# Ruyi-Zha/endosurf

Measured on AMD Instinct MI355X. Metric: training rays/sec (1024 rays x 64 samples), higher is better.
Workload: dtype f32

## Files before the change

### endosurf_amd/_lib.py

```python
from __future__ import annotations

import ctypes as C
import os

HERE = os.path.dirname(os.path.abspath(__file__))
LIB_PATH = os.path.join(HERE, "lib", "libendosurf_hip.so")

_c_float_p = C.c_void_p


class es_points(C.Structure):
    _fields_ = [("x", C.c_void_p), ("t", C.c_void_p), ("dirs", C.c_void_p), ("rays", C.c_void_p), ("z", C.c_void_p),
                ("mode", C.c_int), ("t_scalar", C.c_int), ("n_per_ray", C.c_int), ("ldz", C.c_int), ("M", C.c_int), ("M_split", C.c_int)]


class es_composite_args(C.Structure):
    _fields_ = ([(n, C.c_void_p) for n in ("rays", "z")] + [("ldz", C.c_int)]
                + [(n, C.c_void_p) for n in ("sdf", "g_o", "rgb", "variance")]
                + [("N", C.c_int), ("S", C.c_int), ("sample_dist", C.c_float), ("cos_anneal", C.c_float)]
                + [(n, C.c_void_p) for n in ("color", "depth", "weights", "cdf", "weight_max", "eik_acc", "wmax_idx",
                                             "g_color", "g_depth", "g_weights", "g_cdf", "g_wmax", "g_gradients_o", "g_eik",
                                             "eik_den", "d_sdf", "d_go", "d_rgb", "d_invs_acc", "ray_part", "cos_anneal_dev",
                                             "go_copy", "g_aux_sdf", "g_aux_go")] + [("n_aux", C.c_int)])


class es_render_args(C.Structure):
    _fields_ = [("c", es_composite_args), ("ws", C.c_void_p), ("scratch", C.c_void_p), ("flags", C.c_int), ("wg_scratch", C.c_void_p), ("packed_x3", C.c_void_p)]


class es_loss_args(C.Structure):
    _fields_ = ([(n, C.c_void_p) for n in ("color_map", "depth_map", "eik", "aux_sdf", "aux_go", "rays", "eod_pts", "color_gt", "depth_gt",
                                            "mask", "cmask", "valid_sn")]
                + [("N", C.c_int)] + [(n, C.c_float) for n in ("w_color", "w_depth", "w_sdf", "w_angle", "w_eik", "w_sn")]
                + [(n, C.c_void_p) for n in ("terms", "g_color", "g_depth", "g_eik", "g_aux_sdf", "g_aux_go", "den_out", "den_global")]
                + [("world", C.c_float), ("total_out", C.c_void_p)])


_P = C.c_void_p
_I = C.c_int
_F = C.c_float

PROTOTYPES = {
    "es_abi_version": (C.c_int, []),
    "es_last_error": (C.c_char_p, []),
    "es_init": (C.c_int, []),
    "es_param_floats": (C.c_int64, []),
    "es_param_layout": (C.c_int, [C.c_int, C.c_int, C.POINTER(C.c_int64), C.POINTER(C.c_int64), C.POINTER(C.c_int64),
                                  C.POINTER(C.c_int), C.POINTER(C.c_int)]),
    "es_param_variance_off": (C.c_int64, []),
    "es_weff_floats": (C.c_int64, []),
    "es_weff_layout": (C.c_int, [C.c_int, C.c_int, C.POINTER(C.c_int64), C.POINTER(C.c_int64)]),
    "es_packed_floats": (C.c_int64, []),
    "es_weightnorm_pack": (C.c_int, [_c_float_p, _c_float_p, _c_float_p, C.c_int, C.c_void_p]),
    "es_weightnorm_backward": (C.c_int, [_c_float_p, _c_float_p, _c_float_p, C.c_int, C.c_void_p]),
    "es_query_sdf": (C.c_int, [C.POINTER(es_points), _c_float_p, _c_float_p, _c_float_p, C.c_int, C.c_void_p]),
    "es_query_sdf_tiles": (C.c_int, [C.POINTER(es_points), _c_float_p, _c_float_p, _c_float_p, C.c_int, C.c_int, C.c_void_p]),
    "es_deform_forward": (_I, [C.POINTER(es_points), _P, _P, _P, _P, _P]),
    "es_deform_inverse": (_I, [C.POINTER(es_points), _P, _P, _P, _I, _F, _P, _P, _P, _P]),
    "es_deform_jacobian": (_I, [C.POINTER(es_points), _P, _P, _P, _P, _P]),
    "es_strain_rows": (_I, [_P, _P, _P, _I, _P, _P, _P, _P, _P, _P, _P]),
    "es_trace_surface": (_I, [_P, _I, _F, _F, _F, _F, _I, _I, _P, _P, _I, _P, _P, _P, _P, _P, _P]),
    "es_packed_x3_bytes": (C.c_int64, []),
    "es_pack_x3": (_I, [_P, _P, _I, _P]),
    "es_query_sdf_x3": (_I, [C.POINTER(es_points), _P, _P, _P, _I, _P, _I, _P]),
    "es_ray_setup": (_I, [_P, _P, _I, _I, _F, _I, _P, _I, _P, _P, _P]),
    "es_upsample_step": (_I, [_P, _P, _I, _P, _I, _I, _I, _I, _F, _P, _P, _I, _P, _P]),
    "es_merge_sdf": (_I, [_P, _I, _P, _I, _P, _I, _I, _I, _P, _P]),
    "es_mid_z": (_I, [_P, _I, _I, _I, _F, _P, _P]),
    "es_composite_forward": (_I, [C.POINTER(es_composite_args), _P]),
    "es_composite_backward": (_I, [C.POINTER(es_composite_args), _P]),
    "es_march_find": (_I, [_P, _P, _I, _I, _F, _P, _P, _P, _P]),
    "es_secant_points": (_I, [_P, _P, _I, _P, _P, _P]),
    "es_secant_update": (_I, [_P, _I, _F, _P, _P, _P]),
    "es_march_finish": (_I, [_P, _P, _I, _P, _P]),
    "es_point_workspace_floats": (C.c_int64, [_I, _I]),
    "es_point_workspace_offset": (C.c_int64, [_I, _I, _I]),
    "es_point_forward": (_I, [C.POINTER(es_points), _P, _P, _P, _I, _I, _P]),
    "es_point_forward_rows": (_I, [C.POINTER(es_points), _P, _P, _P, _I, _I, _I, _I, _P]),
    "es_eod_points": (_I, [_P, _P, _P, _I, _P, _P, _P, _P]),
    "es_sn_points": (_I, [_P, _P, _P, _P, _F, _I, _P, _P, _P, _P]),
    "es_eod_loss": (_I, [_P, _P, _P, _P, _P, _I, _P, _P, _P]),
    "es_eod_loss_backward": (_I, [_P, _P, _P, _P, _P, _P, _P, _I, _P, _P, _P]),
    "es_sn_loss": (_I, [_P, _P, _I, _P, _P]),
    "es_sn_loss_backward": (_I, [_P, _P, _P, _P, _I, _P, _P]),
    "es_copy2": (_I, [_P, _P, C.c_longlong, _P, _P, C.c_longlong, _P]),
    "es_color_forward": (_I, [C.POINTER(es_points), _P, _P, _P, _P]),
    "es_point_vjp": (_I, [C.POINTER(es_points), _P, _P, _P, _I, _P]),
    "es_point_backward_stages": (_I, [C.POINTER(es_points), _P, _P, _P, _I, _I, _P, _P, _P, _P, _P, _I, _P]),
    "es_weightnorm_backward_layers": (_I, [_P, _P, _P, _I, _I, _P]),
    "es_point_forward_x3": (_I, [C.POINTER(es_points), _P, _P, _P, _P, _I, _I, _P]),
    "es_gemm_atb": (_I, [_P, _P, _I, _P, _I, _P, _P]),
    "es_point_backward_x3": (_I, [C.POINTER(es_points), _P, _P, _P, _P, _I, _I, _P, _P, _P, _P, _P, _P]),
    "es_point_backward": (_I, [C.POINTER(es_points), _P, _P, _P, _I, _I, _P, _P, _P, _P, _P]),
    "es_wgrad_scratch_floats": (C.c_int64, []),
    "es_point_backward_det": (_I, [C.POINTER(es_points), _P, _P, _P, _I, _I, _P, _P, _P, _P, _P, _P]),
    "es_train_loss": (_I, [C.POINTER(es_loss_args), _P]),
    "es_query_sdf_rays": (_I, [C.POINTER(es_points), _P, _P, _P, _I, _P, _I, _P]),
    "es_march_progress": (_I, [_P, _I, _I, _I, C.c_float, _P, _P]),
    "es_variance_terms": (_I, [_P, _P, _P, _P, _P]),
    "es_sample_scratch_floats": (C.c_int64, [_I, _I, _I, _I]),
    "es_sample_z": (_I, [_P, _P, _I, _I, _I, _I, _I, _P, _P, _I, _P, _P, _P]),
    "es_march_scratch_floats": (C.c_int64, [_I, _I]),
    "es_ray_marching": (_I, [_P, _I, _I, _I, C.c_float, _I, _P, _P, _I, _P, _P, _P]),
    "es_render_scratch_floats": (C.c_int64, [_I, _I]),
    "es_render_forward": (_I, [C.POINTER(es_render_args), _P, _P, _P]),
    "es_render_backward": (_I, [C.POINTER(es_render_args), _P, _P, _P, _P]),
    "es_train_aux_points": (_I, [_P, _P, _P, _P, _P, C.c_float, _I, _P, _P, _P, _P]),
    "es_adam_step": (_I, [_P, _P, _P, _P, C.c_longlong, C.c_float, C.c_float, C.c_float, C.c_float, C.c_float, C.c_float, _P, C.c_longlong, _P]),
    "es_train_schedule": (_I, [_P, C.c_double, C.c_double, C.c_double, C.c_double, C.c_double, C.c_double, C.c_float, C.c_double, _P, _P]),
    "es_adam_step_dev": (_I, [_P, _P, _P, _P, C.c_longlong, C.c_float, C.c_float, C.c_float, _P, _P, C.c_longlong, _P]),
    "es_zero": (_I, [_P, C.c_longlong, _P]),
    "es_uniform": (_I, [_P, C.c_longlong, C.c_ulonglong, C.c_ulonglong, _P, _P]),
    "es_scale": (_I, [_P, _P, C.c_longlong, _P, _P]),
    "es_render_finish": (_I, [_P, _P, _P, _I, _P, _P, _P, _P, _P]),
    "es_iso_scratch_bytes": (C.c_int64, [_I, _I, _I]),
    "es_iso_count": (_I, [_P, _I, _I, _I, C.c_double, _P, _P, _P]),
    "es_iso_emit": (_I, [_P, _I, _I, _I, C.c_double, _P, C.c_longlong, C.c_longlong, _P, _P, _P, _P]),
    "es_cubes_scratch_bytes": (C.c_int64, [_I, _I, _I]),
    "es_cubes_count": (_I, [_P, _I, _I, _I, C.c_double, _P, _P, _P]),
    "es_cubes_emit": (_I, [_P, _I, _I, _I, C.c_double, _P, C.c_longlong, C.c_longlong, _P, _P, _P, _P]),
    "es_band_scratch_bytes": (C.c_int64, [_I, _I, _I, _I]),
    "es_band_lattice_points": (_I, [_P, _P, _P, _I, _I, _I, _I, C.c_longlong, C.c_longlong, _P, _P]),
    "es_band_seed": (_I, [_P, _I, _I, _I, _I, C.c_double, C.c_double, _P, _P, _P]),
# ... 102 lines not shown
```

### endosurf_amd/csrc/api.hip

```cpp
#include "arch.h"
#include "chain_common.h"
#include "host.h"
#include "launch.h"
#include "workspace.h"

namespace es {
static inline PointSrc to_src(const es_points* p) { PointSrc s; static_cast<es_points&>(s) = *p; return s; }
static inline int check_src(const es_points* p) {
    ES_REQUIRE(p != nullptr, "es_points is null");
    ES_REQUIRE(p->M >= 0, "negative point count");
    if (p->M == 0) return ST_OK;
    if (p->mode == 0) {
        ES_REQUIRE(p->x && p->t, "mode 0 needs x and t");
    } else {
        ES_REQUIRE(p->mode == 1 || p->mode == 2, "unknown point-source mode");
        ES_REQUIRE(p->rays && p->z && p->n_per_ray > 0 && p->ldz >= p->n_per_ray, "modes 1/2 need rays, z, n_per_ray <= ldz");
        if (p->mode == 2) ES_REQUIRE(p->M_split >= 0 && p->M_split <= p->M && (p->M_split == p->M || (p->x && p->t)), "mode 2 needs M_split <= M and x, t");
    }
    return ST_OK;
}
static inline int check_points(const es_points* p, bool weights, bool rows) {
    if (int e = check_src(p)) return e;
    ES_REQUIRE(weights && (rows || p->M == 0), "null buffer");
    return ST_OK;
// ... 143 lines not shown
    constexpr float FMAX = 3.402823466e+38f;
    ES_REQUIRE(N >= 0, "es_trace_surface: N must not be negative");
    ES_REQUIRE(tau >= -FMAX && tau <= FMAX, "es_trace_surface: tau must be finite");
    ES_REQUIRE(eps >= 0.f && eps <= FMAX, "es_trace_surface: eps must be finite and not negative");
    ES_REQUIRE(relax > 0.f && relax <= 1.f, "es_trace_surface: relax must be in (0, 1]");
    ES_REQUIRE(min_step > 0.f && min_step <= FMAX, "es_trace_surface: min_step must be finite and positive");
    ES_REQUIRE(max_iters >= 1 && max_iters <= ES_TRACE_MAX_ITERS, "es_trace_surface: max_iters must be in [1, 1024]");
    ES_REQUIRE(tile_points == 0 || tile_points == 32 || tile_points == 64, "es_trace_surface: tile_points: 0 (the library's choice), 32 or 64");
    if (N == 0) return ST_OK;
    ES_REQUIRE(rays && packed && weff && depth_out && status_out, "es_trace_surface: null buffer (rays, packed, weff, depth_out, status_out)");
    return trace_surface(rays, N, tau, eps, relax, min_step, max_iters, tile_points, packed, weff, use_deform, depth_out, status_out, iters_out,
                         residual_out, points_out, (hipStream_t)stream);
}
int64_t es_packed_x3_bytes(void) { return (int64_t)packed_x3_bytes(); }
int es_pack_x3(const float* weff, void* packed_x3, int use_deform, void* stream) {
    ES_REQUIRE(weff && packed_x3, "null buffer");
    return pack_x3(weff, packed_x3, use_deform, (hipStream_t)stream);
}
int es_query_sdf_x3(const es_points* pts, const void* packed_x3, const float* weff, float* sdf_out, int ld_out, const int* ray_done,
                    int use_deform, void* stream) {
    if (int e = check_points(pts, packed_x3 && weff, sdf_out)) return e;
    ES_REQUIRE(ld_out == 0 || (pts->mode == 1 && ld_out >= pts->n_per_ray), "ld_out > 0 needs ray samples (mode 1), ld_out >= n_per_ray");
    ES_REQUIRE(ray_done == nullptr || pts->mode == 1, "ray_done needs ray samples (mode 1)");
    return query_sdf_x3(to_src(pts), packed_x3, weff, sdf_out, use_deform, (hipStream_t)stream, ld_out, ray_done);
}
int es_variance_terms(const float* variance, const float* d_invs_acc, float* s_val, float* d_var, void* stream) {
    ES_REQUIRE(variance && (s_val || d_var) && (!d_var || d_invs_acc), "es_variance_terms arguments");
    return variance_terms(variance, d_invs_acc, s_val, d_var, (hipStream_t)stream);
}
int es_march_progress(const float* sdf, int N, int n, int n_valid, float tau, int* done, void* stream) {
    if (N == 0) return ST_OK;
    ES_REQUIRE(sdf && done && n >= 2 && n_valid >= 1 && n_valid <= n, "es_march_progress arguments");
    return march_progress(sdf, N, n, n_valid, tau, done, (hipStream_t)stream);
}

int es_ray_setup(const float* rays, const float* u, int N, int n, float sample_dist, int lin_mode, float* z, int ldz,
                 float* near_out, float* far_out, void* stream) {
    if (N == 0) return ST_OK;
    ES_REQUIRE(rays && z && N >= 0 && n >= 1 && ldz >= n, "es_ray_setup arguments");
    return ray_setup(rays, u, N, n, sample_dist, lin_mode, z, ldz, near_out, far_out, (hipStream_t)stream);
}
int es_upsample_step(const float* rays, const float* z_in, int ld_in, const float* sdf_in, int ld_sdf, int N, int n, int n_imp,
                     float inv_s, float* z_new, float* z_out, int ld_out, int32_t* src_idx, void* stream) {
    if (N == 0) return ST_OK;
    ES_REQUIRE(rays && z_in && sdf_in && z_new && z_out && src_idx && ld_in >= n && ld_sdf >= n, "es_upsample_step arguments");
    return upsample_step(rays, z_in, ld_in, sdf_in, ld_sdf, N, n, n_imp, inv_s, z_new, z_out, ld_out, src_idx, (hipStream_t)stream);
}
int es_merge_sdf(const float* sdf_in, int ld_in, const float* sdf_new, int n_imp, const int32_t* src_idx, int ld_out, int N, int n,
                 float* sdf_out, void* stream) {
    if (N == 0) return ST_OK;
    ES_REQUIRE(sdf_in && sdf_new && src_idx && sdf_out && sdf_out != sdf_in, "es_merge_sdf arguments (out must not alias in)");
    return merge_sdf(sdf_in, ld_in, sdf_new, n_imp, src_idx, ld_out, N, n, sdf_out, (hipStream_t)stream);
}
int es_mid_z(const float* z, int ldz, int N, int S, float sample_dist, float* mid, void* stream) {
    if (N == 0) return ST_OK;
    ES_REQUIRE(z && mid && ldz >= S && S >= 1, "es_mid_z arguments");
    return mid_z(z, ldz, N, S, sample_dist, mid, (hipStream_t)stream);
}
int es_composite_forward(const es_composite_args* a, void* stream) {
    if (a && a->N == 0) return ST_OK;
    ES_REQUIRE(a && a->rays && a->z && a->sdf && a->g_o && a->rgb && a->variance, "es_composite_forward inputs");
    ES_REQUIRE(a->color && a->depth && a->weights && a->cdf && a->weight_max && a->eik_acc && a->wmax_idx, "es_composite_forward outputs");
    return composite(as_comp(a), 0, (hipStream_t)stream);
}
int es_composite_backward(const es_composite_args* a, void* stream) {
    if (a && a->N == 0) return ST_OK;
    ES_REQUIRE(a && a->rays && a->z && a->sdf && a->g_o && a->rgb && a->variance, "es_composite_backward inputs");
    ES_REQUIRE(a->n_aux >= 0, "es_composite_backward: negative n_aux");
    ES_REQUIRE(a->g_color && a->g_depth && a->g_eik && a->eik_den && a->d_sdf && a->d_go && a->d_rgb && a->d_invs_acc,
               "es_composite_backward adjoints");
    return composite(as_comp(a), 1, (hipStream_t)stream);
}
int es_march_find(const float* sdf, const float* dprop, int N, int n, float tau, float* state, int32_t* flags, float* d_pred, void* stream) {
    if (N == 0) return ST_OK;
    ES_REQUIRE(sdf && dprop && state && flags && d_pred && n >= 2, "es_march_find arguments");
    return march_find(sdf, dprop, N, n, tau, state, flags, d_pred, (hipStream_t)stream);
}
int es_secant_points(const float* rays, const float* d_pred, int N, float* x, float* t, void* stream) {
    if (N == 0) return ST_OK;
    ES_REQUIRE(rays && d_pred && x && t, "es_secant_points arguments");
    return secant_points(rays, d_pred, N, x, t, (hipStream_t)stream);
}
int es_secant_update(const float* sdf_mid, int N, float tau, float* state, float* d_pred, void* stream) {
    if (N == 0) return ST_OK;
    ES_REQUIRE(sdf_mid && state && d_pred, "es_secant_update arguments");
    return secant_update(sdf_mid, N, tau, state, d_pred, (hipStream_t)stream);
}
int es_march_finish(const float* d_pred, const int32_t* flags, int N, float* d_out, void* stream) {
    if (N == 0) return ST_OK;
    ES_REQUIRE(d_pred && flags && d_out, "es_march_finish arguments");
    return march_finish(d_pred, flags, N, d_out, (hipStream_t)stream);
}

int64_t es_point_workspace_floats(int M, int flags) { return M <= 0 ? 0 : (int64_t)ws_layout(M, flags).off[WS_COUNT]; }
int64_t es_point_workspace_offset(int M, int flags, int buffer_id) {
    if (M <= 0 || buffer_id < 0 || buffer_id >= WS_COUNT) return -1;
    return (int64_t)ws_layout(M, flags).off[buffer_id];
}
int es_point_forward(const es_points* pts, const float* packed, const float* weff, float* ws, int flags, int m_color, void* stream) {
    if (int e = check_point_call(pts, packed && weff, ws, flags, m_color, false)) return e;
    return point_forward(to_src(pts), packed, weff, ws, flags, m_color, (hipStream_t)stream);
}
int es_point_forward_rows(const es_points* pts, const float* packed, const float* weff, float* ws, int flags, int m_color, int row0, int nrows,
                          void* stream) {
    if (int e = check_points(pts, packed && weff, ws)) return e;
    ES_REQUIRE(!(flags & (ES_PF_X3 | ES_PF_X3_CHAIN)), "es_point_forward_rows: fp32 family only");
    ES_REQUIRE(!(flags & ES_PF_COLOR) || pts->mode != 0 || pts->dirs, "colour evaluation needs view directions");
    ES_REQUIRE(row0 >= 0 && nrows >= 0, "es_point_forward_rows: negative row range");
    if (int e = check_mcolor(pts, flags, m_color)) return e;
    return point_forward_rows(to_src(pts), packed, weff, ws, flags, m_color, row0, nrows, (hipStream_t)stream);
}
int es_eod_points(const float* rays, const float* depth_gt, const float* mask, int N, float* x, float* t, float* inside, void* stream) {
    ES_REQUIRE(N >= 0 && (N == 0 || (rays && depth_gt && x && t)), "es_eod_points buffers");
    ES_REQUIRE(inside == nullptr || mask != nullptr || N == 0, "es_eod_points: the inside mask needs the ray mask");
    return eod_points(rays, depth_gt, mask, N, x, t, inside, (hipStream_t)stream);
}
int es_sn_points(const float* rays, const float* mask, const float* d_i, const float* u, float rad, int N, float* x, float* t,
                 unsigned char* valid, void* stream) {
    ES_REQUIRE(N >= 0 && (N == 0 || (rays && mask && d_i && u && x && t && valid)), "es_sn_points buffers");
    return sn_points(rays, mask, d_i, u, rad, N, x, t, valid, (hipStream_t)stream);
}
int es_eod_loss(const float* rays, const float* pts, const float* mask, const float* sdf, const float* g_o, int N, float* out, float* inside,
                void* stream) {
    ES_REQUIRE(N >= 0 && out && (N == 0 || (rays && pts && mask && sdf && g_o && inside)), "es_eod_loss buffers");
// ... 120 lines not shown
```

### endosurf_amd/csrc/host.h

```cpp
#pragma once
#include <hip/hip_runtime.h>

#include <cstddef>
#include <type_traits>

#include "../../include/endosurf_hip.h"

namespace es {

struct PointSrc; struct WsLayout; struct FwdArgs; struct BwdArgs;

struct CompositeArgs : ::es_composite_args {};
struct LossArgs : ::es_loss_args {};
static_assert(sizeof(CompositeArgs) == sizeof(es_composite_args) && std::is_standard_layout<CompositeArgs>::value, "es::CompositeArgs is es_composite_args");
static_assert(sizeof(LossArgs) == sizeof(es_loss_args) && std::is_standard_layout<LossArgs>::value, "es::LossArgs is es_loss_args");
inline const CompositeArgs& as_comp(const es_composite_args* a) { return *reinterpret_cast<const CompositeArgs*>(a); }

int init_tables();
int weightnorm_pack(const float* params, float* weff, float* packed, int use_deform, hipStream_t st);
int weightnorm_backward(const float* params, const float* dweff, float* dparams, int use_deform, hipStream_t st);
int weightnorm_backward_layers(const float* params, const float* dweff, float* dparams, int first_layer, int n_layers, hipStream_t st);

int query_sdf(const PointSrc& src, const float* packed, const float* weff, float* sdf_out, int use_deform, hipStream_t st,
              int ld_out = 0, const int* ray_done = nullptr, int tile_points = 0);
int query_sdf16(const PointSrc& src, const float* packed, const float* weff, float* sdf_out, int use_deform, hipStream_t st);
size_t packed_x3_bytes();
int pack_x3(const float* weff, void* packed_x3, int use_deform, hipStream_t st);
int query_sdf_x3(const PointSrc& src, const void* packed_x3, const float* weff, float* sdf_out, int use_deform, hipStream_t st, int ld_out, const int* ray_done);

int deform_forward(const PointSrc& src, const float* packed, const float* weff, float* xc_out, float* d_out, hipStream_t st);
int deform_inverse(const PointSrc& src, const float* init, const float* packed, const float* weff, int max_iters, float tol, float* y_out,
                   float* step_out, int* iters_out, hipStream_t st);

int trace_surface(const float* rays, int N, float tau, float eps, float relax, float min_step, int max_iters, int tile_points,
                  const float* packed, const float* weff, int use_deform, float* depth_out, int* status_out, int* iters_out,
                  float* residual_out, float* points_out, hipStream_t st);

int deform_jacobian(const PointSrc& src, const float* packed, const float* weff, float* jac_out, float* xc_out, hipStream_t st);
int strain_rows(const float* jac_from, const float* jac_to, const float* normals, int M, float* F_out, float* det_out, float* stretch_out,
                float* area_out, float* surface_out, unsigned char* valid_out, hipStream_t st);

int point_forward(const PointSrc& src, const float* packed, const float* weff, float* ws, int flags, int m_color, hipStream_t st,
                  const void* packed_x3 = nullptr);
int point_forward_rows(const PointSrc& src, const float* packed, const float* weff, float* ws, int flags, int m_color, int row0, int nrows, hipStream_t st);
int point_vjp(const PointSrc& src, const float* packed, const float* weff, float* ws, int flags, hipStream_t st);
int color_forward(const PointSrc& src, const float* packed, const float* weff, float* ws, hipStream_t st);
int point_backward_chains(const PointSrc& src, const float* packed, const float* weff, float* ws, int flags, int m_color,
                          const float* d_sdf, const float* d_go, const float* d_rgb, hipStream_t st, const void* packed_x3 = nullptr);

int deform_jvp_x3r(const PointSrc& src, const void* packed_r, const float* weff, float* ws, const WsLayout& L, bool save, hipStream_t st);
int deform_vjp_x3r(const PointSrc& src, const void* packed_r, const float* weff, float* ws, const WsLayout& L, bool save, hipStream_t st, int m_rows = 0);
int deform_jvp_x3r_with_tail(const FwdArgs& fa, const void* packed_r, int m_main, hipStream_t st);
int sdf_fwd_x3r(const PointSrc& src, const void* packed_r, const float* weff, float* ws, const WsLayout& L, bool deform, bool color, hipStream_t st);
int color_fwd_x3r(const PointSrc& src, const void* packed_r, const float* weff, float* ws, const WsLayout& L, bool deform, int Mcp, bool save, hipStream_t st);

int deform_tan_x3r(const PointSrc& src, const void* packed_r, const float* weff, float* ws, const WsLayout& L, const float* d_go, hipStream_t st, int m_rows = 0);
int deform_bwd_x3r_with_tail(const BwdArgs& ba, const void* packed_r, int m_main, hipStream_t st);
int color_bwd_x3r(const PointSrc& src, const void* packed_r, const float* weff, float* ws, const WsLayout& L, bool deform, int m_color, const float* d_rgb, hipStream_t st);
int deform_bwd_x3r(const void* packed_r, const float* weff, float* ws, const WsLayout& L, int M, int m_color, hipStream_t st);

int point_wgrad(int M, float* ws, int flags, int m_color, const float* d_sdf, float* dweff, float* det, hipStream_t st, int net_mask = 7);
size_t wgrad_det_floats();
int gemm_atb(const float* X, const float* dA, int M, float* out, int x3, float* det, hipStream_t st);

int ray_setup(const float* rays, const float* u, int N, int n, float sample_dist, int lin_mode, float* z, int ldz, float* near_out, float* far_out, hipStream_t st);
int upsample_step(const float* rays, const float* z_in, int ld_in, const float* sdf_in, int ld_sdf, int N, int n, int n_imp,
                  float inv_s, float* z_new, float* z_out, int ld_out, int* src_idx, hipStream_t st);
int merge_sdf(const float* sdf_in, int ld_in, const float* sdf_new, int n_imp, const int* src_idx, int ld_out, int N, int n, float* sdf_out, hipStream_t st);
int mid_z(const float* z, int ldz, int N, int S, float sample_dist, float* mid, hipStream_t st);
int composite(const CompositeArgs& a, int backward, hipStream_t st);
int variance_terms(const float* variance, const float* d_invs_acc, float* s_val, float* d_var, hipStream_t st);
int march_progress(const float* sdf, int N, int n, int n_valid, float tau, int* done, hipStream_t st);
int march_find(const float* sdf, const float* dprop, int N, int n, float tau, float* state, int* flags, float* d_pred, hipStream_t st);
int secant_points(const float* rays, const float* d_pred, int N, float* x, float* t, hipStream_t st);
int secant_update(const float* sdf_mid, int N, float tau, float* state, float* d_pred, hipStream_t st);
int march_finish(const float* d_pred, const int* flags, int N, float* d_out, hipStream_t st);
int train_aux_points(const float* rays, const float* depth_gt, const float* mask, const float* d_i, const float* u, float rad, int N, float* x, float* t, unsigned char* valid, hipStream_t st);

int eod_points(const float* rays, const float* depth_gt, const float* mask, int N, float* x, float* t, float* inside, hipStream_t st);
int sn_points(const float* rays, const float* mask, const float* d_i, const float* u, float rad, int N, float* x, float* t, unsigned char* valid, hipStream_t st);
int eod_loss(const float* rays, const float* pts, const float* mask, const float* sdf, const float* go, int N, float* out, float* inside, hipStream_t st);
int eod_loss_bwd(const float* rays, const float* inside, const float* sdf, const float* go, const float* out, const float* g_sdf_err,
                 const float* g_ang_err, int N, float* d_sdf, float* d_go, hipStream_t st);
int sn_loss(const float* g, const unsigned char* valid, int N, float* out, hipStream_t st);
int sn_loss_bwd(const float* g, const unsigned char* valid, const float* out, const float* g_loss, int N, float* d_g, hipStream_t st);
int copy2(float* da, const float* sa, long long na, float* db, const float* sb, long long nb, hipStream_t st);

int train_loss(const LossArgs& a, hipStream_t st);
int train_schedule(double* state, double lr_init, double n_iter, double warm_up_end, double lr_alpha, double beta1, double beta2, float grad_scale, double anneal_end, float* scal, hipStream_t st);
int adam_step_dev(float* p, const float* g, float* m, float* v, long long n, float beta1, float beta2, float eps, const float* scal, const float* g_extra, long long extra_index, hipStream_t st);
int adam_step(float* p, const float* g, float* m, float* v, long long n, float beta1, float beta2, float eps, float step_size,
              float bc2_sqrt, float grad_scale, const float* g_extra, long long extra_index, hipStream_t st);
int uniform(float* out, long long n, unsigned long long seed, unsigned long long subseq, const double* subseq_dev, hipStream_t st);
int scale(float* out, const float* in, long long n, const float* s, hipStream_t st);
int zero(void* p, long long nbytes, hipStream_t st);
int render_finish(const float* eik_acc, const float* aux_sdf_ws, const float* aux_go_ws, int n_aux, float* eik, float* eik_den, float* aux_sdf, float* aux_go, hipStream_t st);

}
```

### endosurf_amd/csrc/pack.hip

```cpp
#include <hip/hip_runtime.h>

#include "arch.h"
#include "host.h"
#include "launch.h"

namespace es {

struct SegDev {
    int net, layer, dir, row0, col0, kreal, nreal, skip_scale, kg, nt;
    unsigned long long off4;
};
__constant__ SegDev c_segs[SEG_COUNT];
__constant__ int c_layer_k[NETS * LAYERS];
__constant__ int c_layer_n[NETS * LAYERS];
__constant__ int c_param_off[NETS * LAYERS];
__constant__ int c_weff_off[NETS * LAYERS];
__constant__ int c_p16_segs[P16_COUNT];
#define P16_SEGS_DEV(i) c_p16_segs[i]

static DeviceOnce g_tables_ready;

int init_tables() {
    if (!g_tables_ready.first()) return 0;
    SegDev h[SEG_COUNT];
    size_t off = 0;
    for (int i = 0; i < SEG_COUNT; ++i) {
        const SegDesc& s = SEGS[i];
        h[i] = {s.net, s.layer, s.dir, s.row0, s.col0, s.kreal, s.nreal, s.skip_scale, seg_kg(s), seg_nt(s), (unsigned long long)off};
        off += (size_t)seg_kg(s) * seg_nt(s) * 64;
    }
    int lk[NETS * LAYERS], ln[NETS * LAYERS], po[NETS * LAYERS], wo[NETS * LAYERS];
    int p = 0, w = 0;
    for (int n = 0; n < NETS; ++n)
        for (int l = 0; l < LAYERS; ++l) {
            lk[n * LAYERS + l] = LAYER_K[n][l];
            ln[n * LAYERS + l] = LAYER_N[n][l];
            po[n * LAYERS + l] = p;
            wo[n * LAYERS + l] = w;
            p += LAYER_N[n][l] * (2 + LAYER_K[n][l]);
            w += LAYER_N[n][l] * (1 + LAYER_K[n][l]);
        }
    ES_HIP(hipMemcpyToSymbol(HIP_SYMBOL(c_segs), h, sizeof(h)));
    ES_HIP(hipMemcpyToSymbol(HIP_SYMBOL(c_layer_k), lk, sizeof(lk)));
    ES_HIP(hipMemcpyToSymbol(HIP_SYMBOL(c_layer_n), ln, sizeof(ln)));
    ES_HIP(hipMemcpyToSymbol(HIP_SYMBOL(c_param_off), po, sizeof(po)));
    ES_HIP(hipMemcpyToSymbol(HIP_SYMBOL(c_weff_off), wo, sizeof(wo)));
    ES_HIP(hipMemcpyToSymbol(HIP_SYMBOL(c_p16_segs), P16_SEGS, sizeof(P16_SEGS)));
    g_tables_ready.done();
    return 0;
}

__device__ __forceinline__ float wave_sum(float v) {
#pragma unroll
    for (int o = 32; o > 0; o >>= 1) v += __shfl_xor(v, o, 64);
    return v;
}

__global__ __launch_bounds__(256) void k_weff(const float* __restrict__ params, float* __restrict__ weff, int first_layer) {
    const int li = first_layer + blockIdx.y;
    const int N = c_layer_n[li], K = c_layer_k[li];
    const int n = blockIdx.x * 4 + (threadIdx.x >> 6);
    const int lane = threadIdx.x & 63;
    if (n >= N) return;
    const float* pb = params + c_param_off[li];
    const float* pg = pb + N;
    const float* pv = pg + N + (size_t)n * K;
    float ss = 0.f;
    for (int k = lane; k < K; k += 64) { const float v = pv[k]; ss = fmaf(v, v, ss); }
    ss = wave_sum(ss);
    const float scale = pg[n] / sqrtf(ss);
    float* w = weff + c_weff_off[li];
    for (int k = lane; k < K; k += 64) w[(size_t)n * K + k] = scale * pv[k];
    if (lane == 0) w[(size_t)N * K + n] = pb[n];
}

__global__ __launch_bounds__(256) void k_pack(const float* __restrict__ weff, float4* __restrict__ packed, int first_net) {
    const unsigned long long idx = (unsigned long long)blockIdx.x * 256 + threadIdx.x;
    if (idx >= PACKED_FLOAT4) return;
    int s = 0;
#pragma unroll 1
    for (int i = 1; i < SEG_COUNT; ++i)
        if (idx >= c_segs[i].off4) s = i;
    const SegDev sd = c_segs[s];
    if (sd.net < first_net) return;
    const unsigned rel = (unsigned)(idx - sd.off4);
    const int lane = rel & 63;
    const int g = (rel >> 6) % sd.kg;
    const int nt = (rel >> 6) / sd.kg;
    const int li = sd.net * LAYERS + sd.layer;
    const int K = c_layer_k[li];
    const float* W = weff + c_weff_off[li];
    const float sc = sd.skip_scale ? INV_SQRT2 : 1.f;
    const int n = 32 * nt + (lane & 31);
    float o[4];
#pragma unroll
    for (int j = 0; j < 4; ++j) {
        const int k = 8 * g + 2 * j + (lane >> 5);
        float v = 0.f;
        if (k < sd.kreal && n < sd.nreal) {
            const int row = sd.dir == 0 ? sd.row0 + n : sd.row0 + k;
            const int col = sd.dir == 0 ? sd.col0 + k : sd.col0 + n;
            v = sc * W[(size_t)row * K + col];
        }
        o[j] = v;
    }
    packed[idx] = make_float4(o[0], o[1], o[2], o[3]);
}

__global__ __launch_bounds__(256) void k_weightnorm_bwd(const float* __restrict__ params, const float* __restrict__ dweff,
                                                        float* __restrict__ dparams, int first_layer) {
    const int li = first_layer + blockIdx.y;
    const int N = c_layer_n[li], K = c_layer_k[li];
    const int n = blockIdx.x * 4 + (threadIdx.x >> 6);
    const int lane = threadIdx.x & 63;
    if (n >= N) return;
    const float* pb = params + c_param_off[li];
    const float* pg = pb + N;
    const float* pv = pg + N + (size_t)n * K;
    const float* dw = dweff + c_weff_off[li] + (size_t)n * K;
    const float lscale = (li % LAYERS) == 4 ? INV_SQRT2 : 1.f;
    float ss = 0.f, dot = 0.f;
    for (int k = lane; k < K; k += 64) { const float v = pv[k]; ss = fmaf(v, v, ss); dot = fmaf(dw[k] * lscale, v, dot); }
    ss = wave_sum(ss); dot = wave_sum(dot);
    const float inv = 1.f / sqrtf(ss);
    const float dg = dot * inv;
    const float gs = pg[n] * inv;
    float* ob = dparams + c_param_off[li];
    float* og = ob + N;
    float* ov = og + N + (size_t)n * K;
    for (int k = lane; k < K; k += 64) ov[k] = gs * (dw[k] * lscale - dg * inv * pv[k]);
    if (lane == 0) { og[n] = dg; ob[n] = dweff[c_weff_off[li] + (size_t)N * K + n]; }
}

__global__ __launch_bounds__(256) void k_pack16(const float* __restrict__ weff, float4* __restrict__ packed, int first_net) {
    const unsigned long long idx = PACKED_FLOAT4 + (unsigned long long)blockIdx.x * 256 + threadIdx.x;
    if (idx >= PACKED_TOTAL_FLOAT4) return;
    int pi = 0;
    unsigned long long base = PACKED_FLOAT4, off = PACKED_FLOAT4;
#pragma unroll 1
    for (int i = 0; i < P16_COUNT; ++i) {
        const unsigned long long sz = (unsigned long long)((c_segs[P16_SEGS_DEV(i)].kreal + 15) / 16) * 16 * 64;
        if (idx >= off) { pi = i; base = off; }
        off += sz;
    }
    const SegDev sd = c_segs[P16_SEGS_DEV(pi)];
    if (sd.net < first_net) return;
    const int kg = (sd.kreal + 15) / 16;
    const unsigned rel = (unsigned)(idx - base);
    const int lane = rel & 63;
    const int g = (rel >> 6) % kg;
    const int nt = (rel >> 6) / kg;
    const int li = sd.net * LAYERS + sd.layer;
    const int K = c_layer_k[li];
    const float* W = weff + c_weff_off[li];
    const float sc = sd.skip_scale ? INV_SQRT2 : 1.f;
    const int n = 16 * nt + (lane & 15);
    float o[4];
#pragma unroll
    for (int j = 0; j < 4; ++j) {
        const int k = 16 * g + 4 * j + (lane >> 4);
        o[j] = (k < sd.kreal && n < sd.nreal) ? sc * W[(size_t)(sd.row0 + n) * K + sd.col0 + k] : 0.f;
    }
    packed[idx] = make_float4(o[0], o[1], o[2], o[3]);
}

int weightnorm_pack(const float* params, float* weff, float* packed, int use_deform, hipStream_t st) {
    if (int e = init_tables()) return e;
    const int first_layer = use_deform ? 0 : LAYERS;
    dim3 g1(65, NETS * LAYERS - first_layer);
    hipLaunchKernelGGL(k_weff, g1, dim3(256), 0, st, params, weff, first_layer);
    const unsigned nb = (unsigned)((PACKED_FLOAT4 + 255) / 256);
    hipLaunchKernelGGL(k_pack, dim3(nb), dim3(256), 0, st, (const float*)weff, reinterpret_cast<float4*>(packed), use_deform ? 0 : 1);
    const unsigned nb16 = (unsigned)((PACKED_TOTAL_FLOAT4 - PACKED_FLOAT4 + 255) / 256);
    hipLaunchKernelGGL(k_pack16, dim3(nb16), dim3(256), 0, st, (const float*)weff, reinterpret_cast<float4*>(packed), use_deform ? 0 : 1);
    return hip_last("weightnorm_pack");
}

int weightnorm_backward_layers(const float* params, const float* dweff, float* dparams, int first_layer, int n_layers, hipStream_t st) {
    if (int e = init_tables()) return e;
    if (n_layers <= 0) return ST_OK;
    dim3 g1(65, n_layers);
    hipLaunchKernelGGL(k_weightnorm_bwd, g1, dim3(256), 0, st, params, dweff, dparams, first_layer);
    return hip_last("weightnorm_backward_layers");
}

int weightnorm_backward(const float* params, const float* dweff, float* dparams, int use_deform, hipStream_t st) {
    if (int e = init_tables()) return e;
    const int first_layer = use_deform ? 0 : LAYERS;
    dim3 g1(65, NETS * LAYERS - first_layer);
    hipLaunchKernelGGL(k_weightnorm_bwd, g1, dim3(256), 0, st, params, dweff, dparams, first_layer);
    return hip_last("weightnorm_backward");
}

}
```

### endosurf_amd/csrc/rays.hip

```cpp
#include <hip/hip_runtime.h>

#include "host.h"
#include "launch.h"

namespace es {

constexpr int RAY_NMAX = 256;
constexpr int WAVES_PER_BLOCK = 4;

__device__ __forceinline__ float wsum(float v) {
#pragma unroll
    for (int o = 32; o > 0; o >>= 1) v += __shfl_xor(v, o, 64);
    return v;
}
__device__ __forceinline__ float wmax(float v) {
#pragma unroll
    for (int o = 32; o > 0; o >>= 1) v = fmaxf(v, __shfl_xor(v, o, 64));
    return v;
}
__device__ __forceinline__ float wscan_add(float v, int lane) {
#pragma unroll
    for (int o = 1; o < 64; o <<= 1) { const float t = __shfl_up(v, o, 64); if (lane >= o) v += t; }
    return v;
}
__device__ __forceinline__ float wscan_mul(float v, int lane) {
#pragma unroll
    for (int o = 1; o < 64; o <<= 1) { const float t = __shfl_up(v, o, 64); if (lane >= o) v *= t; }
    return v;
}
__device__ __forceinline__ float sigmoidf_acc(float x) { return 1.f / (1.f + expf(-x)); }

__device__ __forceinline__ float linspace_f32(float start, float end, int steps, int i) {
    if (steps == 1) return start;
    const float step = (end - start) / (float)(steps - 1);
    return i < steps / 2 ? start + step * (float)i : end - step * (float)(steps - 1 - i);
}

struct RayGeom { float o[3], d[3], dz[3], t; };
__device__ __forceinline__ RayGeom load_ray(const float* __restrict__ rays, int ray) {
    RayGeom g;
    const float* r = rays + 9 * (size_t)ray;
    g.o[0] = r[0]; g.o[1] = r[1]; g.o[2] = r[2];
    g.d[0] = r[3]; g.d[1] = r[4]; g.d[2] = r[5];
    const float inv = r[5] + 1e-6f;
    g.dz[0] = r[3] / inv; g.dz[1] = r[4] / inv; g.dz[2] = r[5] / inv;
    g.t = r[8];
    return g;
}
__device__ __forceinline__ void sphere_near_far(const RayGeom& g, float& near, float& far) {
    const float dd = g.d[0] * g.d[0] + g.d[1] * g.d[1] + g.d[2] * g.d[2];
    const float d1 = -(g.d[0] * g.o[0] + g.d[1] * g.o[1] + g.d[2] * g.o[2]) / dd;
    const float p0 = g.o[0] + d1 * g.d[0], p1 = g.o[1] + d1 * g.d[1], p2 = g.o[2] + d1 * g.d[2];
    const float tmp = 1.f - (p0 * p0 + p1 * p1 + p2 * p2);
    const float d2 = sqrtf(fmaxf(tmp, 0.f)) / sqrtf(dd);
    near = fmaxf(d1 - d2, 0.f);
    far = d1 + d2;
}
__device__ __forceinline__ float pt_norm(const RayGeom& g, float z) {
    const float x = g.o[0] + g.dz[0] * z, y = g.o[1] + g.dz[1] * z, w = g.o[2] + g.dz[2] * z;
    return sqrtf(x * x + y * y + w * w);
}

__global__ __launch_bounds__(256) void k_ray_setup(const float* __restrict__ rays, const float* __restrict__ u, int N, int n,
                                                   float sample_dist, int lin_mode, float* __restrict__ z, int ldz,
                                                   float* __restrict__ near_out, float* __restrict__ far_out) {
    const int ray = blockIdx.x * WAVES_PER_BLOCK + (threadIdx.x >> 6), lane = threadIdx.x & 63;
    if (ray >= N) return;
    const RayGeom g = load_ray(rays, ray);
    float near, far;
    sphere_near_far(g, near, far);
    const float shift = u ? (u[ray] - 0.5f) * sample_dist : 0.f;
    for (int s = lane; s < n; s += 64) {
        const float tv = linspace_f32(0.f, 1.f, n, s);
        float v = lin_mode == 0 ? near + (far - near) * tv : near * (1.f - tv) + far * tv;
        if (u) v = v + shift;
        z[(size_t)ray * ldz + s] = v;
    }
    if (lane == 0) { if (near_out) near_out[ray] = near; if (far_out) far_out[ray] = far; }
}

__global__ __launch_bounds__(256) void k_upsample_step(const float* __restrict__ rays, const float* __restrict__ z_in, int ld_in,
                                                       const float* __restrict__ sdf_in, int ld_sdf, int N, int n, int n_imp,
                                                       float inv_s, float* __restrict__ z_new, float* __restrict__ z_out,
                                                       int ld_out, int* __restrict__ src_idx) {
    __shared__ float s_z[WAVES_PER_BLOCK][RAY_NMAX], s_a[WAVES_PER_BLOCK][RAY_NMAX], s_c[WAVES_PER_BLOCK][RAY_NMAX + 1],
        s_new[WAVES_PER_BLOCK][64];
    const int wv = threadIdx.x >> 6, lane = threadIdx.x & 63;
    const int ray = blockIdx.x * WAVES_PER_BLOCK + wv;
    if (ray >= N) return;
    float* zs = s_z[wv]; float* av = s_a[wv]; float* cdf0 = s_c[wv]; float* nz = s_new[wv];
    const RayGeom g = load_ray(rays, ray);
    const int nsec = n - 1;

    for (int e = lane; e < n; e += 64) { zs[e] = z_in[(size_t)ray * ld_in + e]; av[e] = sdf_in[(size_t)ray * ld_sdf + e]; }
    __builtin_amdgcn_wave_barrier();
    for (int e = lane; e < nsec; e += 64) cdf0[e] = (av[e + 1] - av[e]) / (zs[e + 1] - zs[e] + 1e-6f);
    __builtin_amdgcn_wave_barrier();
    float carry = 1.f, wsum_acc = 0.f;
    const int nchunk = (nsec + 63) / 64;
    float wloc[RAY_NMAX / 64];
#pragma unroll
    for (int c = 0; c < RAY_NMAX / 64; ++c) {
        wloc[c] = 0.f;
        if (c < nchunk) {
            const int e = c * 64 + lane;
            float alpha = 0.f, om = 1.f;
            if (e < nsec) {
                const float cosv = cdf0[e], prev = e == 0 ? 0.f : cdf0[e - 1];
                const bool inside = pt_norm(g, zs[e]) < 1.f || pt_norm(g, zs[e + 1]) < 1.f;
                float cv = fminf(fmaxf(fminf(prev, cosv), -1e3f), 0.f);
                cv = inside ? cv : cv * 0.f;
                const float dist = zs[e + 1] - zs[e];
                const float mid = (av[e] + av[e + 1]) * 0.5f;
                const float pe = mid - cv * dist * 0.5f, ne = mid + cv * dist * 0.5f;
                const float pc = sigmoidf_acc(pe * inv_s), nc = sigmoidf_acc(ne * inv_s);
                alpha = (pc - nc + 1e-6f) / (pc + 1e-6f);
                om = 1.f - alpha + 1e-7f;
            }
            const float incl = wscan_mul(om, lane);
            float excl = __shfl_up(incl, 1, 64);
            if (lane == 0) excl = 1.f;
            const float T = carry * excl;
            carry = carry * __shfl(incl, 63, 64);
            const float w = e < nsec ? alpha * T + 1e-5f : 0.f;
            wloc[c] = w;
            wsum_acc += wsum(w);
        }
    }
    __builtin_amdgcn_wave_barrier();
    float run = 0.f;
#pragma unroll
    for (int c = 0; c < RAY_NMAX / 64; ++c) {
        if (c < nchunk) {
            const int e = c * 64 + lane;
            const float pdf = wloc[c] / wsum_acc;
            const float incl = wscan_add(pdf, lane) + run;
            run = __shfl(incl, 63, 64);
            if (e < nsec) cdf0[e + 1] = incl;
        }
    }
    if (lane == 0) cdf0[0] = 0.f;
    __builtin_amdgcn_wave_barrier();
    if (lane < n_imp) {
        const float uu = linspace_f32(0.5f / (float)n_imp, 1.f - 0.5f / (float)n_imp, n_imp, lane);
        int lo = 0, hi = n;
        while (lo < hi) { const int m = (lo + hi) >> 1; if (cdf0[m] <= uu) lo = m + 1; else hi = m; }
        const int below = max(lo - 1, 0), above = min(lo, n - 1);
        float denom = cdf0[above] - cdf0[below];
        if (denom < 1e-5f) denom = 1.f;
        const float tt = (uu - cdf0[below]) / denom;
        const float v = zs[below] + tt * (zs[above] - zs[below]);
        nz[lane] = v;
        z_new[(size_t)ray * n_imp + lane] = v;
    }
    __builtin_amdgcn_wave_barrier();
    for (int e = lane; e < n; e += 64) {
        const float v = zs[e];
        int cnt = 0;
        for (int j = 0; j < n_imp; ++j) cnt += nz[j] < v ? 1 : 0;
        const int r = e + cnt;
        z_out[(size_t)ray * ld_out + r] = v;
        src_idx[(size_t)ray * ld_out + r] = e;
    }
    if (lane < n_imp) {
        const float v = nz[lane];
        int lo = 0, hi = n;
        while (lo < hi) { const int m = (lo + hi) >> 1; if (zs[m] <= v) lo = m + 1; else hi = m; }
        int before = 0;
        for (int j = 0; j < n_imp; ++j) before += (nz[j] < v || (nz[j] == v && j < lane)) ? 1 : 0;
        const int r = lo + before;
        z_out[(size_t)ray * ld_out + r] = v;
        src_idx[(size_t)ray * ld_out + r] = n + lane;
    }
}

__global__ __launch_bounds__(256) void k_merge_sdf(const float* __restrict__ sdf_in, int ld_in, const float* __restrict__ sdf_new,
                                                   int n_imp, const int* __restrict__ src_idx, int ld_out, int N, int n,
                                                   float* __restrict__ sdf_out) {
    const int i = blockIdx.x * 256 + threadIdx.x;
    const int tot = n + n_imp;
    if (i >= N * tot) return;
    const int ray = i / tot, r = i - ray * tot;
    const int s = src_idx[(size_t)ray * ld_out + r];
    float v = __builtin_nanf("");
    if (s >= 0 && s < n) v = sdf_in[(size_t)ray * ld_in + s];
    else if (s >= n && s < tot) v = sdf_new[(size_t)ray * n_imp + (s - n)];
    sdf_out[(size_t)ray * ld_out + r] = v;
}

__global__ __launch_bounds__(256) void k_mid_z(const float* __restrict__ z, int ldz, int N, int S, float sample_dist,
                                               float* __restrict__ mid) {
    const int i = blockIdx.x * 256 + threadIdx.x;
    if (i >= N * S) return;
    const int ray = i / S, s = i - ray * S;
    const float z0 = z[(size_t)ray * ldz + s];
    const float dist = s + 1 < S ? z[(size_t)ray * ldz + s + 1] - z0 : sample_dist;
    mid[(size_t)ray * S + s] = z0 + dist * 0.5f;
}


__device__ __forceinline__ float inv_s_from_variance(float var) { return fminf(fmaxf(expf(var * 10.f), 1e-6f), 1e6f); }

template <bool BWD>
__global__ __launch_bounds__(256) void k_composite(CompositeArgs a) {
    if (BWD && a.n_aux > 0) {
        const size_t P = (size_t)a.N * a.S;
        for (int i = blockIdx.x * 256 + threadIdx.x; i < a.n_aux; i += gridDim.x * 256) {
            a.d_sdf[P + i] = a.g_aux_sdf ? a.g_aux_sdf[i] : 0.f;
#pragma unroll
            for (int k = 0; k < 3; ++k) a.d_go[3 * (P + i) + k] = a.g_aux_go ? a.g_aux_go[3 * (size_t)i + k] : 0.f;
        }
    }
    const int ray = blockIdx.x * WAVES_PER_BLOCK + (threadIdx.x >> 6), lane = threadIdx.x & 63;
    if (ray >= a.N) return;
    const RayGeom g = load_ray(a.rays, ray);
    const float inv_s = inv_s_from_variance(a.variance[0]);
    const float r = a.cos_anneal_dev != nullptr ? a.cos_anneal_dev[0] : a.cos_anneal;
    const int S = a.S;
    const int nchunk = (S + 63) / 64;
    constexpr int CH = RAY_NMAX / 64;
    float alpha[CH], Texc[CH], w[CH], mid[CH], dist[CH], pcv[CH], ncv[CH], sdfv[CH], tc[CH], gnorm[CH], relax[CH], ratio[CH];
    float go[CH][3], rgb[CH][3];
    float carry = 1.f;
    float csum[3] = {0.f, 0.f, 0.f}, dsum = 0.f, wmx = -1.f, e_num = 0.f, e_den = 0.f;
    int wmx_i = 0;
#pragma unroll
    for (int c = 0; c < CH; ++c) {
        if (c < nchunk) {
            const int s = c * 64 + lane;
            const bool ok = s < S;
            const size_t p = (size_t)ray * S + (ok ? s : 0);
            const float z0 = a.z[(size_t)ray * a.ldz + (ok ? s : 0)];
            dist[c] = (ok && s + 1 < S) ? a.z[(size_t)ray * a.ldz + s + 1] - z0 : a.sample_dist;
            mid[c] = z0 + dist[c] * 0.5f;
            sdfv[c] = a.sdf[p];
#pragma unroll
            for (int k = 0; k < 3; ++k) { go[c][k] = a.g_o[3 * p + k]; rgb[c][k] = a.rgb[3 * p + k]; }
            tc[c] = g.d[0] * go[c][0] + g.d[1] * go[c][1] + g.d[2] * go[c][2];
            const float ic = -(fmaxf(-tc[c] * 0.5f + 0.5f, 0.f) * (1.f - r) + fmaxf(-tc[c], 0.f) * r);
            const float nx = sdfv[c] + ic * dist[c] * 0.5f, pv = sdfv[c] - ic * dist[c] * 0.5f;
            pcv[c] = sigmoidf_acc(pv * inv_s);
            ncv[c] = sigmoidf_acc(nx * inv_s);
            ratio[c] = (pcv[c] - ncv[c] + 1e-6f) / (pcv[c] + 1e-6f);
            alpha[c] = ok ? fminf(fmaxf(ratio[c], 0.f), 1.f) : 0.f;
            const float om = ok ? 1.f - alpha[c] + 1e-7f : 1.f;
            const float incl = wscan_mul(om, lane);
            float excl = __shfl_up(incl, 1, 64);
            if (lane == 0) excl = 1.f;
            Texc[c] = carry * excl;
            carry = carry * __shfl(incl, 63, 64);
            w[c] = alpha[c] * Texc[c];
            gnorm[c] = sqrtf(go[c][0] * go[c][0] + go[c][1] * go[c][1] + go[c][2] * go[c][2]);
            relax[c] = (ok && pt_norm(g, mid[c]) < 1.2f) ? 1.f : 0.f;
            if (ok) {
                csum[0] += w[c] * rgb[c][0]; csum[1] += w[c] * rgb[c][1]; csum[2] += w[c] * rgb[c][2];
                dsum += w[c] * mid[c];
                e_num += relax[c] * (gnorm[c] - 1.f) * (gnorm[c] - 1.f);
                e_den += relax[c];
                if (w[c] > wmx) { wmx = w[c]; wmx_i = s; }
            }
        }
    }
    {
        float m = wmx; int mi = wmx_i;
#pragma unroll
        for (int o = 32; o > 0; o >>= 1) {
            const float om = __shfl_xor(m, o, 64); const int oi = __shfl_xor(mi, o, 64);
            if (om > m || (om == m && oi < mi)) { m = om; mi = oi; }
        }
        wmx = m; wmx_i = mi;
    }
    if (!BWD) {
#pragma unroll
        for (int k = 0; k < 3; ++k) csum[k] = wsum(csum[k]);
        dsum = wsum(dsum); e_num = wsum(e_num); e_den = wsum(e_den);
#pragma unroll
        for (int c = 0; c < CH; ++c)
            if (c < nchunk) {
                const int s = c * 64 + lane;
                if (s < S) {
                    a.weights[(size_t)ray * S + s] = w[c]; a.cdf[(size_t)ray * S + s] = pcv[c];
                    if (a.go_copy != nullptr) {
                        const size_t p = (size_t)ray * S + s;
                        a.go_copy[3 * p] = go[c][0]; a.go_copy[3 * p + 1] = go[c][1]; a.go_copy[3 * p + 2] = go[c][2];
                    }
                }
            }
        if (lane == 0) {
            a.color[3 * (size_t)ray + 0] = csum[0]; a.color[3 * (size_t)ray + 1] = csum[1]; a.color[3 * (size_t)ray + 2] = csum[2];
            a.depth[ray] = dsum; a.weight_max[ray] = wmx; a.wmax_idx[ray] = wmx_i;
            if (a.ray_part) { a.ray_part[2 * (size_t)ray] = e_num; a.ray_part[2 * (size_t)ray + 1] = e_den; }
            else { atomicAdd(a.eik_acc + 0, e_num); atomicAdd(a.eik_acc + 1, e_den); }
        }
        return;
    }
    const float gc0 = a.g_color[3 * (size_t)ray], gc1 = a.g_color[3 * (size_t)ray + 1], gc2 = a.g_color[3 * (size_t)ray + 2];
    const float gd = a.g_depth[ray];
    const float gwm = a.g_wmax ? a.g_wmax[ray] : 0.f;
    const float geik = a.g_eik[0] / a.eik_den[0];
    float suffix_carry = 0.f, dinvs = 0.f;
#pragma unroll
    for (int c = CH - 1; c >= 0; --c) {
        if (c < nchunk) {
            const int s = c * 64 + lane;
            const bool ok = s < S;
            const size_t p = (size_t)ray * S + (ok ? s : 0);
            float wbar = 0.f;
            if (ok) {
                wbar = (a.g_weights ? a.g_weights[p] : 0.f) + gc0 * rgb[c][0] + gc1 * rgb[c][1] + gc2 * rgb[c][2] + gd * mid[c];
                if (s == wmx_i) wbar += gwm;
            }
            const float ww = ok ? wbar * w[c] : 0.f;
            float incl = ww;
#pragma unroll
            for (int o = 1; o < 64; o <<= 1) { const float t = __shfl_down(incl, o, 64); if (lane + o < 64) incl += t; }
            const float later = incl - ww + suffix_carry;
            suffix_carry += __shfl(incl, 0, 64);
            if (ok) {
                float abar = wbar * Texc[c] - later / (1.f - alpha[c] + 1e-7f);
                if (ratio[c] < 0.f || ratio[c] > 1.f) abar = 0.f;
                const float cden = pcv[c] + 1e-6f;
                const float pbar = abar / cden;
                const float cbar = -abar * (pcv[c] - ncv[c] + 1e-6f) / (cden * cden) + (a.g_cdf ? a.g_cdf[p] : 0.f);
                const float pcbar = pbar + cbar, ncbar = -pbar;
                const float dpv = pcbar * pcv[c] * (1.f - pcv[c]);
                const float dnx = ncbar * ncv[c] * (1.f - ncv[c]);
                const float ic = -(fmaxf(-tc[c] * 0.5f + 0.5f, 0.f) * (1.f - r) + fmaxf(-tc[c], 0.f) * r);
                const float nx = sdfv[c] + ic * dist[c] * 0.5f, pv = sdfv[c] - ic * dist[c] * 0.5f;
                dinvs += dpv * pv + dnx * nx;
                const float prevbar = dpv * inv_s, nextbar = dnx * inv_s;
                a.d_sdf[p] = prevbar + nextbar;
                const float icbar = (nextbar - prevbar) * dist[c] * 0.5f;
                const float tcbar = icbar * ((-tc[c] * 0.5f + 0.5f > 0.f ? 0.5f * (1.f - r) : 0.f) + (-tc[c] > 0.f ? r : 0.f));
                const float en = relax[c] * geik * 2.f * (gnorm[c] - 1.f);
                const float invn = gnorm[c] > 0.f ? 1.f / gnorm[c] : 0.f;
#pragma unroll
                for (int k = 0; k < 3; ++k) {
                    float v = tcbar * g.d[k] + en * go[c][k] * invn;
                    if (a.g_gradients_o) v += a.g_gradients_o[3 * p + k];
                    a.d_go[3 * p + k] = v;
                    a.d_rgb[3 * p + k] = w[c] * (k == 0 ? gc0 : (k == 1 ? gc1 : gc2));
                }
            }
        }
    }
    dinvs = wsum(dinvs);
    if (lane == 0) {
        if (a.ray_part) a.ray_part[2 * (size_t)ray] = dinvs;
        else atomicAdd(a.d_invs_acc, dinvs);
    }
}
__global__ __launch_bounds__(1024) void k_ray_part_reduce(const float* __restrict__ part, int N, int ncol, float* __restrict__ acc) {
    __shared__ float sh[1024];
    for (int j = 0; j < ncol; ++j) {
        float s = 0.f;
        for (int i = threadIdx.x; i < N; i += 1024) s += part[2 * (size_t)i + j];
        sh[threadIdx.x] = s;
        __syncthreads();
        for (int o = 512; o > 0; o >>= 1) {
            if ((int)threadIdx.x < o) sh[threadIdx.x] += sh[threadIdx.x + o];
            __syncthreads();
        }
        if (threadIdx.x == 0) acc[j] += sh[0];
        __syncthreads();
    }
}

__global__ __launch_bounds__(256) void k_march_find(const float* __restrict__ sdf, const float* __restrict__ dprop, int N, int n,
                                                    float tau, float* __restrict__ state, int* __restrict__ flags,
                                                    float* __restrict__ d_pred) {
    const int ray = blockIdx.x * WAVES_PER_BLOCK + (threadIdx.x >> 6), lane = threadIdx.x & 63;
    if (ray >= N) return;
    const float* v = sdf + (size_t)ray * n;
    int first = 0x7fffffff;
    for (int s = lane; s + 1 < n; s += 64) {
        const float a0 = -(v[s] - tau), a1 = -(v[s + 1] - tau);
        if (a0 * a1 < 0.f) first = min(first, s);
    }
#pragma unroll
    for (int o = 32; o > 0; o >>= 1) first = min(first, __shfl_xor(first, o, 64));
    if (lane == 0) {
        const float v0 = -(v[0] - tau);
        const bool m0 = v0 < 0.f;
        bool mask = false;
        float dl = 0.f, fl = -1.f, dh = 1.f, fh = 1.f;
        if (first != 0x7fffffff) {
            const int i2 = min(first + 1, n - 1);
            fl = -(v[first] - tau); fh = -(v[i2] - tau);
            dl = dprop[(size_t)ray * n + first]; dh = dprop[(size_t)ray * n + i2];
            mask = (fl < 0.f) && m0;
        }
        state[4 * (size_t)ray + 0] = dl; state[4 * (size_t)ray + 1] = fl; state[4 * (size_t)ray + 2] = dh; state[4 * (size_t)ray + 3] = fh;
        flags[ray] = (mask ? 1 : 0) | (m0 ? 2 : 0);
        d_pred[ray] = -fl * (dh - dl) / (fh - fl) + dl;
    }
}
__global__ __launch_bounds__(256) void k_march_progress(const float* __restrict__ sdf, int N, int n, int n_valid, float tau,
                                                        int* __restrict__ done) {
    const int ray = blockIdx.x * WAVES_PER_BLOCK + (threadIdx.x >> 6), lane = threadIdx.x & 63;
    if (ray >= N) return;
    const float* v = sdf + (size_t)ray * n;
    int found = 0;
    for (int s = lane; s + 1 < n_valid; s += 64) {
        const float a0 = -(v[s] - tau), a1 = -(v[s + 1] - tau);
        if (a0 * a1 < 0.f) found = 1;
    }
    if (lane == 0 && !(-(v[0] - tau) < 0.f)) found = 1;
#pragma unroll
    for (int o = 32; o > 0; o >>= 1) found |= __shfl_xor(found, o, 64);
    if (lane == 0) done[ray] = found;
}
__global__ __launch_bounds__(256) void k_secant_points(const float* __restrict__ rays, const float* __restrict__ d_pred, int N,
                                                       float* __restrict__ x, float* __restrict__ t) {
    const int i = blockIdx.x * 256 + threadIdx.x;
    if (i >= N) return;
    const float* r = rays + 9 * (size_t)i;
    const float dp = d_pred[i];
    x[3 * (size_t)i + 0] = r[0] + dp * (r[3] / r[5]);
// ... 10 lines not shown
    if (fm < 0.f) { dl = dp; fl = fm; } else { dh = dp; fh = fm; }
    state[4 * (size_t)i] = dl; state[4 * (size_t)i + 1] = fl; state[4 * (size_t)i + 2] = dh; state[4 * (size_t)i + 3] = fh;
    d_pred[i] = -fl * (dh - dl) / (fh - fl) + dl;
}
__global__ __launch_bounds__(256) void k_march_finish(const float* __restrict__ d_pred, const int* __restrict__ flags, int N,
                                                      float* __restrict__ d_out) {
    const int i = blockIdx.x * 256 + threadIdx.x;
    if (i >= N) return;
    const int f = flags[i];
    float v = (f & 1) ? d_pred[i] : __builtin_inff();
    if (!(f & 2)) v = 0.f;
    d_out[i] = v;
}

__global__ __launch_bounds__(256) void k_train_aux_points(const float* __restrict__ rays, const float* __restrict__ depth_gt,
                                                          const float* __restrict__ mask, const float* __restrict__ d_i,
                                                          const float* __restrict__ u, float rad, int N, float* __restrict__ x,
                                                          float* __restrict__ t, unsigned char* __restrict__ valid) {
    const int i = blockIdx.x * 256 + threadIdx.x;
    if (i >= N) return;
    const float* r = rays + 9 * (size_t)i;
    const float inv = r[5] + 1e-6f;
    const float dz[3] = {r[3] / inv, r[4] / inv, r[5] / inv};
    const float di = d_i[i];
    const bool ok = !__builtin_isinf(di) && !__builtin_isnan(di) && di != 0.f && mask[i] == 1.f;
    const float ds = ok ? di : 0.f, dg = depth_gt[i];
#pragma unroll
    for (int c = 0; c < 3; ++c) {
        const float ps = r[c] + ds * dz[c];
        x[3 * (size_t)i + c] = r[c] + dz[c] * dg;
        x[3 * (size_t)(N + i) + c] = ps;
        x[3 * (size_t)(2 * N + i) + c] = ps + (u[3 * (size_t)i + c] - 0.5f) * rad;
    }
    t[i] = r[8]; t[N + i] = r[8]; t[2 * N + i] = r[8];
    valid[i] = ok ? 1 : 0;
}

static inline dim3 ray_grid(int N) { return dim3((N + WAVES_PER_BLOCK - 1) / WAVES_PER_BLOCK); }

int ray_setup(const float* rays, const float* u, int N, int n, float sample_dist, int lin_mode, float* z, int ldz, float* near_out,
              float* far_out, hipStream_t st) {
    if (N <= 0) return ST_OK;
    hipLaunchKernelGGL(k_ray_setup, ray_grid(N), dim3(256), 0, st, rays, u, N, n, sample_dist, lin_mode, z, ldz, near_out, far_out);
    return hip_last("ray_setup");
}
int upsample_step(const float* rays, const float* z_in, int ld_in, const float* sdf_in, int ld_sdf, int N, int n, int n_imp,
                  float inv_s, float* z_new, float* z_out, int ld_out, int* src_idx, hipStream_t st) {
    ES_REQUIRE(n >= 2 && n <= RAY_NMAX && n_imp >= 1 && n_imp <= 64 && n + n_imp <= ld_out, "upsample_step sizes");
    if (N <= 0) return ST_OK;
    hipLaunchKernelGGL(k_upsample_step, ray_grid(N), dim3(256), 0, st, rays, z_in, ld_in, sdf_in, ld_sdf, N, n, n_imp, inv_s, z_new,
                       z_out, ld_out, src_idx);
    return hip_last("upsample_step");
}
int merge_sdf(const float* sdf_in, int ld_in, const float* sdf_new, int n_imp, const int* src_idx, int ld_out, int N, int n,
              float* sdf_out, hipStream_t st) {
    if (N <= 0) return ST_OK;
    const int tot = N * (n + n_imp);
    hipLaunchKernelGGL(k_merge_sdf, dim3((tot + 255) / 256), dim3(256), 0, st, sdf_in, ld_in, sdf_new, n_imp, src_idx, ld_out, N, n, sdf_out);
    return hip_last("merge_sdf");
}
int mid_z(const float* z, int ldz, int N, int S, float sample_dist, float* mid, hipStream_t st) {
    if (N <= 0) return ST_OK;
    hipLaunchKernelGGL(k_mid_z, dim3((N * S + 255) / 256), dim3(256), 0, st, z, ldz, N, S, sample_dist, mid);
    return hip_last("mid_z");
}
int composite(const CompositeArgs& a, int backward, hipStream_t st) {
    ES_REQUIRE(a.S >= 1 && a.S <= RAY_NMAX, "composite: samples per ray out of range");
    if (a.N <= 0) return ST_OK;
    if (backward) hipLaunchKernelGGL(k_composite<true>, ray_grid(a.N), dim3(256), 0, st, a);
    else hipLaunchKernelGGL(k_composite<false>, ray_grid(a.N), dim3(256), 0, st, a);
    if (a.ray_part)
        hipLaunchKernelGGL(k_ray_part_reduce, dim3(1), dim3(1024), 0, st, a.ray_part, a.N, backward ? 1 : 2, backward ? a.d_invs_acc : a.eik_acc);
    return hip_last("composite");
}
int march_find(const float* sdf, const float* dprop, int N, int n, float tau, float* state, int* flags, float* d_pred, hipStream_t st) {
    if (N <= 0) return ST_OK;
    hipLaunchKernelGGL(k_march_find, ray_grid(N), dim3(256), 0, st, sdf, dprop, N, n, tau, state, flags, d_pred);
    return hip_last("march_find");
}
__global__ void k_variance_terms(const float* __restrict__ variance, const float* __restrict__ d_invs_acc, float* __restrict__ s_val,
                                 float* __restrict__ d_var) {
    if (threadIdx.x != 0 || blockIdx.x != 0) return;
    const float e = expf(variance[0] * 10.f);
    if (s_val) s_val[0] = 1.f / fminf(fmaxf(e, 1e-6f), 1e6f);
    if (d_var) d_var[0] = (e >= 1e-6f && e <= 1e6f) ? d_invs_acc[0] * 10.f * e : 0.f;
}
int variance_terms(const float* variance, const float* d_invs_acc, float* s_val, float* d_var, hipStream_t st) {
    hipLaunchKernelGGL(k_variance_terms, dim3(1), dim3(64), 0, st, variance, d_invs_acc, s_val, d_var);
    return hip_last("variance_terms");
}

int march_progress(const float* sdf, int N, int n, int n_valid, float tau, int* done, hipStream_t st) {
    if (N <= 0) return ST_OK;
    hipLaunchKernelGGL(k_march_progress, ray_grid(N), dim3(256), 0, st, sdf, N, n, n_valid, tau, done);
    return hip_last("march_progress");
}
int secant_points(const float* rays, const float* d_pred, int N, float* x, float* t, hipStream_t st) {
    if (N <= 0) return ST_OK;
    hipLaunchKernelGGL(k_secant_points, dim3((N + 255) / 256), dim3(256), 0, st, rays, d_pred, N, x, t);
    return hip_last("secant_points");
}
int secant_update(const float* sdf_mid, int N, float tau, float* state, float* d_pred, hipStream_t st) {
    if (N <= 0) return ST_OK;
    hipLaunchKernelGGL(k_secant_update, dim3((N + 255) / 256), dim3(256), 0, st, sdf_mid, N, tau, state, d_pred);
    return hip_last("secant_update");
}
int train_aux_points(const float* rays, const float* depth_gt, const float* mask, const float* d_i, const float* u, float rad, int N,
                     float* x, float* t, unsigned char* valid, hipStream_t st) {
    if (N <= 0) return ST_OK;
    hipLaunchKernelGGL(k_train_aux_points, dim3((N + 255) / 256), dim3(256), 0, st, rays, depth_gt, mask, d_i, u, rad, N, x, t, valid);
    return hip_last("train_aux_points");
}
int march_finish(const float* d_pred, const int* flags, int N, float* d_out, hipStream_t st) {
    if (N <= 0) return ST_OK;
    hipLaunchKernelGGL(k_march_finish, dim3((N + 255) / 256), dim3(256), 0, st, d_pred, flags, N, d_out);
    return hip_last("march_finish");
}

}
```

### endosurf_amd/csrc/stages.hip

```cpp
#include "chain_common.h"
#include "host.h"
#include "launch.h"
#include "workspace.h"

using namespace es;

static inline long long up64(size_t n) { return (long long)((n + 63) / 64 * 64); }

struct SampleScratch { float *z, *sdf_a, *sdf_b; int* src; float *sdf_c0, *z_new, *sdf_new; long long floats; };
static SampleScratch sample_scratch(float* scratch, int N, int n_samples, int S, int n_imp) {
    Carver c(scratch);
    const long long NS = up64((size_t)N * S), NI = up64((size_t)N * n_imp);
    SampleScratch s{c.take<float>(NS), c.take<float>(NS), c.take<float>(NS), c.take<int>(NS), c.take<float>(up64((size_t)N * n_samples)),
                    c.take<float>(NI), c.take<float>(NI), 0};
    s.floats = c.off / (long long)sizeof(float);
    return s;
}
int64_t es_sample_scratch_floats(int N, int n_samples, int n_importance, int up_sample_steps) {
    if (N <= 0 || n_samples <= 0) return 0;
    const int n_imp_all = n_importance > 0 ? n_importance : 0;
    return sample_scratch(nullptr, N, n_samples, n_samples + n_imp_all, up_sample_steps > 0 ? n_imp_all / up_sample_steps : 0).floats;
}
int es_sample_z(const float* rays, const float* u_perturb, int N, int n_samples, int n_importance, int up_sample_steps, int upsample,
                const float* packed, const float* weff, int use_deform, float* z_out, float* scratch, void* stream) {
    if (N == 0) return ST_OK;
    ES_REQUIRE(rays && z_out && packed && weff && N >= 0 && n_samples >= 2, "es_sample_z arguments");
    hipStream_t st = (hipStream_t)stream;
    const bool do_up = upsample && n_importance > 0 && up_sample_steps > 0;
    const int S = n_samples + (do_up ? n_importance : 0);
    const float sample_dist = 2.0f / (float)n_samples;
    if (!do_up) return ray_setup(rays, u_perturb, N, n_samples, sample_dist, 0, z_out, S, nullptr, nullptr, st);
    ES_REQUIRE(scratch != nullptr && n_importance % up_sample_steps == 0, "es_sample_z needs scratch and n_importance divisible by up_sample_steps");
    const int n_imp = n_importance / up_sample_steps;
    const SampleScratch sc = sample_scratch(scratch, N, n_samples, S, n_imp);
    float* zbuf[2] = {z_out, sc.z};
    int cur = up_sample_steps % 2;
    if (int e = ray_setup(rays, u_perturb, N, n_samples, sample_dist, 0, zbuf[cur], S, nullptr, nullptr, st)) return e;
    PointSrc ps{};
    ps.rays = rays; ps.mode = 1; ps.t_scalar = 0;
    ps.z = zbuf[cur]; ps.n_per_ray = n_samples; ps.ldz = S; ps.M = N * n_samples;
    if (int e = query_sdf(ps, packed, weff, sc.sdf_c0, use_deform, st)) return e;
    const float* sdf_c = sc.sdf_c0;
    int ld_sdf = n_samples, n = n_samples;
    for (int i = 0; i < up_sample_steps; ++i) {
        if (int e = upsample_step(rays, zbuf[cur], S, sdf_c, ld_sdf, N, n, n_imp, 64.f * (float)(1 << i), sc.z_new, zbuf[cur ^ 1], S, sc.src, st)) return e;
        if (i + 1 != up_sample_steps) {
            ps.z = sc.z_new; ps.n_per_ray = n_imp; ps.ldz = n_imp; ps.M = N * n_imp;
            if (int e = query_sdf(ps, packed, weff, sc.sdf_new, use_deform, st)) return e;
            float* dst = sdf_c != sc.sdf_a ? sc.sdf_a : sc.sdf_b;
            if (int e = merge_sdf(sdf_c, ld_sdf, sc.sdf_new, n_imp, sc.src, S, N, n, dst, st)) return e;
            sdf_c = dst; ld_sdf = S;
        }
        cur ^= 1;
        n += n_imp;
    }
    return ST_OK;
}

struct RenderScratch { float *mid, *d_sdf, *d_go, *d_rgb; long long floats; };
static RenderScratch render_scratch(float* scratch, int N, int S) {
    Carver c(scratch);
    const long long P = up64((size_t)N * S), P3 = up64(3 * (size_t)N * S);
    RenderScratch r{c.take<float>(P), c.take<float>(P), c.take<float>(P3), c.take<float>(P3), 0};
    r.floats = c.off / (long long)sizeof(float);
    return r;
}
int64_t es_render_scratch_floats(int N, int S) {
    if (N <= 0 || S <= 0) return 0;
    return render_scratch(nullptr, N, S).floats;
}
static int render_points(const es_render_args* a, PointSrc& ps, int& flags) {
    ES_REQUIRE(a && a->c.rays && a->c.z && a->c.variance && a->ws && a->scratch && a->c.N >= 0 && a->c.S >= 1 && a->c.ldz >= a->c.S,
               "es_render arguments");
    ps = PointSrc{};
    ps.rays = a->c.rays; ps.z = render_scratch(a->scratch, a->c.N, a->c.S).mid; ps.mode = 1; ps.n_per_ray = a->c.S; ps.ldz = a->c.S; ps.M = a->c.N * a->c.S;
    flags = (a->flags & (ES_PF_DEFORM | ES_PF_SAVE | ES_PF_X3)) | ES_PF_COLOR;
    return ST_OK;
}
static CompositeArgs render_composite_args(const es_render_args* a, int flags) {
    CompositeArgs c = as_comp(&a->c);
    const WsLayout L = ws_layout(a->c.N * a->c.S, flags);
    c.sdf = a->ws + L.off[WS_SDF]; c.g_o = a->ws + L.off[WS_GO]; c.rgb = a->ws + L.off[WS_RGB];
    const RenderScratch r = render_scratch(a->scratch, a->c.N, a->c.S);
    c.d_sdf = r.d_sdf; c.d_go = r.d_go; c.d_rgb = r.d_rgb;
    c.n_aux = 0; c.g_aux_sdf = nullptr; c.g_aux_go = nullptr;
    return c;
}
int es_render_forward(const es_render_args* a, const float* packed, const float* weff, void* stream) {
    if (a && a->c.N == 0) return ST_OK;
    PointSrc ps; int flags;
    if (int e = render_points(a, ps, flags)) return e;
    ES_REQUIRE(packed && weff, "null weights");
    ES_REQUIRE(a->c.color && a->c.depth && a->c.weights && a->c.cdf && a->c.weight_max && a->c.eik_acc && a->c.wmax_idx, "es_render_forward outputs");
    hipStream_t st = (hipStream_t)stream;
    if (int e = mid_z(a->c.z, a->c.ldz, a->c.N, a->c.S, a->c.sample_dist, render_scratch(a->scratch, a->c.N, a->c.S).mid, st)) return e;
    if ((flags & ES_PF_X3) && (flags & ES_PF_SAVE) && a->packed_x3) flags = (flags & ~ES_PF_X3) | ES_PF_X3_CHAIN;
    if (int e = point_forward(ps, packed, weff, a->ws, flags, 0, st, a->packed_x3)) return e;
    return composite(render_composite_args(a, flags), 0, st);
}
int es_render_backward(const es_render_args* a, const float* packed, const float* weff, float* dweff, void* stream) {
    if (a && a->c.N == 0) return ST_OK;
    PointSrc ps; int flags;
    if (int e = render_points(a, ps, flags)) return e;
    ES_REQUIRE(packed && weff && dweff, "null weights / gradient buffer");
// ... 56 lines not shown
```

### endosurf_amd/csrc/step.hip

```cpp
#include <hip/hip_runtime.h>

#include <cstdint>

#include "host.h"
#include "launch.h"

namespace es {

__device__ __forceinline__ void philox_round(uint32_t (&c)[4], uint32_t k0, uint32_t k1) {
    const uint64_t p0 = (uint64_t)0xD2511F53u * c[0], p1 = (uint64_t)0xCD9E8D57u * c[2];
    const uint32_t n0 = (uint32_t)(p1 >> 32) ^ c[1] ^ k0, n2 = (uint32_t)(p0 >> 32) ^ c[3] ^ k1;
    c[1] = (uint32_t)p1; c[3] = (uint32_t)p0; c[0] = n0; c[2] = n2;
}
__global__ __launch_bounds__(256) void k_uniform(float* __restrict__ out, long long n, unsigned long long seed, unsigned long long subseq,
                                                 const double* __restrict__ subseq_dev) {
    const long long q = (long long)blockIdx.x * 256 + threadIdx.x;
    if (4 * q >= n) return;
    if (subseq_dev != nullptr) subseq += (unsigned long long)subseq_dev[0];
    uint32_t c[4] = {(uint32_t)q, (uint32_t)((unsigned long long)q >> 32), (uint32_t)subseq, (uint32_t)(subseq >> 32)};
    uint32_t k0 = (uint32_t)seed, k1 = (uint32_t)(seed >> 32);
#pragma unroll
    for (int r = 0; r < 10; ++r) {
        philox_round(c, k0, k1);
        k0 += 0x9E3779B9u; k1 += 0xBB67AE85u;
    }
#pragma unroll
    for (int j = 0; j < 4; ++j)
        if (4 * q + j < n) out[4 * q + j] = (float)(c[j] >> 8) * (1.f / 16777216.f);
}
int uniform(float* out, long long n, unsigned long long seed, unsigned long long subseq, const double* subseq_dev, hipStream_t st) {
    if (n <= 0) return ST_OK;
    const long long quads = (n + 3) / 4;
    hipLaunchKernelGGL(k_uniform, dim3((unsigned)((quads + 255) / 256)), dim3(256), 0, st, out, n, seed, subseq, subseq_dev);
    return hip_last("uniform");
}

__global__ __launch_bounds__(256) void k_scale(float* __restrict__ out, const float* __restrict__ in, long long n, const float* __restrict__ s) {
    const long long i = (long long)blockIdx.x * 256 + threadIdx.x;
    if (i < n) out[i] = in[i] * s[0];
}
int scale(float* out, const float* in, long long n, const float* s, hipStream_t st) {
    if (n <= 0) return ST_OK;
    hipLaunchKernelGGL(k_scale, dim3((unsigned)((n + 255) / 256)), dim3(256), 0, st, out, in, n, s);
    return hip_last("scale");
}

int zero(void* p, long long nbytes, hipStream_t st) {
    if (nbytes <= 0) return ST_OK;
    if (hipMemsetAsync(p, 0, (size_t)nbytes, st) != hipSuccess) return hip_last("zero");
    return ST_OK;
}

__global__ __launch_bounds__(256) void k_render_finish(const float* __restrict__ eik_acc, const float* __restrict__ aux_sdf_ws,
                                                       const float* __restrict__ aux_go_ws, int n_aux, float* __restrict__ eik,
                                                       float* __restrict__ eik_den, float* __restrict__ aux_sdf, float* __restrict__ aux_go) {
    const int i = blockIdx.x * 256 + threadIdx.x;
    if (i == 0) {
        const float den = eik_acc[1] + 1e-6f;
        eik_den[0] = den;
        eik_den[1] = den;
        eik[0] = eik_acc[0] / den;
    }
    if (i < n_aux) aux_sdf[i] = aux_sdf_ws[i];
    if (i < 3 * n_aux) aux_go[i] = aux_go_ws[i];
}
int render_finish(const float* eik_acc, const float* aux_sdf_ws, const float* aux_go_ws, int n_aux, float* eik, float* eik_den, float* aux_sdf,
                  float* aux_go, hipStream_t st) {
    const int n = 3 * n_aux > 1 ? 3 * n_aux : 1;
    hipLaunchKernelGGL(k_render_finish, dim3((n + 255) / 256), dim3(256), 0, st, eik_acc, aux_sdf_ws, aux_go_ws, n_aux, eik, eik_den, aux_sdf, aux_go);
    return hip_last("render_finish");
}

}
```

### endosurf_amd/engine.py

```python
from __future__ import annotations

import ctypes as C
import os
from typing import Optional

import torch

from . import _lib
from ._device import f32, mixed_in, u8
from ._lib import check, es_composite_args, es_points, ptr, stream_ptr
from .engine_eval import EvalMixin
from .engine_mesh import MeshMixin
from .engine_trace import TraceMixin
from .engine_track import TrackMixin


class PointCtx:
    _OUT = {"xc": (_lib.WS_XC, 3), "v": (_lib.WS_V, 3), "sdf": (_lib.WS_SDF, 1), "feat": (_lib.WS_FEAT, 256),
            "gc": (_lib.WS_GC, 3), "go": (_lib.WS_GO, 3), "rgb": (_lib.WS_RGB, 3), "curv": (_lib.WS_CURV, 3), "xcbar": (_lib.WS_XCBAR, 3),
            "tbar": (_lib.WS_TBAR, 1), "vbar": (_lib.WS_VBAR, 3)}

    def __init__(self, eng: "Engine", pts, flags: int, m_color: int = 0):
        self.eng, self.pts, self.flags, self.M, self.m_color = eng, pts, flags, pts.M, int(m_color)
        self.x3_chain, self.px3 = False, None
# ... 42 lines not shown
        self._timing_on, self._ssim_window = False, None

    def st(self):
        if torch.cuda.current_device() != self.device.index:
            raise _lib.EndoSurfHipError(
                f"engine for {self.device} used while the current device is cuda:{torch.cuda.current_device()}; "
                f"wrap the call in torch.cuda.device({self.device.index})")
        return stream_ptr(self.device)

    def wg_scratch(self):
        if not self.deterministic:
            return None
        if self._wg_scratch is None:
            self._wg_scratch = self.empty(int(self.lib.es_wgrad_scratch_floats()))
        return self._wg_scratch

    def empty(self, *shape, dtype=torch.float32):
        return torch.empty(*shape, device=self.device, dtype=dtype)

    def zeros(self, *shape, dtype=torch.float32):
        if self._arena_on and dtype == torch.float32:
            shp = tuple(shape[0]) if len(shape) == 1 and isinstance(shape[0], (tuple, list, torch.Size)) else tuple(shape)
            n = 1
            for s in shp:
                n *= int(s)
            off = self._arena_off
            if 0 < n and off + n <= self._arena.numel():
                self._arena_off = off + (n + 63) // 64 * 64
                return self._arena[off:off + n].view(shp)
        return torch.zeros(*shape, device=self.device, dtype=dtype)

    def arena_begin(self, extra_floats: int = 0):
        need = self.n_weff + self.n_param + 4096 + int(extra_floats) + 64 * 32
        need = (need + 4095) // 4096 * 4096
        if self._arena is None or self._arena.numel() < need:
            if torch.cuda.is_current_stream_capturing():
                raise _lib.EndoSurfHipError("the step arena must exist before a step is captured (run one eager step first)")
            self._arena = self.empty(need)
        self.zero(self._arena)
        self._arena_off, self._arena_on = 0, True
        self._rng_step_calls = 0

    def arena_end(self):
        self._arena_on = False

    @property
    def ones1(self) -> torch.Tensor:
        if self._ones1 is None:
            self._ones1 = torch.ones(1, device=self.device)
        return self._ones1

    def uniform(self, n: int, step_dev: Optional[torch.Tensor] = None) -> torch.Tensor:
        out = self.empty(int(n))
        seed = int(torch.initial_seed()) & 0xFFFFFFFFFFFFFFFF
        if step_dev is not None:
            sub = (1 << 63) + (self._rng_step_calls << 40)
            self._rng_step_calls += 1
        else:
            sub = self._rng_calls
            self._rng_calls += 1
        check(self.lib.es_uniform(ptr(out), int(n), seed, sub, ptr(step_dev) if step_dev is not None else None, self.st()), "es_uniform")
        return out

    def weightnorm_pack(self, flat_params: torch.Tensor, use_deform: bool):
        weff = self.empty(self.n_weff)
        packed = self.empty(self.n_packed)
        if not use_deform:
            self.zero(weff)
        check(self.lib.es_weightnorm_pack(ptr(flat_params), ptr(weff), ptr(packed), int(use_deform), self.st()), "es_weightnorm_pack")
        return weff, packed

    def weightnorm_backward_layers(self, flat_params, dweff, dparams, first_layer: int, n_layers: int):
        check(self.lib.es_weightnorm_backward_layers(ptr(flat_params), ptr(dweff), ptr(dparams), int(first_layer), int(n_layers), self.st()),
              "es_weightnorm_backward_layers")

    def weightnorm_backward(self, flat_params, dweff, use_deform: bool):
        dparams = self.zeros(self.n_param)
        check(self.lib.es_weightnorm_backward(ptr(flat_params), ptr(dweff), ptr(dparams), int(use_deform), self.st()),
              "es_weightnorm_backward")
        return dparams

    @staticmethod
    def points(x=None, t=None, dirs=None, rays=None, z=None, n_per_ray=1, ldz=None, M=None) -> es_points:
        for name, v in (("x", x), ("t", t), ("dirs", dirs), ("rays", rays), ("z", z)):
            if torch.is_tensor(v) and not v.is_cuda:
                raise ValueError(f"Engine.points: {name} is on {v.device}; a point source takes device tensors only "
                                 f"(move it with .to(device) first)")
        p = es_points()
        if rays is not None:
            p.rays, p.z = ptr(rays), ptr(z)
            p.n_per_ray = int(n_per_ray)
            p.ldz = int(ldz if ldz is not None else z.shape[-1])
            n_ray_pts = rays.shape[0] * n_per_ray
            if x is not None:
                p.mode, p.M_split = 2, n_ray_pts
                p.x, p.t = ptr(x), ptr(t)
                p.t_scalar = 0
                p.M = n_ray_pts + x.shape[0]
            else:
                p.mode = 1
                p.M = int(M if M is not None else n_ray_pts)
            p._keep = (rays, z, x, t)
        else:
            p.mode = 0
            p.x, p.t = ptr(x), ptr(t)
            p.dirs = ptr(dirs) if dirs is not None else None
            p.t_scalar = 1 if t.numel() == 1 and x.shape[0] != 1 else 0
            p.n_per_ray, p.ldz = 1, 1
            p.M = int(M if M is not None else x.shape[0])
            p._keep = (x, t, dirs)
        return p

    def packed_x3(self, weff, use_deform: bool):
        if self._x3 is None or self._x3["ptr"] != weff.data_ptr():
            self._x3 = {"ptr": weff.data_ptr(), "src": weff.detach(), "packs": {}}
        packs = self._x3["packs"]
        cur = torch.cuda.current_stream(self.device)
        e = packs.get(bool(use_deform))
        if e is None:
            buf = torch.empty(int(self.lib.es_packed_x3_bytes()), device=self.device, dtype=torch.uint8)
            check(self.lib.es_pack_x3(ptr(weff), ptr(buf), int(use_deform), self.st()), "es_pack_x3")
            ev = torch.cuda.Event()
            ev.record(cur)
            e = packs[bool(use_deform)] = (buf, ev, cur)
        elif e[2] != cur:
            cur.wait_event(e[1])
            if not torch.cuda.is_current_stream_capturing():
                e[0].record_stream(cur)
        return e[0]

    def x3_buffers(self):
        return [] if self._x3 is None else [self._x3["src"]] + [e[0] for e in self._x3["packs"].values()]

    def _use_x3(self, M: int) -> bool:
        return self.split_precision and M >= self.x3_query_min

    def query_sdf(self, pts: es_points, weff, packed, use_deform: bool, tile_points: int = 0) -> torch.Tensor:
        out = self.empty(pts.M)
        if self._use_x3(pts.M):
            check(self.lib.es_query_sdf_x3(C.byref(pts), ptr(self.packed_x3(weff, use_deform)), ptr(weff), ptr(out), 0, None, int(use_deform),
                                           self.st()), "es_query_sdf_x3")
            return out
        if tile_points:
            check(self.lib.es_query_sdf_tiles(C.byref(pts), ptr(packed), ptr(weff), ptr(out), int(use_deform), int(tile_points), self.st()),
                  "es_query_sdf_tiles")
            return out
        check(self.lib.es_query_sdf(C.byref(pts), ptr(packed), ptr(weff), ptr(out), int(use_deform), self.st()), "es_query_sdf")
        return out

    def ray_setup(self, rays, u, n, sample_dist, lin_mode, z, want_bounds=False):
        N = rays.shape[0]
        near = self.empty(N) if want_bounds else None
        far = self.empty(N) if want_bounds else None
        check(self.lib.es_ray_setup(ptr(rays), ptr(u) if u is not None else None, N, n, float(sample_dist), lin_mode, ptr(z),
                                    z.shape[1], ptr(near), ptr(far), self.st()), "es_ray_setup")
        return near, far

    def sample_z(self, rays, u_perturb, weff, packed, use_deform, n_samples, n_importance, up_sample_steps, upsample: bool,
                 trace: Optional[list] = None, racing: bool = False):
        N = rays.shape[0]
        n = n_samples
        sample_dist = 2.0 / n_samples
        do_up = upsample and n_importance > 0 and up_sample_steps > 0
        n_imp = n_importance // up_sample_steps if do_up else 0
        if do_up and n_imp == 0:
            raise ValueError(f"n_importance = {n_importance} gives no new sample in any of the {up_sample_steps} up-sampling steps")
        S = n + up_sample_steps * n_imp
        if do_up and not racing and trace is None and N > 0 and n_importance % up_sample_steps == 0 and not self._use_x3(N * n):
            z_out = self.empty(N, S)
            scratch = self.empty(int(self.lib.es_sample_scratch_floats(N, n_samples, n_importance, up_sample_steps)))
            check(self.lib.es_sample_z(ptr(rays), ptr(u_perturb) if u_perturb is not None else None, N, n_samples, n_importance, up_sample_steps, 1,
                                       ptr(packed), ptr(weff), int(use_deform), ptr(z_out), ptr(scratch), self.st()), "es_sample_z")
            return z_out
        zc = self.empty(N, S)
        self.ray_setup(rays, u_perturb, n, sample_dist, 0, zc)
        if trace is not None:
            trace.append(zc[:, :n].clone())
        if not do_up:
            return zc
        zn = self.empty(N, S)
        sdf_c = self.query_sdf(self.points(rays=rays, z=zc, n_per_ray=n, ldz=S), weff, packed, use_deform,
                               tile_points=_lib.QUERY_TILE_RACING if racing and N * n > 16384 else 0).view(N, n)
        ld_sdf = n
        sdf_a, sdf_b = self.empty(N, S), self.empty(N, S)
        src = self.empty(N, S, dtype=torch.int32)
        z_new = self.empty(N, n_imp)
        for i in range(up_sample_steps):
            self.upsample_step(rays, zc, S, sdf_c, ld_sdf, N, n, n_imp, 64 * 2 ** i, z_new, zn, S, src)
            if i + 1 != up_sample_steps:
                sdf_new = self.query_sdf(self.points(rays=rays, z=z_new, n_per_ray=n_imp, ldz=n_imp), weff, packed, use_deform)
                dst = sdf_a if sdf_c.data_ptr() != sdf_a.data_ptr() else sdf_b
                self.merge_sdf(sdf_c, ld_sdf, sdf_new, n_imp, src, S, N, n, dst)
                sdf_c, ld_sdf = dst, S
            zc, zn = zn, zc
            n += n_imp
            if trace is not None:
                trace.append(zc[:, :n].clone())
        return zc

    def mid_z(self, z, sample_dist):
        N, S = z.shape
        mid = self.empty(N, S)
        check(self.lib.es_mid_z(ptr(z), S, N, S, float(sample_dist), ptr(mid), self.st()), "es_mid_z")
        return mid

    def composite_args(self, rays, z, sdf, g_o, rgb, variance, sample_dist, cos_anneal) -> es_composite_args:
        a = es_composite_args()
        N, S = z.shape
        a.rays, a.z, a.ldz = ptr(rays), ptr(z), S
        a.sdf, a.g_o, a.rgb, a.variance = ptr(sdf), ptr(g_o), ptr(rgb), ptr(variance)
        a.N, a.S, a.sample_dist = N, S, float(sample_dist)
        if torch.is_tensor(cos_anneal):
            a.cos_anneal, a.cos_anneal_dev = 0.0, ptr(cos_anneal)
        else:
            a.cos_anneal, a.cos_anneal_dev = float(cos_anneal), None
        a._keep = [rays, z, sdf, g_o, rgb, variance, cos_anneal]
        if self.deterministic:
            part = self.empty(N, 2)
            a.ray_part = ptr(part)
            a._keep.append(part)
        return a

    def composite_forward(self, a: es_composite_args, eik_acc=None, go_copy: bool = False):
        N, S = a.N, a.S
        out = dict(color=self.empty(N, 3), depth=self.empty(N, 1), weights=self.empty(N, S), cdf=self.empty(N, S),
                   weight_max=self.empty(N, 1), eik_acc=eik_acc if eik_acc is not None else self.zeros(2),
                   wmax_idx=self.empty(N, dtype=torch.int32))
        for k, v in out.items():
            setattr(a, k, ptr(v))
        if go_copy:
            out["go"] = self.empty(N, S, 3)
            a.go_copy = ptr(out["go"])
        a._keep.append(out)
        check(self.lib.es_composite_forward(C.byref(a), self.st()), "es_composite_forward")
        return out

    def composite_backward(self, a: es_composite_args, g_color, g_depth, g_eik, eik_den, g_weights=None, g_cdf=None, g_wmax=None,
                           g_gradients_o=None, d_invs_acc=None, n_aux: int = 0, g_aux_sdf=None, g_aux_go=None):
        N, S = a.N, a.S
        out = dict(d_sdf=self.empty(N * S + n_aux), d_go=self.empty(N * S + n_aux, 3), d_rgb=self.empty(N * S, 3),
                   d_invs_acc=d_invs_acc if d_invs_acc is not None else self.zeros(1))
        keep = [g_color, g_depth, g_eik, eik_den, g_weights, g_cdf, g_wmax, g_gradients_o, g_aux_sdf, g_aux_go]
        a.n_aux = int(n_aux)
        a.g_aux_sdf = ptr(g_aux_sdf) if (n_aux and g_aux_sdf is not None) else None
        a.g_aux_go = ptr(g_aux_go) if (n_aux and g_aux_go is not None) else None
        a.g_color, a.g_depth, a.g_eik, a.eik_den = ptr(g_color), ptr(g_depth), ptr(g_eik), ptr(eik_den)
        a.g_weights = ptr(g_weights) if g_weights is not None else None
        a.g_cdf = ptr(g_cdf) if g_cdf is not None else None
        a.g_wmax = ptr(g_wmax) if g_wmax is not None else None
        a.g_gradients_o = ptr(g_gradients_o) if g_gradients_o is not None else None
        for k, v in out.items():
            setattr(a, k, ptr(v))
        a._keep += keep + [out]
        check(self.lib.es_composite_backward(C.byref(a), self.st()), "es_composite_backward")
        return out

    def variance_terms(self, variance, d_invs_acc=None):
        out = self.empty(1)
        v = f32(variance).reshape(1)
        if d_invs_acc is None:
            check(self.lib.es_variance_terms(ptr(v), None, ptr(out), None, self.st()), "es_variance_terms")
        else:
            check(self.lib.es_variance_terms(ptr(v), ptr(d_invs_acc), None, ptr(out), self.st()), "es_variance_terms")
        return out

    def march_begin(self, rays, weff, packed, use_deform, n_steps=128, tau=0.0):
        N = rays.shape[0]
        dprop = self.empty(N, n_steps)
        self.ray_setup(rays, None, n_steps, 0.0, 1, dprop)
        B = self.march_block
        if B and n_steps % B == 0 and n_steps > B and N * B >= 16384:
            sdf = self.zeros(N, n_steps)
            done = self.empty(N, dtype=torch.int32)
            for b in range(n_steps // B):
                p = self.points(rays=rays, z=dprop, n_per_ray=B, ldz=n_steps)
                p.z = C.c_void_p(dprop.data_ptr() + 4 * b * B)
                if self._use_x3(p.M):
                    check(self.lib.es_query_sdf_x3(C.byref(p), ptr(self.packed_x3(weff, use_deform)), ptr(weff),
                                                   C.c_void_p(sdf.data_ptr() + 4 * b * B), n_steps, ptr(done) if b else None, int(use_deform),
                                                   self.st()), "es_query_sdf_x3")
                else:
                    check(self.lib.es_query_sdf_rays(C.byref(p), ptr(packed), ptr(weff), C.c_void_p(sdf.data_ptr() + 4 * b * B), n_steps,
                                                     ptr(done) if b else None, int(use_deform), self.st()), "es_query_sdf_rays")
                if b + 1 < n_steps // B:
                    check(self.lib.es_march_progress(ptr(sdf), N, n_steps, (b + 1) * B, float(tau), ptr(done), self.st()), "es_march_progress")
        else:
            sdf = self.query_sdf(self.points(rays=rays, z=dprop, n_per_ray=n_steps, ldz=n_steps), weff, packed, use_deform)
        state = self.empty(N, 4)
        flags = self.empty(N, dtype=torch.int32)
        d_pred = self.empty(N)
        check(self.lib.es_march_find(ptr(sdf), ptr(dprop), N, n_steps, float(tau), ptr(state), ptr(flags), ptr(d_pred), self.st()),
              "es_march_find")
        return dict(rays=rays, weff=weff, packed=packed, use_deform=use_deform, tau=float(tau), state=state, flags=flags, d_pred=d_pred,
                    keep=(dprop, sdf))

    def march_refine(self, ms, n_secant_steps=8):
        rays, N = ms["rays"], ms["rays"].shape[0]
        x = self.empty(N, 3)
        t = self.empty(N)
        for _ in range(n_secant_steps):
            self.secant_points(rays, ms["d_pred"], N, x, t)
            f_mid = self.query_sdf(self.points(x=x, t=t), ms["weff"], ms["packed"], ms["use_deform"])
            self.secant_update(f_mid, N, ms["tau"], ms["state"], ms["d_pred"])
        d_out = self.empty(N, 1)
        check(self.lib.es_march_finish(ptr(ms["d_pred"]), ptr(ms["flags"]), N, ptr(d_out), self.st()), "es_march_finish")
        return d_out

    def ray_marching(self, rays, weff, packed, use_deform, n_steps=128, n_secant_steps=8, tau=0.0):
        N = rays.shape[0]
        B = self.march_block
        blocks = bool(B and n_steps % B == 0 and n_steps > B and N * B >= 16384)
        if N > 0 and not self._use_x3(N * (B if blocks else n_steps)):
            d_out = self.empty(N, 1)
            scratch = self.empty(int(self.lib.es_march_scratch_floats(N, n_steps)))
            check(self.lib.es_ray_marching(ptr(rays), N, int(n_steps), int(n_secant_steps), float(tau), int(B) if blocks else 0, ptr(packed), ptr(weff),
                                           int(use_deform), ptr(d_out), ptr(scratch), self.st()), "es_ray_marching")
            return d_out
        return self.march_refine(self.march_begin(rays, weff, packed, use_deform, n_steps, tau), n_secant_steps)

    def point_forward(self, pts, weff, packed, flags: int, m_color: int = 0, fp32_only: bool = False) -> PointCtx:
        ctx = PointCtx(self, pts, flags, m_color)
        save = bool(flags & _lib.PF_SAVE)
# ... 134 lines not shown
```

### endosurf_amd/functions.py

```python
from __future__ import annotations

import torch

from . import _lib
from .engine import Engine, PointCtx, f32, u8

class _PackFn(torch.autograd.Function):

    @staticmethod
    def forward(ctx, model_ref, eng: Engine, *plist):
        model = model_ref()
        weff, packed = eng.weightnorm_pack(model._flat, model.use_deform)
        ctx.model_ref, ctx.eng, ctx.flat, ctx.use_deform = model_ref, eng, model._flat, model.use_deform
        ctx.slots = [(model._layout[key][0], p.numel(), tuple(p.shape)) for key, p in model.ordered_params()]
        ctx.mark_non_differentiable(packed)
        ctx.set_materialize_grads(False)
        return weff, packed

    @staticmethod
    def backward(ctx, dweff, _dpacked):
        model = ctx.model_ref()
        if model is not None:
            model._pack_cache = None
        if dweff is None:
            return (None, None, *[None for _ in ctx.slots])
        pipe = getattr(ctx.eng, "_grad_pipeline", None)
        if pipe is not None and pipe.get("dflat") is not None and pipe.get("dweff_ptr") == dweff.data_ptr() and pipe.get("buffers") == 1:
            pipe["adopted"] = True
            dflat = pipe["dflat"]
            for first, n in pipe["remaining"]:
                ctx.eng.weightnorm_backward_layers(ctx.flat, dweff, dflat, first, n)
        else:
            dflat = ctx.eng.weightnorm_backward(ctx.flat, dweff.contiguous(), ctx.use_deform)
        if model is not None:
            model._flat_grad = dflat
        return (None, None, *[dflat[off:off + n].view(shape) for off, n, shape in ctx.slots])


class _SValFn(torch.autograd.Function):

    @staticmethod
    def forward(ctx, variance, eng: Engine):
        s = eng.variance_terms(variance.detach())
        ctx.save_for_backward(s)
        ctx.shape = variance.shape
        return s.reshape(variance.shape)

    @staticmethod
    def backward(ctx, g):
        s, = ctx.saved_tensors
        inside = ((s > 1e-6) & (s < 1e6)).to(s.dtype)
        return (g.reshape(1) * -10.0 * s * inside).reshape(ctx.shape), None


class _PointEvalFn(torch.autograd.Function):

    @staticmethod
    def forward(ctx, weff, packed, eng: Engine, pts, flags: int, x_in=None):
        pctx = eng.point_forward(pts, weff, packed, flags, fp32_only=x_in is not None)
        ctx.pctx, ctx.eng, ctx.weff, ctx.packed = pctx, eng, weff, packed
        ctx.pts, ctx.flags = pts, flags
        ctx.set_materialize_grads(False)
        ctx.wrt_x = x_in is not None
        ctx.x_shape = tuple(x_in.shape) if x_in is not None else None
        ctx.x_dtype = x_in.dtype if x_in is not None else None
        outs = [pctx.view("sdf").clone(), pctx.view("go").clone()]
        if flags & _lib.PF_COLOR:
            outs.append(pctx.view("rgb").clone())
        return tuple(outs)

    @staticmethod
    def backward(ctx, d_sdf, d_go, d_rgb=None):
        eng, pctx = ctx.eng, ctx.pctx
        if not (ctx.flags & _lib.PF_SAVE):
            raise RuntimeError("point evaluation was run without PF_SAVE; cannot backpropagate")
        if ctx.wrt_x and d_go is None and d_rgb is None and not ctx.needs_input_grad[0]:
            return None, None, None, None, None, torch.zeros(ctx.x_shape, device=eng.device, dtype=ctx.x_dtype)
        if pctx is None:
            with torch.no_grad():
                pctx = eng.point_forward(ctx.pts, ctx.weff.detach(), ctx.packed, ctx.flags, fp32_only=ctx.wrt_x)
        dweff = eng.point_backward(pctx, ctx.weff, ctx.packed, d_sdf, d_go, d_rgb)
        xbar = None
        if ctx.wrt_x and ctx.needs_input_grad[5]:
            if d_go is None:
                xbar = torch.zeros(ctx.x_shape, device=eng.device, dtype=ctx.x_dtype)
            else:
                xbar = eng.point_input_adjoint(pctx, ctx.weff, ctx.packed, d_sdf, d_go).reshape(ctx.x_shape).to(ctx.x_dtype)
        ctx.pctx = None
        return dweff, None, None, None, None, xbar


class _NetForwardFn(torch.autograd.Function):

    @staticmethod
    def forward(ctx, weff, packed, eng: Engine, inputs, flags: int):
        inp = inputs.detach().to(torch.float32).reshape(-1, 7)
        x, d, t = inp[:, :3].contiguous(), inp[:, 3:6].contiguous(), inp[:, 6].contiguous()
        pts = eng.points(x=x, t=t, dirs=d)
        pctx = eng.point_forward(pts, weff, packed, flags, fp32_only=True)
        ctx.pctx, ctx.eng, ctx.weff, ctx.packed, ctx.pts, ctx.flags, ctx.d = pctx, eng, weff, packed, pts, flags, d
        ctx.in_shape, ctx.in_dtype = tuple(inputs.shape), inputs.dtype
        ctx.set_materialize_grads(False)
        return pctx.view("sdf").clone(), pctx.view("rgb").clone()

    @staticmethod
# ... 67 lines not shown
            raise ValueError("surface_neighbour_error expects the gradients of N surface points followed by their N neighbours")
        v8 = u8(valid)
        out = eng.empty(2)
        eng.sn_loss(g_, v8, N, out)
        ctx.eng, ctx.saved, ctx.n, ctx.shape = eng, (g_, v8, out), N, tuple(g.shape)
        ctx.set_materialize_grads(False)
        return out[0]

    @staticmethod
    def backward(ctx, g_loss):
        if g_loss is None:
            return None, None, None
        eng, N = ctx.eng, ctx.n
        g_, v8, out = ctx.saved
        gl = g_loss.detach().to(torch.float32).reshape(1)
        d_g = eng.empty(2 * N, 3)
        eng.sn_loss_backward(g_, v8, out, gl, N, d_g)
        return d_g.view(ctx.shape), None, None


class _RenderFn(torch.autograd.Function):

    @staticmethod
    def forward(ctx, weff, packed, variance, eng: Engine, rays, z, sample_dist: float, cos_anneal: float, flags: int, aux_x, aux_t,
                chunk_rays: int, tail=None):
        N, S = z.shape
        P_ = N * S
        ctx.tail = None
        ctx.set_materialize_grads(False)
        var1 = variance.detach().reshape(1)
        ctx.eng, ctx.weff, ctx.packed, ctx.variance = eng, weff, packed, variance
        ctx.geom = (rays, z, float(sample_dist), cos_anneal if torch.is_tensor(cos_anneal) else float(cos_anneal))
        ctx.flags = flags
        if (flags & _lib.PF_SAVE) and 0 < chunk_rays < N:
            ctx.chunk_rays, ctx.pctx, ctx.n_aux = int(chunk_rays), None, 0
            outs = {k: [] for k in ("color", "depth", "weights", "weight_max", "cdf", "wmax_idx", "go")}
            eik_acc = eng.zeros(2)
            for i in range(0, N, chunk_rays):
                r_, z_ = rays[i:i + chunk_rays], z[i:i + chunk_rays]
                n_ = r_.shape[0]
                mid = eng.mid_z(z_, sample_dist)
                pctx = eng.point_forward(eng.points(rays=r_, z=mid, n_per_ray=S, ldz=S), weff, packed, flags | _lib.PF_COLOR)
                a = eng.composite_args(r_, z_, pctx.view("sdf").view(-1), pctx.view("go"), pctx.view("rgb"), var1, sample_dist, cos_anneal)
                out = eng.composite_forward(a, eik_acc=eik_acc)
                for k in ("color", "depth", "weights", "weight_max", "cdf", "wmax_idx"):
                    outs[k].append(out[k])
                outs["go"].append(pctx.view("go")[:n_ * S].view(n_, S, 3).clone())
            cat = {k: torch.cat(v, 0) for k, v in outs.items()}
            ctx.eik_den = (eik_acc[1] + 1e-6).reshape(1)
            eik = eik_acc[0] / ctx.eik_den[0]
            den_out = ctx.eik_den.clone()
            ctx.mark_non_differentiable(cat["wmax_idx"], den_out)
            return (cat["color"], cat["depth"], cat["go"], eik, cat["weights"], cat["weight_max"], cat["cdf"], cat["wmax_idx"],
                    eng.zeros(0, 1), eng.zeros(0, 3), den_out, eng.empty(1))
        ctx.chunk_rays = 0
        mid = eng.mid_z(z, sample_dist)
        fused = aux_x is not None and aux_x.shape[0] > 0 and P_ % 64 == 0
        if tail is not None and not fused and (flags & _lib.PF_SAVE) and P_ % 64 == 0 and P_ > 0:
            pts = eng.points(rays=rays, z=mid, n_per_ray=S, ldz=S, x=tail.aux_x, t=tail.aux_t)
            pctx = PointCtx(eng, pts, flags | _lib.PF_COLOR, m_color=P_)
            eng.point_forward_rows(pctx, weff, packed, 0, P_)
            tail.open(pctx, weff, flags)
            ctx.tail = tail
        else:
            pts = eng.points(rays=rays, z=mid, n_per_ray=S, ldz=S, x=aux_x if fused else None, t=aux_t if fused else None)
            pctx = eng.point_forward(pts, weff, packed, flags | _lib.PF_COLOR, m_color=P_ if fused else 0)
        sdf_all, go_all = pctx.view("sdf"), pctx.view("go")
        a = eng.composite_args(rays, z, sdf_all.view(-1), go_all, pctx.view("rgb"), var1, sample_dist, cos_anneal)
        out = eng.composite_forward(a, go_copy=True)
        n_aux = aux_x.shape[0] if fused else 0
        eik, den2 = eng.empty(1), eng.empty(2)
        aux_sdf, aux_go = eng.empty(n_aux, 1), eng.empty(n_aux, 3)
        eng.render_finish(out["eik_acc"], sdf_all[P_:] if n_aux else None, go_all[P_:] if n_aux else None, n_aux, eik, den2,
                          aux_sdf if n_aux else None, aux_go if n_aux else None)
        eik_den, den_out = den2[0:1], den2[1:2]
        ctx.pctx, ctx.eik_den = pctx, eik_den
        ctx.n_aux = n_aux
        ctx.mark_non_differentiable(out["wmax_idx"], den_out)
        return (out["color"], out["depth"], out["go"], eik.reshape(()), out["weights"], out["weight_max"], out["cdf"], out["wmax_idx"], aux_sdf,
                aux_go, den_out, eng.empty(1))

    @staticmethod
    def backward(ctx, g_color, g_depth, g_go, g_eik, g_weights, g_wmax, g_cdf, _, g_aux_sdf, g_aux_go, _g_den=None, _g_token=None):
        eng = ctx.eng
        tail = ctx.tail
        if tail is not None:
            tail.finish(eng, ctx.weff, ctx.packed)
            ctx.n_aux, g_aux_sdf, g_aux_go = tail.cap, tail.g_sdf, tail.g_go
            if ctx.pctx is None:
                rays_, zs_, sd_, _ = ctx.geom
                mid = eng.mid_z(zs_, sd_)
                pts = eng.points(rays=rays_, z=mid, n_per_ray=zs_.shape[1], ldz=zs_.shape[1], x=tail.aux_x, t=tail.aux_t)
                ctx.pctx = eng.point_forward(pts, ctx.weff, ctx.packed, ctx.flags | _lib.PF_COLOR, m_color=zs_.numel(), fp32_only=True)
        if not (ctx.flags & _lib.PF_SAVE):
            raise RuntimeError("render was run without saved activations; cannot backpropagate")
        rays, zs, sample_dist, cos_anneal = ctx.geom
        N, S = zs.shape
        var = ctx.variance.detach()
        var1 = var.reshape(1)
        z = lambda g, *shape: (g.contiguous() if g is not None else eng.zeros(*shape))
        opt = lambda g: g.contiguous() if g is not None else None
        g_color, g_depth, g_eik = z(g_color, N, 3), z(g_depth, N, 1).view(-1), z(g_eik, 1).reshape(1)
        g_weights, g_cdf, g_go = opt(g_weights), opt(g_cdf), opt(g_go)
        g_wmax = g_wmax.contiguous().view(-1) if g_wmax is not None else None
        sl = lambda g, i, j: g[i:j] if g is not None else None
        d_invs_acc = eng.zeros(1)
        dweff = eng.zeros(eng.n_weff) if N == 0 else None
        C = max(1, ctx.chunk_rays if ctx.chunk_rays else N)
        for i in range(0, N, C):
            j = min(i + C, N)
            if ctx.chunk_rays:
                r_, z_ = rays[i:j], zs[i:j]
                mid = eng.mid_z(z_, sample_dist)
                pctx = eng.point_forward(eng.points(rays=r_, z=mid, n_per_ray=S, ldz=S), ctx.weff, ctx.packed, ctx.flags | _lib.PF_COLOR)
            else:
                r_, z_, pctx = rays, zs, ctx.pctx
            a = eng.composite_args(r_, z_, pctx.view("sdf").view(-1), pctx.view("go"), pctx.view("rgb"), var1, sample_dist, cos_anneal)
            bw = eng.composite_backward(a, g_color[i:j], g_depth[i:j], g_eik, ctx.eik_den, g_weights=sl(g_weights, i, j), g_cdf=sl(g_cdf, i, j),
                                        g_wmax=sl(g_wmax, i, j), g_gradients_o=sl(g_go, i, j), d_invs_acc=d_invs_acc, n_aux=ctx.n_aux,
                                        g_aux_sdf=opt(g_aux_sdf), g_aux_go=opt(g_aux_go))
            d_sdf, d_go = bw["d_sdf"].view(-1, 1), bw["d_go"]
            dweff = eng.point_backward(pctx, ctx.weff, ctx.packed, d_sdf, d_go, bw["d_rgb"], dweff=dweff, staged=not ctx.chunk_rays)
            del pctx
        dvar = eng.variance_terms(var, d_invs_acc=d_invs_acc).reshape(ctx.variance.shape)
        ctx.pctx = None
        if tail is not None:
            tail.close(eng)
        return dweff, None, dvar, None, None, None, None, None, None, None, None, None, None
```

### endosurf_amd/renderer.py

```python
from __future__ import annotations

import os
import weakref

import numpy as np
import torch
import torch.nn as nn

from . import _lib
from ._device import _on_device, mixed_in
from .engine import Engine, f32
from .functions import _EodLossFn, _PackFn, _PointEvalFn, _RenderFn, _SnLossFn, _SValFn
from .model import EndoSurfNet, WNLinear, _check_arch, _reference_style_init
from .renderer_mesh import RendererMeshMixin
from .renderer_trace import RendererTraceMixin
from .renderer_track import RendererTrackMixin
from .tail import _Lazy, _LazyEodFn, _PendingEod, _Tail, _TailEvalFn


@mixed_in(RendererTraceMixin)
@mixed_in(RendererTrackMixin)
class EndoSurfRenderer(RendererMeshMixin, nn.Module):

    def __init__(self, render_cfg, net_cfg, device="cuda"):
# ... 127 lines not shown
        if g is None or g["key"] != key:
            slots[skey] = dict(key=key, graph=None)
            while len(slots) > 3:
                slots.pop(next(iter(slots)))
            return None
        slots[skey] = g
        cos = self.get_cos_anneal_ratio(iter_step)
        if g["graph"] is False:
            return None
        if g["graph"] is None:
            static_in = eng.empty(*rays.shape)
            static_in.copy_(self._rays32(rays))
            cos_dev = torch.full((1,), float(cos), device=self.device)
            kw = dict(kwargs, perturb_overwrite=perturb)
            graph = torch.cuda.CUDAGraph()
            self._cos_anneal_dev = cos_dev
            try:
                with torch.cuda.graph(graph):
                    ret = self.render_rays(static_in, **kw)
                    names = sorted(ret)
                    flat = torch.cat([ret[k].reshape(-1) for k in names])
            except Exception as e:
                g["graph"] = False
                import warnings
                warnings.warn(f"endosurf_amd: capturing the no-grad forward failed ({type(e).__name__}: {e}); it stays eager for this shape",
                              RuntimeWarning, stacklevel=3)
                return None
            finally:
                self._cos_anneal_dev = None
            g.update(graph=graph, static_in=static_in, cos_dev=cos_dev, cos=float(cos), flat=flat,
                     layout=[(k, tuple(ret[k].shape), ret[k].numel()) for k in names],
                     keep=(self._weights(), eng.x3_buffers()))
        g["static_in"].copy_(rays if rays.dtype == torch.float32 else rays.to(torch.float32))
        if float(cos) != g["cos"]:
            g["cos_dev"].fill_(float(cos))
            g["cos"] = float(cos)
        g["graph"].replay()
        flat = g["flat"].clone()
        out, off = {}, 0
        for k, shape, n in g["layout"]:
            out[k] = flat[off:off + n].view(shape)
            off += n
        return out

    @property
    def _fwd_graph(self):
        slots = self.__dict__.get("_fwd_graphs")
        return slots[next(reversed(slots))] if slots else None

    def release_forward_graphs(self):
        self.__dict__.pop("_fwd_graphs", None)

    @_on_device
    def sample_z(self, rays, iter_step=0, perturb_overwrite=None, u_perturb=None, racing=False):
        rays = self._rays32(rays)
        weff, packed = self._weights()
        perturb = self.perturb if perturb_overwrite is None else perturb_overwrite
        u = None
        if perturb:
            u = u_perturb if u_perturb is not None else torch.rand([rays.shape[0], 1], device=self.device)
            u = f32(u).reshape(-1)
        upsample = iter_step >= self.important_begin_iter and self.n_importance > 0
        with torch.no_grad():
            return self.engine.sample_z(rays, u, weff.detach(), packed, self.use_deform, self.n_samples, self.n_importance,
                                        self.up_sample_steps, upsample, racing=racing)

    def _rays_from(self, rays_o, rays_d, time=None):
        n = rays_o.shape[0]
        t = time.reshape(n, 1) if time is not None else torch.zeros(n, 1, device=self.device)
        return f32(torch.cat([rays_o, rays_d, torch.zeros(n, 2, device=self.device), t], -1))

    @_on_device
    def up_sample(self, rays_o, rays_d, z_vals, sdf, n_importance, inv_s):
        N, n = z_vals.shape
        eng = self.engine
        rays = self._rays_from(rays_o, rays_d)
        z = f32(z_vals)
        sd = f32(sdf).reshape(N, n)
        S = n + int(n_importance)
        z_new, z_out, src = eng.empty(N, int(n_importance)), eng.empty(N, S), eng.empty(N, S, dtype=torch.int32)
        eng.upsample_step(rays, z, n, sd, n, N, n, int(n_importance), inv_s, z_new, z_out, S, src)
        return z_new

    @_on_device
    def cat_z_vals(self, rays_o, rays_d, time, z_vals, new_z_vals, sdf, last=False):
        N, n = z_vals.shape
        m = new_z_vals.shape[1]
        eng = self.engine
        z_new = f32(new_z_vals)
        z_cat = torch.cat([z_vals.detach().to(torch.float32), z_new], dim=-1)
        z_sorted, index = torch.sort(z_cat, dim=-1, stable=True)
        if last:
            return z_sorted, sdf
        rays = self._rays_from(rays_o, rays_d, time)
        weff, packed = self._weights()
        with torch.no_grad():
            sdf_new = eng.query_sdf(eng.points(rays=rays, z=z_new, n_per_ray=m, ldz=m), weff.detach(), packed, self.use_deform)
        sd = f32(sdf).reshape(N, n)
        src = index.to(torch.int32).contiguous()
        out = eng.empty(N, n + m)
        eng.merge_sdf(sd, n, sdf_new, m, src, n + m, N, n, out)
        return z_sorted, out

    @_on_device
    def secant(self, f_low, f_high, d_low, d_high, n_secant_steps, rays, tau, max_points=64000):
        M = rays.shape[0]
        eng = self.engine
        if M == 0:
            return torch.zeros(0, device=self.device)
        rays32 = self._rays32(rays)
        weff, packed = self._weights()
        f = lambda a: a.detach().to(torch.float32).reshape(M)
        state = torch.stack([f(d_low), f(f_low), f(d_high), f(f_high)], -1).contiguous()
        d_pred = (-state[:, 1] * (state[:, 2] - state[:, 0]) / (state[:, 3] - state[:, 1]) + state[:, 0]).contiguous()
        x, t = eng.empty(M, 3), eng.empty(M)
        with torch.no_grad():
            for _ in range(int(n_secant_steps)):
                eng.secant_points(rays32, d_pred, M, x, t)
                f_mid = eng.query_sdf(eng.points(x=x, t=t), weff.detach(), packed, self.use_deform)
                eng.secant_update(f_mid, M, tau, state, d_pred)
            for k, dst in enumerate((d_low, f_low, d_high, f_high)):
                dst.copy_(state[:, k].reshape(dst.shape).to(dst.dtype))
        return d_pred

    @_on_device
    def render_rays(self, rays, iter_step=0, perturb_overwrite=None, eval=False, u_perturb=None, aux_points=None, z_vals=None, **kwargs):
        rays = self._rays32(rays)
        n_rays = rays.shape[0]
        weff, packed = self._weights()
        z = z_vals if z_vals is not None else self.sample_z(rays, iter_step, perturb_overwrite, u_perturb)
        sample_dist = 2.0 / self.n_samples
        ret = self.render_core(rays[:, :3], rays[:, 3:6], rays[:, 8], z, sample_dist,
                               cos_anneal_ratio=self._cos_anneal(iter_step), eval=eval, _rays=rays, _aux=aux_points)
        n_samples = z.shape[1]
        extra = {"aux_sdf": ret["aux_sdf"], "aux_gradients_o": ret["aux_gradients_o"], "eik_den": ret["eik_den"]} if aux_points is not None else {}
        return {
            **extra,
            "color_map": ret["color_map"],
            "depth_map": ret["depth_map"],
            "gradients_o": ret["gradients_o"],
            "gradient_o_error": ret["gradient_o_error"],
            "weights": ret["weights"],
            "weight_max": ret["weight_max"],
            "cdf": ret["cdf"],
            "s_val": ret["s_val"].reshape(1, 1).expand(n_rays, 1),
        }

    @_on_device
    def render_core(self, rays_o, rays_d, time, z_vals, sample_dist, cos_anneal_ratio=0.0, eval=False, _rays=None, _aux=None):
        if _rays is None:
            n = rays_o.shape[0]
            _rays = torch.cat([rays_o, rays_d, torch.zeros(n, 2, device=self.device), time.reshape(n, 1)], -1).to(torch.float32).contiguous()
        weff, packed = self._weights()
        var = self.model.deviation_network.variance
        z = f32(z_vals)
        aux_x = aux_t = None
        if _aux is not None:
            aux_x = f32(_aux[0])
            aux_t = f32(_aux[1]).reshape(-1)
        flags = self._flags(weff)
        chunk = self._chunk_rays(z.shape[0], z.shape[1], flags)
        tail = self._new_tail(z.numel(), flags, chunk, z.shape[0]) if _aux is None else None
        color, depth, g_o, eik, weights, wmax, cdf, _, aux_sdf, aux_go, eik_den, token = _RenderFn.apply(
            weff, packed, var, self.engine, _rays, z, float(sample_dist), cos_anneal_ratio if torch.is_tensor(cos_anneal_ratio) else float(cos_anneal_ratio), flags, aux_x, aux_t,
            chunk, tail)
        self._live_tail = (tail, token) if (tail is not None and tail.pctx is not None) else None
        if _aux is not None and aux_sdf.shape[0] != aux_x.shape[0]:
            aux_sdf, aux_go = self._point_eval(aux_x, aux_t)
        s_val = _SValFn.apply(var, self.engine)
        return {"color_map": color, "depth_map": depth, "gradients_o": g_o, "gradient_o_error": eik, "cdf": cdf,
                "weights": weights, "weight_max": wmax, "s_val": s_val, "aux_sdf": aux_sdf, "aux_gradients_o": aux_go, "eik_den": eik_den}

    def _point_eval(self, x, t, dirs=None, canonical=False, x_in=None):
        weff, packed = self._weights()
        flags = self._flags(weff)
        if (flags & _lib.PF_SAVE) and not canonical and x_in is None and dirs is None:
            xx, tt = x.detach().to(torch.float32).reshape(-1, 3), t.detach().to(torch.float32).reshape(-1)
            m = xx.shape[0]
            self._aux_demand = (self._aux_demand or 0) + _Tail.rows64(m)
            slot = self._tail_peek(m, weff, flags)
            if slot is not None and tt.numel() == m:
                eng = self.engine
                tail, token = self._live_tail
                if xx.data_ptr() != slot.x.data_ptr():
                    eng.copy2(slot.x, xx.contiguous(), 3 * m, slot.t, tt.contiguous(), m)
                off = tail.claim(m)
                tail.evaluate(eng, off, m, weff, packed)
                return _TailEvalFn.apply(token, tail, eng, off, m)
        pts = self.engine.points(x=f32(x), t=f32(t).reshape(-1), dirs=dirs)
        if canonical:
            flags &= ~_lib.PF_DEFORM
        if x_in is not None:
            sdf, g_o = _PointEvalFn.apply(weff, packed, self.engine, pts, flags | _lib.PF_SAVE, x_in)
        else:
            sdf, g_o = _PointEvalFn.apply(weff, packed, self.engine, pts, flags)
        return sdf, g_o

    def _new_tail(self, P_: int, flags: int, chunk: int, n_rays: int = 0):
        if not (flags & _lib.PF_SAVE):
            return None
        if self.__dict__.get("_fwd_graphs"):
            self.release_forward_graphs()
        demand = self._aux_demand if self._aux_demand is not None else _Tail.rows64(n_rays) + _Tail.rows64(2 * n_rays)
        self._aux_demand = 0
        eng = self.engine
        if demand <= 0 or chunk or P_ <= 0 or P_ % 64 or eng.split_precision or torch.cuda.is_current_stream_capturing():
            return None
        demand = min(demand, max(P_ // 4, 4096) // 64 * 64)
        if demand <= 0:
            return None
        cap = demand + (-(P_ + demand)) % 128
        self.tails_made = getattr(self, "tails_made", 0) + 1
        return _Tail(eng, P_, cap)

    def _tail_peek(self, m: int, weff, flags: int):
        live = self._live_tail
        if live is None or m == 0 or not torch.is_grad_enabled():
            return None
        return live[0].peek(m, weff, flags)

    def _aux_buffers(self, m: int):
        weff, _ = self._weights()
# ... 8 lines not shown
        rays = self._rays32(rays)
        N = rays.shape[0]
        weff, packed = self._weights()
        flags = self._flags(weff)
        slot = None
        if (bool(self.render_cfg.get("defer_errorondepth", True)) and (flags & _lib.PF_SAVE) and N > 0 and torch.is_grad_enabled()
                and not torch.cuda.is_current_stream_capturing()):
            slot = self._tail_peek(N, weff, flags)
        if slot is None:
            pts, time, inside = self._eod_points(rays, d_gt, mask)
            sdf, gradient_o = self._point_eval(pts, time)
            return self._eod_loss(rays, pts, mask, sdf, gradient_o)
        tail, token = self._live_tail
        self._aux_demand = (self._aux_demand or 0) + _Tail.rows64(N)
        tail.force_pending()
        inside = self._eod_points(rays, d_gt, mask, into=(slot.x, slot.t))[2]
        pend = _PendingEod(self.engine, tail, tail.claim(N), N, rays, f32(mask).reshape(-1), weff, packed)
        tail.defer(pend)
        a, b = _LazyEodFn.apply(token, pend)
        return _Lazy.wrap(a, pend), _Lazy.wrap(b, pend), inside

    def _eod_points(self, rays, d_gt, mask=None, into=None):
        N = rays.shape[0]
        x, t = into if into is not None else self._aux_buffers(N)
        d = f32(d_gt).reshape(-1)
        if d.numel() != N:
            raise ValueError("errorondepth expects one ground-truth depth per ray")
        inside = m = None
        if mask is not None:
            m = f32(mask).reshape(-1)
            if m.numel() != N:
                raise ValueError("errorondepth expects one mask value per ray")
            inside = self.engine.empty(N, 1)
        self.engine.eod_points(rays, d, m, N, x, t, inside)
        return (x, t, inside) if mask is not None else (x, t)

    def _eod_loss(self, rays, pts, mask, sdf, gradient_o):
        return _EodLossFn.apply(sdf, gradient_o, self.engine, rays, pts, mask)

    @_on_device
    def ray_marching(self, rays, tau=0.0, n_steps=(128, 129), n_secant_steps=8, max_points=64000):
        rays = self._rays32(rays)
        weff, packed = self._weights()
        with torch.no_grad():
            return self.engine.ray_marching(rays, weff.detach(), packed, self.use_deform, int(n_steps[0]), n_secant_steps, tau)

    @_on_device
    def surface_neighbour_error(self, rays, mask, iter_step=0, neighbour_rad=0.05, u_neigh=None):
        rays = self._rays32(rays)
        pp, tt, valid = self._sn_points(rays, mask, neighbour_rad, u_neigh)
        _, g = self._point_eval(pp, tt)
        return self._sn_loss(g, valid)

    def _march_begin(self, rays):
        weff, packed = self._weights()
        with torch.no_grad():
            return self.engine.march_begin(self._rays32(rays), weff.detach(), packed, self.use_deform)

    def _march_refine(self, ms):
        with torch.no_grad():
            return self.engine.march_refine(ms)

    def _sn_points(self, rays, mask, neighbour_rad, u_neigh=None, d_i=None):
        N = rays.shape[0]
        eng = self.engine
        x, t = self._aux_buffers(2 * N)
        with torch.no_grad():
            if d_i is None:
                d_i = self.ray_marching(rays)
            if u_neigh is not None:
                u = f32(u_neigh)
            elif torch.cuda.is_current_stream_capturing():
                u = torch.rand(N, 3, device=self.device)
            else:
                u = eng.uniform(3 * N).view(N, 3)
            m = f32(mask).reshape(-1)
            if m.numel() != N:
                raise ValueError("surface_neighbour_error expects one mask value per ray")
            valid = eng.empty(N, dtype=torch.bool)
            eng.sn_points(rays, m, f32(d_i).reshape(-1), u, neighbour_rad, N, x, t, valid)
            return x, t, valid

    def _train_aux_points(self, rays, depth_gt, mask, d_i, neighbour_rad, u_neigh=None):
        N = rays.shape[0]
        u = f32(u_neigh) if u_neigh is not None else torch.rand(N, 3, device=self.device)
        x, t = self.engine.empty(3 * N, 3), self.engine.empty(3 * N)
        valid = self.engine.empty(N, dtype=torch.bool)
        self.engine.train_aux_points(rays, f32(depth_gt), f32(mask), f32(d_i), u, neighbour_rad, N, x, t, valid)
        return x, t, valid

    def _sn_loss(self, g, valid):
        return _SnLossFn.apply(g, self.engine, valid)

    @_on_device
    def render_frames(self, rays, iter_step=0, ray_chunk=2048, perturb_overwrite=None, use_graph=True):
        flat = self._rays32(rays.reshape(-1, rays.shape[-1]))
        n = flat.shape[0]
        C = int(ray_chunk)
        out = {"color": self.engine.empty(n, 3), "depth": self.engine.empty(n, 1), "normal": self.engine.empty(n, 3)}
        if n == 0:
            return out

        def chunk_forward(r):
            ret = self.render_rays(r, iter_step=iter_step, perturb_overwrite=perturb_overwrite)
            normal = (ret["gradients_o"] * ret["weights"][:, :, None]).sum(dim=1)
            return ret["color_map"], ret["depth_map"], normal

        with torch.no_grad():
            weff, _ = self._weights()
            if not use_graph:
# ... 113 lines not shown
```

### endosurf_amd/trainer.py

```python
from __future__ import annotations

import math
from typing import Dict, Optional

import numpy as np
import torch

from . import _lib
from .engine import f32, u8

LOSS_WEIGHTS = dict(color=1.0, depth=1.0, sdf=1.0, angle=0.1, eikonal=0.1, surf_neig=0.1)


def compute_loss(renderer, batch: Dict[str, torch.Tensor], iter_step: int, weights=LOSS_WEIGHTS, surf_neig_rad: float = 0.1,
                 u_perturb=None, u_neigh=None):
    rays, color_gt, depth_gt = batch["rays"], batch["color"], batch["depth"]
    mask_gt, cmask = batch["mask"], batch["color_mask"]
    ret = renderer(rays, iter_step=iter_step, u_perturb=u_perturb)
    color_error = (ret["color_map"] - color_gt) * cmask
    color_loss = color_error.abs().sum() / (cmask.sum() + 1e-10)
    sdf_loss, angle_loss, valid = renderer.errorondepth(rays, d_gt=depth_gt, mask=mask_gt, iter_step=iter_step)
    depth_error = (ret["depth_map"] - depth_gt) * valid * mask_gt
    depth_loss = depth_error.abs().sum() / ((valid * mask_gt).sum() + 1e-10)
    eik = ret["gradient_o_error"]
    sn = renderer.surface_neighbour_error(rays=rays, mask=mask_gt, iter_step=iter_step, neighbour_rad=surf_neig_rad, u_neigh=u_neigh)
    total = (color_loss * weights["color"] + depth_loss * weights["depth"] + sdf_loss * weights["sdf"]
             + angle_loss * weights["angle"] + eik * weights["eikonal"] + weights["surf_neig"] * sn)
    terms = dict(color=color_loss, depth=depth_loss, sdf=sdf_loss, angle=angle_loss, eikonal=eik, surf_neig=sn)
    return total, terms, ret


def compute_loss_fused(renderer, batch: Dict[str, torch.Tensor], iter_step: int, weights=LOSS_WEIGHTS, surf_neig_rad: float = 0.1,
                       u_perturb=None, u_neigh=None, loss_kernel: bool = True, exact: bool = False, group=None):
    rays = renderer._rays32(batch["rays"])
    color_gt, depth_gt, mask_gt, cmask = batch["color"], batch["depth"], batch["mask"], batch["color_mask"]
    N = rays.shape[0]
    eng = renderer.engine
    need_p, need_n = renderer.perturb and u_perturb is None, u_neigh is None
    if need_p or need_n:
        u4 = eng.uniform(4 * N, renderer._rng_step_dev)
        if need_p:
            u_perturb = u4[:N]
        if need_n:
            u_neigh = u4[N:].view(N, 3)
    renderer._weights()
    main = torch.cuda.current_stream(rays.device)
    side = renderer._side_stream
    if side is None:
        side = renderer._side_stream = torch.cuda.Stream(device=rays.device)
    ms = renderer._march_begin(rays)
    side.wait_stream(main)
    with torch.cuda.stream(side):
        z = renderer.sample_z(rays, iter_step, u_perturb=u_perturb, racing=True)
    d_i = renderer._march_refine(ms)
    aux_x, aux_t, valid_sn = renderer._train_aux_points(rays, depth_gt, mask_gt, d_i, surf_neig_rad, u_neigh)
    eod_pts = aux_x[:N]
    main.wait_stream(side)
    if not torch.cuda.is_current_stream_capturing():
        z.record_stream(main)
    ret = renderer(rays, iter_step=iter_step, aux_points=(aux_x, aux_t), z_vals=z)
    a_sdf, a_go = ret["aux_sdf"], ret["aux_gradients_o"]
    if loss_kernel:
        eik = ret["gradient_o_error"]
        exact_args = None
        if exact:
            import torch.distributed as dist
            world = dist.get_world_size(group) if dist.is_initialized() else 1
            den = renderer.engine.empty(5)
            _LossFn.sums(renderer.engine, rays, eod_pts, mask_gt, cmask, valid_sn, den)
            den_local_eik = ret["eik_den"]
            den[4:5].copy_(den_local_eik - 1e-6)
            if world > 1:
                dist.all_reduce(den, group=group)
            eik = eik * (float(world) * den_local_eik[0] / (den[4] + 1e-6))
            exact_args = (den, float(world))
        total, t = _LossFn.apply(ret["color_map"], ret["depth_map"], eik, a_sdf, a_go, renderer.engine, rays, eod_pts,
                                 color_gt, depth_gt, mask_gt, cmask, valid_sn, weights, exact_args)
        return total, dict(color=t[0], depth=t[1], sdf=t[2], angle=t[3], eikonal=t[4], surf_neig=t[5]), ret
    color_loss = ((ret["color_map"] - color_gt) * cmask).abs().sum() / (cmask.sum() + 1e-10)
    sdf_loss, angle_loss, valid = renderer._eod_loss(rays, eod_pts, mask_gt, a_sdf[:N], a_go[:N])
    depth_loss = ((ret["depth_map"] - depth_gt) * valid * mask_gt).abs().sum() / ((valid * mask_gt).sum() + 1e-10)
    eik = ret["gradient_o_error"]
    sn = renderer._sn_loss(a_go[N:], valid_sn)
    total = (color_loss * weights["color"] + depth_loss * weights["depth"] + sdf_loss * weights["sdf"]
             + angle_loss * weights["angle"] + eik * weights["eikonal"] + weights["surf_neig"] * sn)
    terms = dict(color=color_loss, depth=depth_loss, sdf=sdf_loss, angle=angle_loss, eikonal=eik, surf_neig=sn)
    return total, terms, ret


class _LossFn(torch.autograd.Function):

    @staticmethod
    def sums(eng, rays, eod_pts, mask, cmask, valid_sn, out):
        N = rays.shape[0]
        keep = [f32(rays), f32(eod_pts), f32(mask), f32(cmask), u8(valid_sn)]
        z3, z1 = eng.zeros(3 * N, 3), eng.zeros(3 * N, 1)
        a = _lib.es_loss_args()
        for name, t in zip(("rays", "eod_pts", "mask", "cmask", "valid_sn"), keep):
            setattr(a, name, _lib.ptr(t))
        for name, t in (("color_map", z3), ("color_gt", z3), ("depth_map", z1), ("depth_gt", z1), ("aux_sdf", z1), ("aux_go", z3), ("eik", z1)):
            setattr(a, name, _lib.ptr(t))
        a.N = N
        a.den_out = _lib.ptr(out)
        eng.train_loss(a)

    @staticmethod
# ... 461 lines not shown
```

### include/endosurf_hip.h

```cpp
#ifndef ENDOSURF_HIP_H
#define ENDOSURF_HIP_H

#include <stddef.h>
#include <stdint.h>

#ifdef __cplusplus
extern "C" {
#endif

#define ES_ABI_VERSION 14

int es_abi_version(void);
const char* es_last_error(void);
int es_init(void);

int64_t es_param_floats(void);
int es_param_layout(int net, int layer, int64_t* bias_off, int64_t* g_off, int64_t* v_off, int* out_dim, int* in_dim);
int64_t es_param_variance_off(void);
int64_t es_weff_floats(void);
int es_weff_layout(int net, int layer, int64_t* w_off, int64_t* b_off);
int64_t es_packed_floats(void);

int es_weightnorm_pack(const float* params, float* weff, float* packed, int use_deform, void* stream);
int es_weightnorm_backward(const float* params, const float* dweff, float* dparams, int use_deform, void* stream);
int es_weightnorm_backward_layers(const float* params, const float* dweff, float* dparams, int first_layer, int n_layers, void* stream);

typedef struct es_points {
    const float* x;
    const float* t;
    const float* dirs;
    const float* rays;
    const float* z;
    int mode, t_scalar, n_per_ray, ldz;
    int M;
    int M_split;
} es_points;

int es_query_sdf(const es_points* pts, const float* packed, const float* weff, float* sdf_out, int use_deform, void* stream);
#define ES_QUERY_TILE_RACING 32
int es_query_sdf_tiles(const es_points* pts, const float* packed, const float* weff, float* sdf_out, int use_deform, int tile_points,
                       void* stream);
int es_query_sdf_rays(const es_points* pts, const float* packed, const float* weff, float* sdf_out, int ld_out, const int* ray_done,
                      int use_deform, void* stream);
int es_march_progress(const float* sdf, int N, int n, int n_valid, float tau, int* done, void* stream);

int es_deform_forward(const es_points* pts, const float* packed, const float* weff, float* xc_out, float* d_out, void* stream);
int es_deform_inverse(const es_points* pts, const float* init, const float* packed, const float* weff, int max_iters, float tol, float* y_out,
                      float* step_out, int* iters_out, void* stream);

int es_deform_jacobian(const es_points* pts, const float* packed, const float* weff, float* jac_out, float* xc_out, void* stream);
int es_strain_rows(const float* jac_from, const float* jac_to, const float* normals, int M, float* F_out, float* det_out, float* stretch_out,
                   float* area_out, float* surface_out, unsigned char* valid_out, void* stream);

#define ES_TRACE_HIT 1
#define ES_TRACE_MISS 2
#define ES_TRACE_OCCUPIED 3
#define ES_TRACE_NOT_CONVERGED 4
#define ES_TRACE_MAX_ITERS 1024
int es_trace_surface(const float* rays, int N, float tau, float eps, float relax, float min_step, int max_iters, int tile_points,
                     const float* packed, const float* weff, int use_deform, float* depth_out, int* status_out, int* iters_out,
                     float* residual_out, float* points_out, void* stream);

int64_t es_packed_x3_bytes(void);
int es_pack_x3(const float* weff, void* packed_x3, int use_deform, void* stream);
int es_query_sdf_x3(const es_points* pts, const void* packed_x3, const float* weff, float* sdf_out, int ld_out, const int* ray_done,
                    int use_deform, void* stream);

int es_ray_setup(const float* rays, const float* u, int N, int n, float sample_dist, int lin_mode, float* z, int ldz,
                 float* near_out, float* far_out, void* stream);
int es_upsample_step(const float* rays, const float* z_in, int ld_in, const float* sdf_in, int ld_sdf, int N, int n, int n_imp,
                     float inv_s, float* z_new, float* z_out, int ld_out, int32_t* src_idx, void* stream);
int es_merge_sdf(const float* sdf_in, int ld_in, const float* sdf_new, int n_imp, const int32_t* src_idx, int ld_out, int N, int n,
                 float* sdf_out, void* stream);
int es_mid_z(const float* z, int ldz, int N, int S, float sample_dist, float* mid, void* stream);

typedef struct es_composite_args {
    const float* rays; const float* z; int ldz; const float* sdf; const float* g_o; const float* rgb;
    const float* variance;
    int N, S; float sample_dist, cos_anneal;
    float* color; float* depth; float* weights; float* cdf; float* weight_max; float* eik_acc; int32_t* wmax_idx;
    const float* g_color; const float* g_depth; const float* g_weights ; const float* g_cdf ; const float* g_wmax ;
    const float* g_gradients_o ; const float* g_eik ; const float* eik_den ;
    float* d_sdf; float* d_go; float* d_rgb; float* d_invs_acc;
    float* ray_part;
    const float* cos_anneal_dev;
    float* go_copy;
    const float* g_aux_sdf; const float* g_aux_go; int n_aux;
} es_composite_args;
int es_composite_forward(const es_composite_args* a, void* stream);
int es_composite_backward(const es_composite_args* a, void* stream);
int es_variance_terms(const float* variance, const float* d_invs_acc, float* s_val, float* d_var, void* stream);

int64_t es_sample_scratch_floats(int N, int n_samples, int n_importance, int up_sample_steps);
int es_sample_z(const float* rays, const float* u_perturb, int N, int n_samples, int n_importance, int up_sample_steps, int upsample,
                const float* packed, const float* weff, int use_deform, float* z_out, float* scratch, void* stream);

int64_t es_march_scratch_floats(int N, int n_steps);
int es_ray_marching(const float* rays, int N, int n_steps, int n_secant, float tau, int block, const float* packed, const float* weff,
                    int use_deform, float* d_out, float* scratch, void* stream);

typedef struct es_render_args {
    es_composite_args c;
    float* ws; float* scratch; int flags;
    float* wg_scratch;
    const void* packed_x3;
} es_render_args;
int64_t es_render_scratch_floats(int N, int S);
int es_render_forward(const es_render_args* a, const float* packed, const float* weff, void* stream);
int es_render_backward(const es_render_args* a, const float* packed, const float* weff, float* dweff, void* stream);

int es_march_find(const float* sdf, const float* dprop, int N, int n, float tau, float* state, int32_t* flags, float* d_pred, void* stream);
int es_secant_points(const float* rays, const float* d_pred, int N, float* x, float* t, void* stream);
int es_secant_update(const float* sdf_mid, int N, float tau, float* state, float* d_pred, void* stream);
int es_march_finish(const float* d_pred, const int32_t* flags, int N, float* d_out, void* stream);

#define ES_PF_DEFORM 1
#define ES_PF_COLOR 2
#define ES_PF_SAVE 4
#define ES_PF_X3 8
#define ES_PF_X3_CHAIN 32
enum { ES_WS_XC = 0, ES_WS_V = 1, ES_WS_SDF = 2, ES_WS_FEAT = 3, ES_WS_GC = 4, ES_WS_GO = 5, ES_WS_RGB = 6,
       ES_WS_XCBAR = 27,
       ES_WS_VBAR = 23,
       ES_WS_TBAR = 35,
       ES_WS_CURV = 34 };
int64_t es_point_workspace_floats(int M, int flags);
int64_t es_point_workspace_offset(int M, int flags, int buffer_id);
int es_point_forward(const es_points* pts, const float* packed, const float* weff, float* ws, int flags, int m_color, void* stream);
int es_point_forward_rows(const es_points* pts, const float* packed, const float* weff, float* ws, int flags, int m_color, int row0, int nrows,
                          void* stream);
int es_point_vjp(const es_points* pts, const float* packed, const float* weff, float* ws, int flags, void* stream);
int es_color_forward(const es_points* pts, const float* packed, const float* weff, float* ws, void* stream);
int es_point_forward_x3(const es_points* pts, const float* packed, const void* packed_x3, const float* weff, float* ws, int flags, int m_color,
                        void* stream);
int es_gemm_atb(const float* X, const float* dA, int M, float* out, int split_precision, float* wg_scratch, void* stream);
int es_point_backward_x3(const es_points* pts, const float* packed, const void* packed_x3, const float* weff, float* ws, int flags, int m_color,
                         const float* d_sdf, const float* d_go, const float* d_rgb, float* dweff, float* wg_scratch, void* stream);
int es_point_backward(const es_points* pts, const float* packed, const float* weff, float* ws, int flags, int m_color,
                      const float* d_sdf, const float* d_go, const float* d_rgb, float* dweff, void* stream);

#define ES_BWD_CHAINS 1
#define ES_BWD_WGRAD_DEFORM 2
#define ES_BWD_WGRAD_SDF 4
// ... 138 lines not shown
```

Before: 72970.

## Fuse small launches: step setup, upsample+merge, composite tails, pack kernels

```diff
diff --git a/endosurf_amd/_lib.py b/endosurf_amd/_lib.py
--- a/endosurf_amd/_lib.py
+++ b/endosurf_amd/_lib.py
@@ -66,9 +66,13 @@
     "es_ray_setup": (_I, [_P, _P, _I, _I, _F, _I, _P, _I, _P, _P, _P]),
     "es_upsample_step": (_I, [_P, _P, _I, _P, _I, _I, _I, _I, _F, _P, _P, _I, _P, _P]),
     "es_merge_sdf": (_I, [_P, _I, _P, _I, _P, _I, _I, _I, _P, _P]),
+    "es_upsample_merge_step": (_I, [_P, _P, _I, _P, _I, _I, _P, _I, _P, _I, _P, _I, _I, _F, _P, _P, _I, _P, _P]),
+    "es_step_setup": (_I, [_P, _I, C.c_ulonglong, C.c_ulonglong, _P, _P, _I, _P, _I, _F, _P, _I, _P]),
     "es_mid_z": (_I, [_P, _I, _I, _I, _F, _P, _P]),
     "es_composite_forward": (_I, [C.POINTER(es_composite_args), _P]),
     "es_composite_backward": (_I, [C.POINTER(es_composite_args), _P]),
+    "es_composite_forward_finish": (_I, [C.POINTER(es_composite_args), _P, _P, _P, _I, _P, _P, _P, _P, _P, _P]),
+    "es_composite_backward_finish": (_I, [C.POINTER(es_composite_args), _P, _P, _P]),
     "es_march_find": (_I, [_P, _P, _I, _I, _F, _P, _P, _P, _P]),
     "es_secant_points": (_I, [_P, _P, _I, _P, _P, _P]),
     "es_secant_update": (_I, [_P, _I, _F, _P, _P, _P]),
diff --git a/endosurf_amd/csrc/api.hip b/endosurf_amd/csrc/api.hip
--- a/endosurf_amd/csrc/api.hip
+++ b/endosurf_amd/csrc/api.hip
@@ -219,6 +219,21 @@
     ES_REQUIRE(sdf_in && sdf_new && src_idx && sdf_out && sdf_out != sdf_in, "es_merge_sdf arguments (out must not alias in)");
     return merge_sdf(sdf_in, ld_in, sdf_new, n_imp, src_idx, ld_out, N, n, sdf_out, (hipStream_t)stream);
 }
+int es_upsample_merge_step(const float* rays, const float* z_in, int ld_in, const float* sdf_old, int ld_old, int n_old, const float* sdf_new,
+                           int n_new, const int32_t* src_prev, int ld_src, float* sdf_out, int N, int n_imp, float inv_s, float* z_new,
+                           float* z_out, int ld_out, int32_t* src_idx, void* stream) {
+    if (N == 0) return ST_OK;
+    ES_REQUIRE(rays && z_in && sdf_old && sdf_new && src_prev && z_new && z_out && src_idx && N >= 0, "es_upsample_merge_step arguments");
+    ES_REQUIRE(sdf_out != sdf_old && sdf_out != sdf_new, "es_upsample_merge_step: sdf_out must not alias an input row");
+    return upsample_merge_step(rays, z_in, ld_in, sdf_old, ld_old, n_old, sdf_new, n_new, src_prev, ld_src, sdf_out, N, n_imp, inv_s, z_new, z_out,
+                               ld_out, src_idx, (hipStream_t)stream);
+}
+int es_step_setup(const float* rays, int N, unsigned long long seed, unsigned long long subsequence, const double* subsequence_dev, float* u4,
+                  int n_march, float* dprop, int n_samples, float sample_dist, float* z, int ldz, void* stream) {
+    if (N == 0) return ST_OK;
+    ES_REQUIRE(rays && u4 && dprop && z && N >= 0 && n_march >= 1 && n_samples >= 1 && ldz >= n_samples, "es_step_setup arguments");
+    return step_setup(rays, N, seed, subsequence, subsequence_dev, u4, n_march, dprop, n_samples, sample_dist, z, ldz, (hipStream_t)stream);
+}
 int es_mid_z(const float* z, int ldz, int N, int S, float sample_dist, float* mid, void* stream) {
     if (N == 0) return ST_OK;
     ES_REQUIRE(z && mid && ldz >= S && S >= 1, "es_mid_z arguments");
@@ -237,6 +252,25 @@
     ES_REQUIRE(a->g_color && a->g_depth && a->g_eik && a->eik_den && a->d_sdf && a->d_go && a->d_rgb && a->d_invs_acc,
                "es_composite_backward adjoints");
     return composite(as_comp(a), 1, (hipStream_t)stream);
+}
+int es_composite_forward_finish(const es_composite_args* a, int32_t* counter, const float* aux_sdf_ws, const float* aux_go_ws, int n_aux, float* eik,
+                                float* eik_den, float* aux_sdf, float* aux_go, float* s_val, void* stream) {
+    ES_REQUIRE(a && a->N > 0, "es_composite_forward_finish needs rays (an empty batch: es_composite_forward + es_render_finish)");
+    ES_REQUIRE(a->rays && a->z && a->sdf && a->g_o && a->rgb && a->variance, "es_composite_forward_finish inputs");
+    ES_REQUIRE(a->color && a->depth && a->weights && a->cdf && a->weight_max && a->eik_acc && a->wmax_idx, "es_composite_forward_finish outputs");
+    ES_REQUIRE(counter && eik && eik_den && n_aux >= 0 && (n_aux == 0 || (aux_sdf_ws && aux_go_ws && aux_sdf && aux_go)), "es_composite_forward_finish epilogue");
+    const CompositeTail t{counter, aux_sdf_ws, aux_go_ws, n_aux, eik, eik_den, aux_sdf, aux_go, s_val, nullptr};
+    return composite(as_comp(a), 0, (hipStream_t)stream, &t);
+}
+int es_composite_backward_finish(const es_composite_args* a, int32_t* counter, float* d_var, void* stream) {
+    ES_REQUIRE(a && a->N > 0, "es_composite_backward_finish needs rays (an empty batch: es_composite_backward + es_variance_terms)");
+    ES_REQUIRE(a->rays && a->z && a->sdf && a->g_o && a->rgb && a->variance, "es_composite_backward_finish inputs");
+    ES_REQUIRE(a->n_aux >= 0, "es_composite_backward_finish: negative n_aux");
+    ES_REQUIRE(a->g_color && a->g_depth && a->g_eik && a->eik_den && a->d_sdf && a->d_go && a->d_rgb && a->d_invs_acc,
+               "es_composite_backward_finish adjoints");
+    ES_REQUIRE(counter && d_var, "es_composite_backward_finish epilogue");
+    const CompositeTail t{counter, nullptr, nullptr, 0, nullptr, nullptr, nullptr, nullptr, nullptr, d_var};
+    return composite(as_comp(a), 1, (hipStream_t)stream, &t);
 }
 int es_march_find(const float* sdf, const float* dprop, int N, int n, float tau, float* state, int32_t* flags, float* d_pred, void* stream) {
     if (N == 0) return ST_OK;
diff --git a/endosurf_amd/csrc/host.h b/endosurf_amd/csrc/host.h
--- a/endosurf_amd/csrc/host.h
+++ b/endosurf_amd/csrc/host.h
@@ -15,6 +15,13 @@
 static_assert(sizeof(CompositeArgs) == sizeof(es_composite_args) && std::is_standard_layout<CompositeArgs>::value, "es::CompositeArgs is es_composite_args");
 static_assert(sizeof(LossArgs) == sizeof(es_loss_args) && std::is_standard_layout<LossArgs>::value, "es::LossArgs is es_loss_args");
 inline const CompositeArgs& as_comp(const es_composite_args* a) { return *reinterpret_cast<const CompositeArgs*>(a); }
+
+struct CompositeTail {
+    int* counter;
+    const float* aux_sdf_ws; const float* aux_go_ws; int n_aux;
+    float* eik; float* eik_den; float* aux_sdf; float* aux_go; float* s_val;
+    float* d_var;
+};
 
 int init_tables();
 int weightnorm_pack(const float* params, float* weff, float* packed, int use_deform, hipStream_t st);
@@ -67,8 +74,13 @@
 int upsample_step(const float* rays, const float* z_in, int ld_in, const float* sdf_in, int ld_sdf, int N, int n, int n_imp,
                   float inv_s, float* z_new, float* z_out, int ld_out, int* src_idx, hipStream_t st);
 int merge_sdf(const float* sdf_in, int ld_in, const float* sdf_new, int n_imp, const int* src_idx, int ld_out, int N, int n, float* sdf_out, hipStream_t st);
+int upsample_merge_step(const float* rays, const float* z_in, int ld_in, const float* sdf_old, int ld_old, int n_old, const float* sdf_new,
+                        int n_new, const int* src_prev, int ld_src, float* sdf_out, int N, int n_imp, float inv_s, float* z_new, float* z_out,
+                        int ld_out, int* src_idx, hipStream_t st);
+int step_setup(const float* rays, int N, unsigned long long seed, unsigned long long subseq, const double* subseq_dev, float* u4, int n_march,
+               float* dprop, int n_samples, float sample_dist, float* z, int ldz, hipStream_t st);
 int mid_z(const float* z, int ldz, int N, int S, float sample_dist, float* mid, hipStream_t st);
-int composite(const CompositeArgs& a, int backward, hipStream_t st);
+int composite(const CompositeArgs& a, int backward, hipStream_t st, const CompositeTail* tail = nullptr);
 int variance_terms(const float* variance, const float* d_invs_acc, float* s_val, float* d_var, hipStream_t st);
 int march_progress(const float* sdf, int N, int n, int n_valid, float tau, int* done, hipStream_t st);
 int march_find(const float* sdf, const float* dprop, int N, int n, float tau, float* state, int* flags, float* d_pred, hipStream_t st);
diff --git a/endosurf_amd/csrc/pack.hip b/endosurf_amd/csrc/pack.hip
--- a/endosurf_amd/csrc/pack.hip
+++ b/endosurf_amd/csrc/pack.hip
@@ -74,9 +74,7 @@
     if (lane == 0) w[(size_t)N * K + n] = pb[n];
 }
 
-__global__ __launch_bounds__(256) void k_pack(const float* __restrict__ weff, float4* __restrict__ packed, int first_net) {
-    const unsigned long long idx = (unsigned long long)blockIdx.x * 256 + threadIdx.x;
-    if (idx >= PACKED_FLOAT4) return;
+__device__ __forceinline__ void pack32_item(const float* __restrict__ weff, float4* __restrict__ packed, int first_net, unsigned long long idx) {
     int s = 0;
 #pragma unroll 1
     for (int i = 1; i < SEG_COUNT; ++i)
@@ -132,9 +130,7 @@
     if (lane == 0) { og[n] = dg; ob[n] = dweff[c_weff_off[li] + (size_t)N * K + n]; }
 }
 
-__global__ __launch_bounds__(256) void k_pack16(const float* __restrict__ weff, float4* __restrict__ packed, int first_net) {
-    const unsigned long long idx = PACKED_FLOAT4 + (unsigned long long)blockIdx.x * 256 + threadIdx.x;
-    if (idx >= PACKED_TOTAL_FLOAT4) return;
+__device__ __forceinline__ void pack16_item(const float* __restrict__ weff, float4* __restrict__ packed, int first_net, unsigned long long idx) {
     int pi = 0;
     unsigned long long base = PACKED_FLOAT4, off = PACKED_FLOAT4;
 #pragma unroll 1
@@ -164,15 +160,20 @@
     packed[idx] = make_float4(o[0], o[1], o[2], o[3]);
 }
 
+__global__ __launch_bounds__(256) void k_pack(const float* __restrict__ weff, float4* __restrict__ packed, int first_net) {
+    const unsigned long long idx = (unsigned long long)blockIdx.x * 256 + threadIdx.x;
+    if (idx >= PACKED_TOTAL_FLOAT4) return;
+    if (idx < PACKED_FLOAT4) pack32_item(weff, packed, first_net, idx);
+    else pack16_item(weff, packed, first_net, idx);
+}
+
 int weightnorm_pack(const float* params, float* weff, float* packed, int use_deform, hipStream_t st) {
     if (int e = init_tables()) return e;
     const int first_layer = use_deform ? 0 : LAYERS;
     dim3 g1(65, NETS * LAYERS - first_layer);
     hipLaunchKernelGGL(k_weff, g1, dim3(256), 0, st, params, weff, first_layer);
-    const unsigned nb = (unsigned)((PACKED_FLOAT4 + 255) / 256);
+    const unsigned nb = (unsigned)((PACKED_TOTAL_FLOAT4 + 255) / 256);
     hipLaunchKernelGGL(k_pack, dim3(nb), dim3(256), 0, st, (const float*)weff, reinterpret_cast<float4*>(packed), use_deform ? 0 : 1);
-    const unsigned nb16 = (unsigned)((PACKED_TOTAL_FLOAT4 - PACKED_FLOAT4 + 255) / 256);
-    hipLaunchKernelGGL(k_pack16, dim3(nb16), dim3(256), 0, st, (const float*)weff, reinterpret_cast<float4*>(packed), use_deform ? 0 : 1);
     return hip_last("weightnorm_pack");
 }
 
diff --git a/endosurf_amd/csrc/philox.h b/endosurf_amd/csrc/philox.h
--- /dev/null
+++ b/endosurf_amd/csrc/philox.h
@@ -0,0 +1,25 @@
+#pragma once
+#include <hip/hip_runtime.h>
+
+#include <cstdint>
+
+namespace es {
+
+__device__ __forceinline__ void philox_round(uint32_t (&c)[4], uint32_t k0, uint32_t k1) {
+    const uint64_t p0 = (uint64_t)0xD2511F53u * c[0], p1 = (uint64_t)0xCD9E8D57u * c[2];
+    const uint32_t n0 = (uint32_t)(p1 >> 32) ^ c[1] ^ k0, n2 = (uint32_t)(p0 >> 32) ^ c[3] ^ k1;
+    c[1] = (uint32_t)p1; c[3] = (uint32_t)p0; c[0] = n0; c[2] = n2;
+}
+__device__ __forceinline__ void philox_uniform4(unsigned long long q, unsigned long long seed, unsigned long long subseq, float (&u)[4]) {
+    uint32_t c[4] = {(uint32_t)q, (uint32_t)(q >> 32), (uint32_t)subseq, (uint32_t)(subseq >> 32)};
+    uint32_t k0 = (uint32_t)seed, k1 = (uint32_t)(seed >> 32);
+#pragma unroll
+    for (int r = 0; r < 10; ++r) {
+        philox_round(c, k0, k1);
+        k0 += 0x9E3779B9u; k1 += 0xBB67AE85u;
+    }
+#pragma unroll
+    for (int j = 0; j < 4; ++j) u[j] = (float)(c[j] >> 8) * (1.f / 16777216.f);
+}
+
+}
diff --git a/endosurf_amd/csrc/rays.hip b/endosurf_amd/csrc/rays.hip
--- a/endosurf_amd/csrc/rays.hip
+++ b/endosurf_amd/csrc/rays.hip
@@ -2,6 +2,8 @@
 
 #include "host.h"
 #include "launch.h"
+#include "philox.h"
+#include "render_tail.h"
 
 namespace es {
 
@@ -61,6 +63,15 @@
     return sqrtf(x * x + y * y + w * w);
 }
 
+__device__ __forceinline__ void ray_setup_row(float near, float far, bool jitter, float shift, int lin_mode, int lane, int n,
+                                              float* __restrict__ zrow) {
+    for (int s = lane; s < n; s += 64) {
+        const float tv = linspace_f32(0.f, 1.f, n, s);
+        float v = lin_mode == 0 ? near + (far - near) * tv : near * (1.f - tv) + far * tv;
+        if (jitter) v = v + shift;
+        zrow[s] = v;
+    }
+}
 __global__ __launch_bounds__(256) void k_ray_setup(const float* __restrict__ rays, const float* __restrict__ u, int N, int n,
                                                    float sample_dist, int lin_mode, float* __restrict__ z, int ldz,
                                                    float* __restrict__ near_out, float* __restrict__ far_out) {
@@ -70,30 +81,34 @@
     float near, far;
     sphere_near_far(g, near, far);
     const float shift = u ? (u[ray] - 0.5f) * sample_dist : 0.f;
-    for (int s = lane; s < n; s += 64) {
-        const float tv = linspace_f32(0.f, 1.f, n, s);
-        float v = lin_mode == 0 ? near + (far - near) * tv : near * (1.f - tv) + far * tv;
-        if (u) v = v + shift;
-        z[(size_t)ray * ldz + s] = v;
-    }
+    ray_setup_row(near, far, u != nullptr, shift, lin_mode, lane, n, z + (size_t)ray * ldz);
     if (lane == 0) { if (near_out) near_out[ray] = near; if (far_out) far_out[ray] = far; }
 }
-
-__global__ __launch_bounds__(256) void k_upsample_step(const float* __restrict__ rays, const float* __restrict__ z_in, int ld_in,
-                                                       const float* __restrict__ sdf_in, int ld_sdf, int N, int n, int n_imp,
-                                                       float inv_s, float* __restrict__ z_new, float* __restrict__ z_out,
-                                                       int ld_out, int* __restrict__ src_idx) {
-    __shared__ float s_z[WAVES_PER_BLOCK][RAY_NMAX], s_a[WAVES_PER_BLOCK][RAY_NMAX], s_c[WAVES_PER_BLOCK][RAY_NMAX + 1],
-        s_new[WAVES_PER_BLOCK][64];
-    const int wv = threadIdx.x >> 6, lane = threadIdx.x & 63;
-    const int ray = blockIdx.x * WAVES_PER_BLOCK + wv;
+__global__ __launch_bounds__(256) void k_step_setup(const float* __restrict__ rays, int N, unsigned long long seed,
+                                                    unsigned long long subseq, const double* __restrict__ subseq_dev,
+                                                    float* __restrict__ u4, int n_march, float* __restrict__ dprop, int n_samples,
+                                                    float sample_dist, float* __restrict__ z, int ldz) {
+    const int ray = blockIdx.x * WAVES_PER_BLOCK + (threadIdx.x >> 6), lane = threadIdx.x & 63;
     if (ray >= N) return;
-    float* zs = s_z[wv]; float* av = s_a[wv]; float* cdf0 = s_c[wv]; float* nz = s_new[wv];
+    if (subseq_dev != nullptr) subseq += (unsigned long long)subseq_dev[0];
+    float q[4], qu[4];
+    philox_uniform4((unsigned long long)ray, seed, subseq, q);
+    philox_uniform4((unsigned long long)(ray >> 2), seed, subseq, qu);
+    if (lane < 4) u4[4 * (size_t)ray + lane] = lane == 0 ? q[0] : (lane == 1 ? q[1] : (lane == 2 ? q[2] : q[3]));
+    const int j = ray & 3;
+    const float u = j == 0 ? qu[0] : (j == 1 ? qu[1] : (j == 2 ? qu[2] : qu[3]));
     const RayGeom g = load_ray(rays, ray);
+    float near, far;
+    sphere_near_far(g, near, far);
+    ray_setup_row(near, far, false, 0.f, 1, lane, n_march, dprop + (size_t)ray * n_march);
+    const float shift = (u - 0.5f) * sample_dist;
+    ray_setup_row(near, far, true, shift, 0, lane, n_samples, z + (size_t)ray * ldz);
+}
+
+__device__ __forceinline__ void upsample_ray(const RayGeom& g, float* zs, float* av, float* cdf0, float* nz, int ray, int lane, int n,
+                                             int n_imp, float inv_s, float* __restrict__ z_new, float* __restrict__ z_out, int ld_out,
+                                             int* src_idx) {
     const int nsec = n - 1;
-
-    for (int e = lane; e < n; e += 64) { zs[e] = z_in[(size_t)ray * ld_in + e]; av[e] = sdf_in[(size_t)ray * ld_sdf + e]; }
-    __builtin_amdgcn_wave_barrier();
     for (int e = lane; e < nsec; e += 64) cdf0[e] = (av[e + 1] - av[e]) / (zs[e + 1] - zs[e] + 1e-6f);
     __builtin_amdgcn_wave_barrier();
     float carry = 1.f, wsum_acc = 0.f;
@@ -174,6 +189,54 @@
     }
 }
 
+__global__ __launch_bounds__(256) void k_upsample_step(const float* __restrict__ rays, const float* __restrict__ z_in, int ld_in,
+                                                       const float* __restrict__ sdf_in, int ld_sdf, int N, int n, int n_imp,
+                                                       float inv_s, float* __restrict__ z_new, float* __restrict__ z_out,
+                                                       int ld_out, int* __restrict__ src_idx) {
+    __shared__ float s_z[WAVES_PER_BLOCK][RAY_NMAX], s_a[WAVES_PER_BLOCK][RAY_NMAX], s_c[WAVES_PER_BLOCK][RAY_NMAX + 1],
+        s_new[WAVES_PER_BLOCK][64];
+    const int wv = threadIdx.x >> 6, lane = threadIdx.x & 63;
+    const int ray = blockIdx.x * WAVES_PER_BLOCK + wv;
+    if (ray >= N) return;
+    float* zs = s_z[wv]; float* av = s_a[wv];
+    const RayGeom g = load_ray(rays, ray);
+    for (int e = lane; e < n; e += 64) { zs[e] = z_in[(size_t)ray * ld_in + e]; av[e] = sdf_in[(size_t)ray * ld_sdf + e]; }
+    __builtin_amdgcn_wave_barrier();
+    upsample_ray(g, zs, av, s_c[wv], s_new[wv], ray, lane, n, n_imp, inv_s, z_new, z_out, ld_out, src_idx);
+}
+
+__device__ __forceinline__ float merged_sdf(const float* __restrict__ sdf_old, int ld_old, int n_old, const float* __restrict__ sdf_new,
+                                            int n_new, int ray, int s) {
+    float v = __builtin_nanf("");
+    if (s >= 0 && s < n_old) v = sdf_old[(size_t)ray * ld_old + s];
+    else if (s >= n_old && s < n_old + n_new) v = sdf_new[(size_t)ray * n_new + (s - n_old)];
+    return v;
+}
+
+__global__ __launch_bounds__(256) void k_upsample_merge_step(const float* __restrict__ rays, const float* __restrict__ z_in, int ld_in,
+                                                             const float* __restrict__ sdf_old, int ld_old, int n_old,
+                                                             const float* __restrict__ sdf_new, int n_new, const int* src_prev,
+                                                             int ld_src, float* __restrict__ sdf_out, int N, int n_imp, float inv_s,
+                                                             float* __restrict__ z_new, float* __restrict__ z_out, int ld_out,
+                                                             int* src_idx) {
+    __shared__ float s_z[WAVES_PER_BLOCK][RAY_NMAX], s_a[WAVES_PER_BLOCK][RAY_NMAX], s_c[WAVES_PER_BLOCK][RAY_NMAX + 1],
+        s_new[WAVES_PER_BLOCK][64];
+    const int wv = threadIdx.x >> 6, lane = threadIdx.x & 63;
+    const int ray = blockIdx.x * WAVES_PER_BLOCK + wv;
+    if (ray >= N) return;
+    float* zs = s_z[wv]; float* av = s_a[wv];
+    const RayGeom g = load_ray(rays, ray);
+    const int n = n_old + n_new;
+    for (int e = lane; e < n; e += 64) {
+        zs[e] = z_in[(size_t)ray * ld_in + e];
+        const float v = merged_sdf(sdf_old, ld_old, n_old, sdf_new, n_new, ray, src_prev[(size_t)ray * ld_src + e]);
+        av[e] = v;
+        if (sdf_out != nullptr) sdf_out[(size_t)ray * ld_out + e] = v;
+    }
+    __builtin_amdgcn_wave_barrier();
+    upsample_ray(g, zs, av, s_c[wv], s_new[wv], ray, lane, n, n_imp, inv_s, z_new, z_out, ld_out, src_idx);
+}
+
 __global__ __launch_bounds__(256) void k_merge_sdf(const float* __restrict__ sdf_in, int ld_in, const float* __restrict__ sdf_new,
                                                    int n_imp, const int* __restrict__ src_idx, int ld_out, int N, int n,
                                                    float* __restrict__ sdf_out) {
@@ -181,10 +244,7 @@
     const int tot = n + n_imp;
     if (i >= N * tot) return;
     const int ray = i / tot, r = i - ray * tot;
-    const int s = src_idx[(size_t)ray * ld_out + r];
-    float v = __builtin_nanf("");
-    if (s >= 0 && s < n) v = sdf_in[(size_t)ray * ld_in + s];
-    else if (s >= n && s < tot) v = sdf_new[(size_t)ray * n_imp + (s - n)];
+    const float v = merged_sdf(sdf_in, ld_in, n, sdf_new, n_imp, ray, src_idx[(size_t)ray * ld_out + r]);
     sdf_out[(size_t)ray * ld_out + r] = v;
 }
 
@@ -202,7 +262,37 @@
 __device__ __forceinline__ float inv_s_from_variance(float var) { return fminf(fmaxf(expf(var * 10.f), 1e-6f), 1e6f); }
 
 template <bool BWD>
-__global__ __launch_bounds__(256) void k_composite(CompositeArgs a) {
+__device__ __forceinline__ void composite_scalars(const CompositeTail& t, const float* __restrict__ variance, float sum0, float sum1) {
+    if (BWD) {
+        t.d_var[0] = d_var_of(expf(variance[0] * 10.f), sum0);
+        return;
+    }
+    finish_eik(sum0, sum1, t.eik, t.eik_den);
+    if (t.s_val != nullptr) t.s_val[0] = s_val_of(expf(variance[0] * 10.f));
+}
+template <bool BWD>
+__device__ __forceinline__ void composite_finish(const float* sums, const float* variance, const CompositeTail& t) {
+    asm volatile("s_waitcnt vmcnt(0)" ::: "memory");
+    __syncthreads();
+    if (threadIdx.x != 0) return;
+    const int ticket = __hip_atomic_fetch_add(t.counter, 1, __ATOMIC_RELAXED, __HIP_MEMORY_SCOPE_AGENT);
+    if (ticket != (int)gridDim.x - 1) return;
+    const float sum0 = __hip_atomic_load(sums, __ATOMIC_RELAXED, __HIP_MEMORY_SCOPE_AGENT);
+    const float sum1 = BWD ? 0.f : __hip_atomic_load(sums + 1, __ATOMIC_RELAXED, __HIP_MEMORY_SCOPE_AGENT);
+    composite_scalars<BWD>(t, variance, sum0, sum1);
+    __hip_atomic_store(t.counter, 0, __ATOMIC_RELAXED, __HIP_MEMORY_SCOPE_AGENT);
+}
+#define ES_COMPOSITE_EXIT                                                                                                   \
+    do {                                                                                                                    \
+        if (t.counter != nullptr && a.ray_part == nullptr) composite_finish<BWD>(BWD ? a.d_invs_acc : a.eik_acc, a.variance, t); \
+        return;                                                                                                             \
+    } while (0)
+
+template <bool BWD>
+__global__ __launch_bounds__(256) void k_composite(CompositeArgs a, CompositeTail t) {
+    if (!BWD && t.counter != nullptr)
+        for (int i = blockIdx.x * 256 + threadIdx.x; i < 3 * t.n_aux; i += gridDim.x * 256)
+            copy_aux_rows(i, t.n_aux, t.aux_sdf_ws, t.aux_go_ws, t.aux_sdf, t.aux_go);
     if (BWD && a.n_aux > 0) {
         const size_t P = (size_t)a.N * a.S;
         for (int i = blockIdx.x * 256 + threadIdx.x; i < a.n_aux; i += gridDim.x * 256) {
@@ -212,7 +302,7 @@
         }
     }
     const int ray = blockIdx.x * WAVES_PER_BLOCK + (threadIdx.x >> 6), lane = threadIdx.x & 63;
-    if (ray >= a.N) return;
+    if (ray >= a.N) ES_COMPOSITE_EXIT;
     const RayGeom g = load_ray(a.rays, ray);
     const float inv_s = inv_s_from_variance(a.variance[0]);
     const float r = a.cos_anneal_dev != nullptr ? a.cos_anneal_dev[0] : a.cos_anneal;
@@ -292,7 +382,7 @@
             if (a.ray_part) { a.ray_part[2 * (size_t)ray] = e_num; a.ray_part[2 * (size_t)ray + 1] = e_den; }
             else { atomicAdd(a.eik_acc + 0, e_num); atomicAdd(a.eik_acc + 1, e_den); }
         }
-        return;
+        ES_COMPOSITE_EXIT;
     }
     const float gc0 = a.g_color[3 * (size_t)ray], gc1 = a.g_color[3 * (size_t)ray + 1], gc2 = a.g_color[3 * (size_t)ray + 2];
     const float gd = a.g_depth[ray];
@@ -349,9 +439,15 @@
         if (a.ray_part) a.ray_part[2 * (size_t)ray] = dinvs;
         else atomicAdd(a.d_invs_acc, dinvs);
     }
-}
-__global__ __launch_bounds__(1024) void k_ray_part_reduce(const float* __restrict__ part, int N, int ncol, float* __restrict__ acc) {
+    ES_COMPOSITE_EXIT;
+}
+#undef ES_COMPOSITE_EXIT
+template <bool BWD>
+__global__ __launch_bounds__(1024) void k_ray_part_reduce(const float* __restrict__ part, int N, float* __restrict__ acc, CompositeTail t,
+                                                          const float* __restrict__ variance) {
+    constexpr int ncol = BWD ? 1 : 2;
     __shared__ float sh[1024];
+    __shared__ float total[2];
     for (int j = 0; j < ncol; ++j) {
         float s = 0.f;
         for (int i = threadIdx.x; i < N; i += 1024) s += part[2 * (size_t)i + j];
@@ -361,9 +457,10 @@
             if ((int)threadIdx.x < o) sh[threadIdx.x] += sh[threadIdx.x + o];
             __syncthreads();
         }
-        if (threadIdx.x == 0) acc[j] += sh[0];
+        if (threadIdx.x == 0) { const float v = acc[j] + sh[0]; acc[j] = v; total[j] = v; }
         __syncthreads();
     }
+    if (t.counter != nullptr && threadIdx.x == 0) composite_scalars<BWD>(t, variance, total[0], BWD ? 0.f : total[1]);
 }
 
 __global__ __launch_bounds__(256) void k_march_find(const float* __restrict__ sdf, const float* __restrict__ dprop, int N, int n,
@@ -480,6 +577,24 @@
                        z_out, ld_out, src_idx);
     return hip_last("upsample_step");
 }
+int upsample_merge_step(const float* rays, const float* z_in, int ld_in, const float* sdf_old, int ld_old, int n_old, const float* sdf_new,
+                        int n_new, const int* src_prev, int ld_src, float* sdf_out, int N, int n_imp, float inv_s, float* z_new, float* z_out,
+                        int ld_out, int* src_idx, hipStream_t st) {
+    const int n = n_old + n_new;
+    ES_REQUIRE(n_old >= 1 && n_new >= 1 && n >= 2 && n <= RAY_NMAX && n_imp >= 1 && n_imp <= 64 && n + n_imp <= ld_out, "upsample_merge_step sizes");
+    ES_REQUIRE(ld_in >= n && ld_old >= n_old && ld_src >= n, "upsample_merge_step row strides");
+    if (N <= 0) return ST_OK;
+    hipLaunchKernelGGL(k_upsample_merge_step, ray_grid(N), dim3(256), 0, st, rays, z_in, ld_in, sdf_old, ld_old, n_old, sdf_new, n_new, src_prev,
+                       ld_src, sdf_out, N, n_imp, inv_s, z_new, z_out, ld_out, src_idx);
+    return hip_last("upsample_merge_step");
+}
+int step_setup(const float* rays, int N, unsigned long long seed, unsigned long long subseq, const double* subseq_dev, float* u4, int n_march,
+               float* dprop, int n_samples, float sample_dist, float* z, int ldz, hipStream_t st) {
+    if (N <= 0) return ST_OK;
+    hipLaunchKernelGGL(k_step_setup, ray_grid(N), dim3(256), 0, st, rays, N, seed, subseq, subseq_dev, u4, n_march, dprop, n_samples,
+                       sample_dist, z, ldz);
+    return hip_last("step_setup");
+}
 int merge_sdf(const float* sdf_in, int ld_in, const float* sdf_new, int n_imp, const int* src_idx, int ld_out, int N, int n,
               float* sdf_out, hipStream_t st) {
     if (N <= 0) return ST_OK;
@@ -492,13 +607,16 @@
     hipLaunchKernelGGL(k_mid_z, dim3((N * S + 255) / 256), dim3(256), 0, st, z, ldz, N, S, sample_dist, mid);
     return hip_last("mid_z");
 }
-int composite(const CompositeArgs& a, int backward, hipStream_t st) {
+int composite(const CompositeArgs& a, int backward, hipStream_t st, const CompositeTail* tail) {
     ES_REQUIRE(a.S >= 1 && a.S <= RAY_NMAX, "composite: samples per ray out of range");
     if (a.N <= 0) return ST_OK;
-    if (backward) hipLaunchKernelGGL(k_composite<true>, ray_grid(a.N), dim3(256), 0, st, a);
-    else hipLaunchKernelGGL(k_composite<false>, ray_grid(a.N), dim3(256), 0, st, a);
-    if (a.ray_part)
-        hipLaunchKernelGGL(k_ray_part_reduce, dim3(1), dim3(1024), 0, st, a.ray_part, a.N, backward ? 1 : 2, backward ? a.d_invs_acc : a.eik_acc);
+    const CompositeTail t = tail != nullptr ? *tail : CompositeTail{};
+    if (backward) hipLaunchKernelGGL(k_composite<true>, ray_grid(a.N), dim3(256), 0, st, a, t);
+    else hipLaunchKernelGGL(k_composite<false>, ray_grid(a.N), dim3(256), 0, st, a, t);
+    if (a.ray_part) {
+        if (backward) hipLaunchKernelGGL(k_ray_part_reduce<true>, dim3(1), dim3(1024), 0, st, a.ray_part, a.N, a.d_invs_acc, t, a.variance);
+        else hipLaunchKernelGGL(k_ray_part_reduce<false>, dim3(1), dim3(1024), 0, st, a.ray_part, a.N, a.eik_acc, t, a.variance);
+    }
     return hip_last("composite");
 }
 int march_find(const float* sdf, const float* dprop, int N, int n, float tau, float* state, int* flags, float* d_pred, hipStream_t st) {
@@ -510,8 +628,8 @@
                                  float* __restrict__ d_var) {
     if (threadIdx.x != 0 || blockIdx.x != 0) return;
     const float e = expf(variance[0] * 10.f);
-    if (s_val) s_val[0] = 1.f / fminf(fmaxf(e, 1e-6f), 1e6f);
-    if (d_var) d_var[0] = (e >= 1e-6f && e <= 1e6f) ? d_invs_acc[0] * 10.f * e : 0.f;
+    if (s_val) s_val[0] = s_val_of(e);
+    if (d_var) d_var[0] = d_var_of(e, d_invs_acc[0]);
 }
 int variance_terms(const float* variance, const float* d_invs_acc, float* s_val, float* d_var, hipStream_t st) {
     hipLaunchKernelGGL(k_variance_terms, dim3(1), dim3(64), 0, st, variance, d_invs_acc, s_val, d_var);
diff --git a/endosurf_amd/csrc/render_tail.h b/endosurf_amd/csrc/render_tail.h
--- /dev/null
+++ b/endosurf_amd/csrc/render_tail.h
@@ -0,0 +1,20 @@
+#pragma once
+#include <hip/hip_runtime.h>
+
+namespace es {
+
+__device__ __forceinline__ void finish_eik(float sum_err, float sum_relax, float* __restrict__ eik, float* __restrict__ eik_den) {
+    const float den = sum_relax + 1e-6f;
+    eik_den[0] = den;
+    eik_den[1] = den;
+    eik[0] = sum_err / den;
+}
+__device__ __forceinline__ void copy_aux_rows(int i, int n_aux, const float* __restrict__ aux_sdf_ws, const float* __restrict__ aux_go_ws,
+                                              float* __restrict__ aux_sdf, float* __restrict__ aux_go) {
+    if (i < n_aux) aux_sdf[i] = aux_sdf_ws[i];
+    if (i < 3 * n_aux) aux_go[i] = aux_go_ws[i];
+}
+__device__ __forceinline__ float s_val_of(float e) { return 1.f / fminf(fmaxf(e, 1e-6f), 1e6f); }
+__device__ __forceinline__ float d_var_of(float e, float d_invs) { return (e >= 1e-6f && e <= 1e6f) ? d_invs * 10.f * e : 0.f; }
+
+}
diff --git a/endosurf_amd/csrc/stages.hip b/endosurf_amd/csrc/stages.hip
--- a/endosurf_amd/csrc/stages.hip
+++ b/endosurf_amd/csrc/stages.hip
@@ -43,13 +43,19 @@
     const float* sdf_c = sc.sdf_c0;
     int ld_sdf = n_samples, n = n_samples;
     for (int i = 0; i < up_sample_steps; ++i) {
-        if (int e = upsample_step(rays, zbuf[cur], S, sdf_c, ld_sdf, N, n, n_imp, 64.f * (float)(1 << i), sc.z_new, zbuf[cur ^ 1], S, sc.src, st)) return e;
-        if (i + 1 != up_sample_steps) {
+        const float inv_s = 64.f * (float)(1 << i);
+        const bool last = i + 1 == up_sample_steps;
+        if (i == 0) {
+            if (int e = upsample_step(rays, zbuf[cur], S, sdf_c, ld_sdf, N, n, n_imp, inv_s, sc.z_new, zbuf[cur ^ 1], S, sc.src, st)) return e;
+        } else {
+            float* dst = last ? nullptr : (sdf_c != sc.sdf_a ? sc.sdf_a : sc.sdf_b);
+            if (int e = upsample_merge_step(rays, zbuf[cur], S, sdf_c, ld_sdf, n - n_imp, sc.sdf_new, n_imp, sc.src, S, dst, N, n_imp, inv_s,
+                                            sc.z_new, zbuf[cur ^ 1], S, sc.src, st)) return e;
+            if (dst != nullptr) { sdf_c = dst; ld_sdf = S; }
+        }
+        if (!last) {
             ps.z = sc.z_new; ps.n_per_ray = n_imp; ps.ldz = n_imp; ps.M = N * n_imp;
             if (int e = query_sdf(ps, packed, weff, sc.sdf_new, use_deform, st)) return e;
-            float* dst = sdf_c != sc.sdf_a ? sc.sdf_a : sc.sdf_b;
-            if (int e = merge_sdf(sdf_c, ld_sdf, sc.sdf_new, n_imp, sc.src, S, N, n, dst, st)) return e;
-            sdf_c = dst; ld_sdf = S;
         }
         cur ^= 1;
         n += n_imp;
diff --git a/endosurf_amd/csrc/step.hip b/endosurf_amd/csrc/step.hip
--- a/endosurf_amd/csrc/step.hip
+++ b/endosurf_amd/csrc/step.hip
@@ -4,29 +4,21 @@
 
 #include "host.h"
 #include "launch.h"
+#include "philox.h"
+#include "render_tail.h"
 
 namespace es {
 
-__device__ __forceinline__ void philox_round(uint32_t (&c)[4], uint32_t k0, uint32_t k1) {
-    const uint64_t p0 = (uint64_t)0xD2511F53u * c[0], p1 = (uint64_t)0xCD9E8D57u * c[2];
-    const uint32_t n0 = (uint32_t)(p1 >> 32) ^ c[1] ^ k0, n2 = (uint32_t)(p0 >> 32) ^ c[3] ^ k1;
-    c[1] = (uint32_t)p1; c[3] = (uint32_t)p0; c[0] = n0; c[2] = n2;
-}
 __global__ __launch_bounds__(256) void k_uniform(float* __restrict__ out, long long n, unsigned long long seed, unsigned long long subseq,
                                                  const double* __restrict__ subseq_dev) {
     const long long q = (long long)blockIdx.x * 256 + threadIdx.x;
     if (4 * q >= n) return;
     if (subseq_dev != nullptr) subseq += (unsigned long long)subseq_dev[0];
-    uint32_t c[4] = {(uint32_t)q, (uint32_t)((unsigned long long)q >> 32), (uint32_t)subseq, (uint32_t)(subseq >> 32)};
-    uint32_t k0 = (uint32_t)seed, k1 = (uint32_t)(seed >> 32);
-#pragma unroll
-    for (int r = 0; r < 10; ++r) {
-        philox_round(c, k0, k1);
-        k0 += 0x9E3779B9u; k1 += 0xBB67AE85u;
-    }
+    float u[4];
+    philox_uniform4((unsigned long long)q, seed, subseq, u);
 #pragma unroll
     for (int j = 0; j < 4; ++j)
-        if (4 * q + j < n) out[4 * q + j] = (float)(c[j] >> 8) * (1.f / 16777216.f);
+        if (4 * q + j < n) out[4 * q + j] = u[j];
 }
 int uniform(float* out, long long n, unsigned long long seed, unsigned long long subseq, const double* subseq_dev, hipStream_t st) {
     if (n <= 0) return ST_OK;
@@ -55,14 +47,8 @@
                                                        const float* __restrict__ aux_go_ws, int n_aux, float* __restrict__ eik,
                                                        float* __restrict__ eik_den, float* __restrict__ aux_sdf, float* __restrict__ aux_go) {
     const int i = blockIdx.x * 256 + threadIdx.x;
-    if (i == 0) {
-        const float den = eik_acc[1] + 1e-6f;
-        eik_den[0] = den;
-        eik_den[1] = den;
-        eik[0] = eik_acc[0] / den;
-    }
-    if (i < n_aux) aux_sdf[i] = aux_sdf_ws[i];
-    if (i < 3 * n_aux) aux_go[i] = aux_go_ws[i];
+    if (i == 0) finish_eik(eik_acc[0], eik_acc[1], eik, eik_den);
+    copy_aux_rows(i, n_aux, aux_sdf_ws, aux_go_ws, aux_sdf, aux_go);
 }
 int render_finish(const float* eik_acc, const float* aux_sdf_ws, const float* aux_go_ws, int n_aux, float* eik, float* eik_den, float* aux_sdf,
                   float* aux_go, hipStream_t st) {
diff --git a/endosurf_amd/engine.py b/endosurf_amd/engine.py
--- a/endosurf_amd/engine.py
+++ b/endosurf_amd/engine.py
@@ -118,6 +118,11 @@
 
     def uniform(self, n: int, step_dev: Optional[torch.Tensor] = None) -> torch.Tensor:
         out = self.empty(int(n))
+        seed, sub = self._next_subsequence(step_dev)
+        check(self.lib.es_uniform(ptr(out), int(n), seed, sub, ptr(step_dev) if step_dev is not None else None, self.st()), "es_uniform")
+        return out
+
+    def _next_subsequence(self, step_dev):
         seed = int(torch.initial_seed()) & 0xFFFFFFFFFFFFFFFF
         if step_dev is not None:
             sub = (1 << 63) + (self._rng_step_calls << 40)
@@ -125,8 +130,15 @@
         else:
             sub = self._rng_calls
             self._rng_calls += 1
-        check(self.lib.es_uniform(ptr(out), int(n), seed, sub, ptr(step_dev) if step_dev is not None else None, self.st()), "es_uniform")
-        return out
+        return seed, sub
+
+    def step_setup(self, rays, n_march: int, n_samples: int, S: int, step_dev: Optional[torch.Tensor] = None):
+        N = rays.shape[0]
+        u4, dprop, z = self.empty(4 * N), self.empty(N, n_march), self.empty(N, S)
+        seed, sub = self._next_subsequence(step_dev)
+        check(self.lib.es_step_setup(ptr(rays), N, seed, sub, ptr(step_dev) if step_dev is not None else None, ptr(u4), int(n_march), ptr(dprop),
+                                     int(n_samples), float(2.0 / n_samples), ptr(z), int(S), self.st()), "es_step_setup")
+        return u4, dprop, z
 
     def weightnorm_pack(self, flat_params: torch.Tensor, use_deform: bool):
         weff = self.empty(self.n_weff)
@@ -222,24 +234,38 @@
                                     z.shape[1], ptr(near), ptr(far), self.st()), "es_ray_setup")
         return near, far
 
+    MARCH_STEPS = 128
+
+    @staticmethod
+    def sample_columns(n_samples, n_importance, up_sample_steps, upsample: bool) -> int:
+        do_up = upsample and n_importance > 0 and up_sample_steps > 0
+        n_imp = n_importance // up_sample_steps if do_up else 0
+        if do_up and n_imp == 0:
+            raise ValueError(f"n_importance = {n_importance} gives no new sample in any of the {up_sample_steps} up-sampling steps")
+        return n_samples + up_sample_steps * n_imp
+
     def sample_z(self, rays, u_perturb, weff, packed, use_deform, n_samples, n_importance, up_sample_steps, upsample: bool,
-                 trace: Optional[list] = None, racing: bool = False):
+                 trace: Optional[list] = None, racing: bool = False, z_coarse: Optional[torch.Tensor] = None):
         N = rays.shape[0]
         n = n_samples
         sample_dist = 2.0 / n_samples
         do_up = upsample and n_importance > 0 and up_sample_steps > 0
         n_imp = n_importance // up_sample_steps if do_up else 0
-        if do_up and n_imp == 0:
-            raise ValueError(f"n_importance = {n_importance} gives no new sample in any of the {up_sample_steps} up-sampling steps")
-        S = n + up_sample_steps * n_imp
-        if do_up and not racing and trace is None and N > 0 and n_importance % up_sample_steps == 0 and not self._use_x3(N * n):
+        S = self.sample_columns(n_samples, n_importance, up_sample_steps, upsample)
+        if (do_up and not racing and trace is None and z_coarse is None and N > 0 and n_importance % up_sample_steps == 0
+                and not self._use_x3(N * n)):
             z_out = self.empty(N, S)
             scratch = self.empty(int(self.lib.es_sample_scratch_floats(N, n_samples, n_importance, up_sample_steps)))
             check(self.lib.es_sample_z(ptr(rays), ptr(u_perturb) if u_perturb is not None else None, N, n_samples, n_importance, up_sample_steps, 1,
                                        ptr(packed), ptr(weff), int(use_deform), ptr(z_out), ptr(scratch), self.st()), "es_sample_z")
             return z_out
-        zc = self.empty(N, S)
-        self.ray_setup(rays, u_perturb, n, sample_dist, 0, zc)
+        if z_coarse is not None:
+            if tuple(z_coarse.shape) != (N, S):
+                raise ValueError(f"z_coarse has shape {tuple(z_coarse.shape)}, expected {(N, S)}")
+            zc = z_coarse
+        else:
+            zc = self.empty(N, S)
+            self.ray_setup(rays, u_perturb, n, sample_dist, 0, zc)
         if trace is not None:
             trace.append(zc[:, :n].clone())
         if not do_up:
@@ -251,13 +277,19 @@
         sdf_a, sdf_b = self.empty(N, S), self.empty(N, S)
         src = self.empty(N, S, dtype=torch.int32)
         z_new = self.empty(N, n_imp)
+        sdf_new = None
         for i in range(up_sample_steps):
-            self.upsample_step(rays, zc, S, sdf_c, ld_sdf, N, n, n_imp, 64 * 2 ** i, z_new, zn, S, src)
-            if i + 1 != up_sample_steps:
+            last = i + 1 == up_sample_steps
+            if i == 0:
+                self.upsample_step(rays, zc, S, sdf_c, ld_sdf, N, n, n_imp, 64 * 2 ** i, z_new, zn, S, src)
+            else:
+                dst = None if last else (sdf_a if sdf_c.data_ptr() != sdf_a.data_ptr() else sdf_b)
+                check(self.lib.es_upsample_merge_step(ptr(rays), ptr(zc), S, ptr(sdf_c), ld_sdf, n - n_imp, ptr(sdf_new), n_imp, ptr(src), S, ptr(dst), N,
+                                                      n_imp, float(64 * 2 ** i), ptr(z_new), ptr(zn), S, ptr(src), self.st()), "es_upsample_merge_step")
+                if dst is not None:
+                    sdf_c, ld_sdf = dst, S
+            if not last:
                 sdf_new = self.query_sdf(self.points(rays=rays, z=z_new, n_per_ray=n_imp, ldz=n_imp), weff, packed, use_deform)
-                dst = sdf_a if sdf_c.data_ptr() != sdf_a.data_ptr() else sdf_b
-                self.merge_sdf(sdf_c, ld_sdf, sdf_new, n_imp, src, S, N, n, dst)
-                sdf_c, ld_sdf = dst, S
             zc, zn = zn, zc
             n += n_imp
             if trace is not None:
@@ -287,8 +319,14 @@
             a._keep.append(part)
         return a
 
-    def composite_forward(self, a: es_composite_args, eik_acc=None, go_copy: bool = False):
+    def composite_forward(self, a: es_composite_args, eik_acc=None, go_copy: bool = False, finish=None):
         N, S = a.N, a.S
+        counter = None
+        if finish is not None:
+            if eik_acc is not None:
+                raise ValueError("composite_forward: the epilogue needs a launch that owns eik_acc")
+            acc = self.zeros(4)
+            eik_acc, counter = acc[0:2], acc[2:3]
         out = dict(color=self.empty(N, 3), depth=self.empty(N, 1), weights=self.empty(N, S), cdf=self.empty(N, S),
                    weight_max=self.empty(N, 1), eik_acc=eik_acc if eik_acc is not None else self.zeros(2),
                    wmax_idx=self.empty(N, dtype=torch.int32))
@@ -298,11 +336,18 @@
             out["go"] = self.empty(N, S, 3)
             a.go_copy = ptr(out["go"])
         a._keep.append(out)
+        if finish is not None:
+            aux_sdf_ws, aux_go_ws, n_aux, eik, den2, aux_sdf, aux_go, s_val = finish
+            a._keep += [counter, finish]
+            check(self.lib.es_composite_forward_finish(C.byref(a), ptr(counter), ptr(aux_sdf_ws), ptr(aux_go_ws), int(n_aux), ptr(eik), ptr(den2),
+                                                       ptr(aux_sdf), ptr(aux_go), ptr(s_val), self.st()), "es_composite_forward_finish")
+            return out
         check(self.lib.es_composite_forward(C.byref(a), self.st()), "es_composite_forward")
         return out
 
     def composite_backward(self, a: es_composite_args, g_color, g_depth, g_eik, eik_den, g_weights=None, g_cdf=None, g_wmax=None,
-                           g_gradients_o=None, d_invs_acc=None, n_aux: int = 0, g_aux_sdf=None, g_aux_go=None):
+                           g_gradients_o=None, d_invs_acc=None, n_aux: int = 0, g_aux_sdf=None, g_aux_go=None, d_var=None,
+                           counter=None):
         N, S = a.N, a.S
         out = dict(d_sdf=self.empty(N * S + n_aux), d_go=self.empty(N * S + n_aux, 3), d_rgb=self.empty(N * S, 3),
                    d_invs_acc=d_invs_acc if d_invs_acc is not None else self.zeros(1))
@@ -318,6 +363,10 @@
         for k, v in out.items():
             setattr(a, k, ptr(v))
         a._keep += keep + [out]
+        if d_var is not None:
+            a._keep += [counter, d_var]
+            check(self.lib.es_composite_backward_finish(C.byref(a), ptr(counter), ptr(d_var), self.st()), "es_composite_backward_finish")
+            return out
         check(self.lib.es_composite_backward(C.byref(a), self.st()), "es_composite_backward")
         return out
 
@@ -330,10 +379,13 @@
             check(self.lib.es_variance_terms(ptr(v), ptr(d_invs_acc), None, ptr(out), self.st()), "es_variance_terms")
         return out
 
-    def march_begin(self, rays, weff, packed, use_deform, n_steps=128, tau=0.0):
+    def march_begin(self, rays, weff, packed, use_deform, n_steps=128, tau=0.0, dprop=None):
         N = rays.shape[0]
-        dprop = self.empty(N, n_steps)
-        self.ray_setup(rays, None, n_steps, 0.0, 1, dprop)
+        if dprop is None:
+            dprop = self.empty(N, n_steps)
+            self.ray_setup(rays, None, n_steps, 0.0, 1, dprop)
+        elif tuple(dprop.shape) != (N, n_steps):
+            raise ValueError(f"dprop has shape {tuple(dprop.shape)}, expected {(N, n_steps)}")
         B = self.march_block
         if B and n_steps % B == 0 and n_steps > B and N * B >= 16384:
             sdf = self.zeros(N, n_steps)
diff --git a/endosurf_amd/functions.py b/endosurf_amd/functions.py
--- a/endosurf_amd/functions.py
+++ b/endosurf_amd/functions.py
@@ -40,8 +40,8 @@
 class _SValFn(torch.autograd.Function):
 
     @staticmethod
-    def forward(ctx, variance, eng: Engine):
-        s = eng.variance_terms(variance.detach())
+    def forward(ctx, variance, eng: Engine, s_pre=None):
+        s = s_pre[0] if s_pre is not None else eng.variance_terms(variance.detach())
         ctx.save_for_backward(s)
         ctx.shape = variance.shape
         return s.reshape(variance.shape)
@@ -50,7 +50,7 @@
     def backward(ctx, g):
         s, = ctx.saved_tensors
         inside = ((s > 1e-6) & (s < 1e6)).to(s.dtype)
-        return (g.reshape(1) * -10.0 * s * inside).reshape(ctx.shape), None
+        return (g.reshape(1) * -10.0 * s * inside).reshape(ctx.shape), None, None
 
 
 class _PointEvalFn(torch.autograd.Function):
@@ -224,7 +224,7 @@
             den_out = ctx.eik_den.clone()
             ctx.mark_non_differentiable(cat["wmax_idx"], den_out)
             return (cat["color"], cat["depth"], cat["go"], eik, cat["weights"], cat["weight_max"], cat["cdf"], cat["wmax_idx"],
-                    eng.zeros(0, 1), eng.zeros(0, 3), den_out, eng.empty(1))
+                    eng.zeros(0, 1), eng.zeros(0, 3), den_out, eng.empty(1), None)
         ctx.chunk_rays = 0
         mid = eng.mid_z(z, sample_dist)
         fused = aux_x is not None and aux_x.shape[0] > 0 and P_ % 64 == 0
@@ -239,21 +239,27 @@
             pctx = eng.point_forward(pts, weff, packed, flags | _lib.PF_COLOR, m_color=P_ if fused else 0)
         sdf_all, go_all = pctx.view("sdf"), pctx.view("go")
         a = eng.composite_args(rays, z, sdf_all.view(-1), go_all, pctx.view("rgb"), var1, sample_dist, cos_anneal)
-        out = eng.composite_forward(a, go_copy=True)
         n_aux = aux_x.shape[0] if fused else 0
         eik, den2 = eng.empty(1), eng.empty(2)
         aux_sdf, aux_go = eng.empty(n_aux, 1), eng.empty(n_aux, 3)
-        eng.render_finish(out["eik_acc"], sdf_all[P_:] if n_aux else None, go_all[P_:] if n_aux else None, n_aux, eik, den2,
-                          aux_sdf if n_aux else None, aux_go if n_aux else None)
+        finish = (sdf_all[P_:] if n_aux else None, go_all[P_:] if n_aux else None, n_aux, eik, den2, aux_sdf if n_aux else None,
+                  aux_go if n_aux else None)
+        s_val = None
+        if N > 0:
+            s_val = eng.empty(1)
+            out = eng.composite_forward(a, go_copy=True, finish=finish + (s_val,))
+        else:
+            out = eng.composite_forward(a, go_copy=True)
+            eng.render_finish(out["eik_acc"], *finish)
         eik_den, den_out = den2[0:1], den2[1:2]
         ctx.pctx, ctx.eik_den = pctx, eik_den
         ctx.n_aux = n_aux
-        ctx.mark_non_differentiable(out["wmax_idx"], den_out)
+        ctx.mark_non_differentiable(out["wmax_idx"], den_out, *([s_val] if s_val is not None else []))
         return (out["color"], out["depth"], out["go"], eik.reshape(()), out["weights"], out["weight_max"], out["cdf"], out["wmax_idx"], aux_sdf,
-                aux_go, den_out, eng.empty(1))
-
-    @staticmethod
-    def backward(ctx, g_color, g_depth, g_go, g_eik, g_weights, g_wmax, g_cdf, _, g_aux_sdf, g_aux_go, _g_den=None, _g_token=None):
+                aux_go, den_out, eng.empty(1), s_val)
+
+    @staticmethod
+    def backward(ctx, g_color, g_depth, g_go, g_eik, g_weights, g_wmax, g_cdf, _, g_aux_sdf, g_aux_go, _g_den=None, _g_token=None, _g_sval=None):
         eng = ctx.eng
         tail = ctx.tail
         if tail is not None:
@@ -276,8 +282,10 @@
         g_weights, g_cdf, g_go = opt(g_weights), opt(g_cdf), opt(g_go)
         g_wmax = g_wmax.contiguous().view(-1) if g_wmax is not None else None
         sl = lambda g, i, j: g[i:j] if g is not None else None
-        d_invs_acc = eng.zeros(1)
+        acc = eng.zeros(2)
+        d_invs_acc, counter = acc[0:1], acc[1:2]
         dweff = eng.zeros(eng.n_weff) if N == 0 else None
+        dvar1 = eng.empty(1) if (N > 0 and not ctx.chunk_rays) else None
         C = max(1, ctx.chunk_rays if ctx.chunk_rays else N)
         for i in range(0, N, C):
             j = min(i + C, N)
@@ -290,11 +298,11 @@
             a = eng.composite_args(r_, z_, pctx.view("sdf").view(-1), pctx.view("go"), pctx.view("rgb"), var1, sample_dist, cos_anneal)
             bw = eng.composite_backward(a, g_color[i:j], g_depth[i:j], g_eik, ctx.eik_den, g_weights=sl(g_weights, i, j), g_cdf=sl(g_cdf, i, j),
                                         g_wmax=sl(g_wmax, i, j), g_gradients_o=sl(g_go, i, j), d_invs_acc=d_invs_acc, n_aux=ctx.n_aux,
-                                        g_aux_sdf=opt(g_aux_sdf), g_aux_go=opt(g_aux_go))
+                                        g_aux_sdf=opt(g_aux_sdf), g_aux_go=opt(g_aux_go), d_var=dvar1, counter=counter)
             d_sdf, d_go = bw["d_sdf"].view(-1, 1), bw["d_go"]
             dweff = eng.point_backward(pctx, ctx.weff, ctx.packed, d_sdf, d_go, bw["d_rgb"], dweff=dweff, staged=not ctx.chunk_rays)
             del pctx
-        dvar = eng.variance_terms(var, d_invs_acc=d_invs_acc).reshape(ctx.variance.shape)
+        dvar = (dvar1 if dvar1 is not None else eng.variance_terms(var, d_invs_acc=d_invs_acc)).reshape(ctx.variance.shape)
         ctx.pctx = None
         if tail is not None:
             tail.close(eng)
diff --git a/endosurf_amd/renderer.py b/endosurf_amd/renderer.py
--- a/endosurf_amd/renderer.py
+++ b/endosurf_amd/renderer.py
@@ -203,7 +203,7 @@
         self.__dict__.pop("_fwd_graphs", None)
 
     @_on_device
-    def sample_z(self, rays, iter_step=0, perturb_overwrite=None, u_perturb=None, racing=False):
+    def sample_z(self, rays, iter_step=0, perturb_overwrite=None, u_perturb=None, racing=False, z_coarse=None):
         rays = self._rays32(rays)
         weff, packed = self._weights()
         perturb = self.perturb if perturb_overwrite is None else perturb_overwrite
@@ -214,7 +214,7 @@
         upsample = iter_step >= self.important_begin_iter and self.n_importance > 0
         with torch.no_grad():
             return self.engine.sample_z(rays, u, weff.detach(), packed, self.use_deform, self.n_samples, self.n_importance,
-                                        self.up_sample_steps, upsample, racing=racing)
+                                        self.up_sample_steps, upsample, racing=racing, z_coarse=z_coarse)
 
     def _rays_from(self, rays_o, rays_d, time=None):
         n = rays_o.shape[0]
@@ -312,13 +312,13 @@
         flags = self._flags(weff)
         chunk = self._chunk_rays(z.shape[0], z.shape[1], flags)
         tail = self._new_tail(z.numel(), flags, chunk, z.shape[0]) if _aux is None else None
-        color, depth, g_o, eik, weights, wmax, cdf, _, aux_sdf, aux_go, eik_den, token = _RenderFn.apply(
+        color, depth, g_o, eik, weights, wmax, cdf, _, aux_sdf, aux_go, eik_den, token, s_pre = _RenderFn.apply(
             weff, packed, var, self.engine, _rays, z, float(sample_dist), cos_anneal_ratio if torch.is_tensor(cos_anneal_ratio) else float(cos_anneal_ratio), flags, aux_x, aux_t,
             chunk, tail)
         self._live_tail = (tail, token) if (tail is not None and tail.pctx is not None) else None
         if _aux is not None and aux_sdf.shape[0] != aux_x.shape[0]:
             aux_sdf, aux_go = self._point_eval(aux_x, aux_t)
-        s_val = _SValFn.apply(var, self.engine)
+        s_val = _SValFn.apply(var, self.engine, [s_pre.detach()] if s_pre is not None else None)
         return {"color_map": color, "depth_map": depth, "gradients_o": g_o, "gradient_o_error": eik, "cdf": cdf,
                 "weights": weights, "weight_max": wmax, "s_val": s_val, "aux_sdf": aux_sdf, "aux_gradients_o": aux_go, "eik_den": eik_den}
 
@@ -433,10 +433,10 @@
         _, g = self._point_eval(pp, tt)
         return self._sn_loss(g, valid)
 
-    def _march_begin(self, rays):
-        weff, packed = self._weights()
-        with torch.no_grad():
-            return self.engine.march_begin(self._rays32(rays), weff.detach(), packed, self.use_deform)
+    def _march_begin(self, rays, dprop=None):
+        weff, packed = self._weights()
+        with torch.no_grad():
+            return self.engine.march_begin(self._rays32(rays), weff.detach(), packed, self.use_deform, dprop=dprop)
 
     def _march_refine(self, ms):
         with torch.no_grad():
diff --git a/endosurf_amd/trainer.py b/endosurf_amd/trainer.py
--- a/endosurf_amd/trainer.py
+++ b/endosurf_amd/trainer.py
@@ -37,7 +37,13 @@
     N = rays.shape[0]
     eng = renderer.engine
     need_p, need_n = renderer.perturb and u_perturb is None, u_neigh is None
-    if need_p or need_n:
+    dprop = z_coarse = None
+    if need_p and need_n and N > 0:
+        upsample = iter_step >= renderer.important_begin_iter and renderer.n_importance > 0
+        S = eng.sample_columns(renderer.n_samples, renderer.n_importance, renderer.up_sample_steps, upsample)
+        u4, dprop, z_coarse = eng.step_setup(rays, eng.MARCH_STEPS, renderer.n_samples, S, renderer._rng_step_dev)
+        u_perturb, u_neigh = u4[:N], u4[N:].view(N, 3)
+    elif need_p or need_n:
         u4 = eng.uniform(4 * N, renderer._rng_step_dev)
         if need_p:
             u_perturb = u4[:N]
@@ -48,10 +54,12 @@
     side = renderer._side_stream
     if side is None:
         side = renderer._side_stream = torch.cuda.Stream(device=rays.device)
-    ms = renderer._march_begin(rays)
+    ms = renderer._march_begin(rays, dprop=dprop)
     side.wait_stream(main)
+    if z_coarse is not None and not torch.cuda.is_current_stream_capturing():
+        z_coarse.record_stream(side)
     with torch.cuda.stream(side):
-        z = renderer.sample_z(rays, iter_step, u_perturb=u_perturb, racing=True)
+        z = renderer.sample_z(rays, iter_step, u_perturb=u_perturb, racing=True, z_coarse=z_coarse)
     d_i = renderer._march_refine(ms)
     aux_x, aux_t, valid_sn = renderer._train_aux_points(rays, depth_gt, mask_gt, d_i, surf_neig_rad, u_neigh)
     eod_pts = aux_x[:N]
diff --git a/include/endosurf_hip.h b/include/endosurf_hip.h
--- a/include/endosurf_hip.h
+++ b/include/endosurf_hip.h
@@ -72,6 +72,11 @@
                      float inv_s, float* z_new, float* z_out, int ld_out, int32_t* src_idx, void* stream);
 int es_merge_sdf(const float* sdf_in, int ld_in, const float* sdf_new, int n_imp, const int32_t* src_idx, int ld_out, int N, int n,
                  float* sdf_out, void* stream);
+int es_upsample_merge_step(const float* rays, const float* z_in, int ld_in, const float* sdf_old, int ld_old, int n_old, const float* sdf_new,
+                           int n_new, const int32_t* src_prev, int ld_src, float* sdf_out, int N, int n_imp, float inv_s, float* z_new,
+                           float* z_out, int ld_out, int32_t* src_idx, void* stream);
+int es_step_setup(const float* rays, int N, unsigned long long seed, unsigned long long subsequence, const double* subsequence_dev, float* u4,
+                  int n_march, float* dprop, int n_samples, float sample_dist, float* z, int ldz, void* stream);
 int es_mid_z(const float* z, int ldz, int N, int S, float sample_dist, float* mid, void* stream);
 
 typedef struct es_composite_args {
@@ -89,6 +94,9 @@
 } es_composite_args;
 int es_composite_forward(const es_composite_args* a, void* stream);
 int es_composite_backward(const es_composite_args* a, void* stream);
+int es_composite_forward_finish(const es_composite_args* a, int32_t* counter, const float* aux_sdf_ws, const float* aux_go_ws, int n_aux, float* eik,
+                                float* eik_den, float* aux_sdf, float* aux_go, float* s_val, void* stream);
+int es_composite_backward_finish(const es_composite_args* a, int32_t* counter, float* d_var, void* stream);
 int es_variance_terms(const float* variance, const float* d_invs_acc, float* s_val, float* d_var, void* stream);
 
 int64_t es_sample_scratch_floats(int N, int n_samples, int n_importance, int up_sample_steps);
```

Result: no change. 73040, median of 2 (+0.1%).
